# GenkiK/monodepth2

Measured on AMD Instinct MI355X. Metric: training images/sec at 640x192 mono, 1/2/4/8 GPUs; loss delta vs ref, higher is better.
Workload: dtype f32; 1 GPU; mono_640x192 ResNet-18 batch=12/GPU full train step (configs[1]); global_batch=12, height=192, width=640, parallelism=dp1, step=hipgraph replay

## Files before the change

include/md2hot.h:

```cpp
#ifndef MD2HOT_H
#define MD2HOT_H

#include <stddef.h>
#include <stdint.h>

#ifdef __cplusplus
extern "C" {
#endif

#define MD2_ABI_VERSION 24
#define MD2_MAX_SCALES 4
#define MD2_MAX_SRC 3

#define MD2_OK 0
#define MD2_ERR_ARG (-1)
#define MD2_ERR_HIP (-2)

#define MD2_NO_SSIM          (1u << 0)
#define MD2_AVG_REPROJECTION (1u << 1)
#define MD2_NO_AUTOMASK      (1u << 2)
#define MD2_V1_MULTISCALE    (1u << 3)
#define MD2_T_PER_SCALE      (1u << 4)
#define MD2_PREDICTIVE_MASK  (1u << 5)

#define MD2_DTYPE_F32  0u
#define MD2_DTYPE_BF16 1u

typedef struct md2_desc {
    int32_t batch;
    int32_t height, width;
    int32_t num_src;
    int32_t num_scales;
    uint32_t flags;
    float min_depth, max_depth;
    float disparity_smoothness;
    uint32_t disp_dtype;
    uint64_t seed;
} md2_desc;

typedef struct md2_tensors {
    const float* disp[MD2_MAX_SCALES];
    const float* color[MD2_MAX_SCALES][1 + MD2_MAX_SRC];
    const float* K[MD2_MAX_SCALES];
    const float* inv_K[MD2_MAX_SCALES];
    const float* T;
    const float* noise;
    const uint64_t* seed_ptr;
    const float* mask;
    const uint32_t* src8;
} md2_tensors;

int md2_abi_version(void);
const char* md2_last_error(void);
const char* md2_build_id(void);

size_t md2_workspace_bytes(const md2_desc* desc);

size_t md2_select_bytes(const md2_desc* desc);

int md2_photometric_fwd(const md2_desc* desc, const md2_tensors* t,
                        float* loss_out, uint8_t* select_out,
                        void* workspace, void* stream);

int md2_photometric_bwd(const md2_desc* desc, const md2_tensors* t,
                        const float* grad_loss, const uint8_t* select,
                        float* const* grad_disp, float* grad_T, float* grad_mask,
                        void* workspace, void* stream);

int md2_generate_images(const md2_desc* desc, const md2_tensors* t,
                        float* const* depth_out, float* const* sample_out,
                        float* const* color_out, void* stream);

int md2_tiebreak_noise(const md2_desc* desc, const uint64_t* seed_ptr, int scale,
                       float* out, void* stream);

int md2_timing_begin(int max_launches);
int md2_timing_end(double* fwd_ms, int* n_fwd, double* bwd_ms, int* n_bwd);
int md2_timing_calls(double* fwd_ms, int* n_fwd, double* bwd_ms, int* n_bwd);

#define MD2_PAD_ELU      (1u << 0)
#define MD2_PAD_UPSAMPLE (1u << 1)
#define MD2_PAD_NHWC     (1u << 2)
#define MD2_PAD_BF16     (1u << 3)

typedef struct md2_pad_desc {
    int32_t batch, channels, height, width;
    int32_t skip_channels;
    uint32_t flags;
} md2_pad_desc;

size_t md2_decoder_pad_workspace_bytes(const md2_pad_desc* desc);
int md2_decoder_pad_fwd(const md2_pad_desc* desc, const float* x, const float* skip, const float* bias,
                        float* out, void* stream);
int md2_decoder_pad_bwd(const md2_pad_desc* desc, const float* x, const float* bias, const float* grad_out,
                        float* grad_x, float* grad_skip, float* grad_bias, void* workspace, void* stream);
int md2_decoder_pad_bwd2(const md2_pad_desc* desc, const float* x, const float* bias, const float* grad_out,
                         const float* grad_out2, float* grad_x, float* grad_skip, float* grad_bias, void* workspace,
                         void* stream);

#define MD2_HEAD_WEIGHT_CL (1u << 0)
#define MD2_HEAD_BF16 (1u << 1)

typedef struct md2_head_desc {
    int32_t batch, channels, height, width;
    uint32_t flags;
} md2_head_desc;

size_t md2_disp_head_workspace_bytes(const md2_head_desc* desc);
int md2_disp_head_fwd(const md2_head_desc* desc, const float* padded, const float* weight, const float* bias,
                      float* disp, void* stream);
int md2_disp_head_bwd(const md2_head_desc* desc, const float* padded, const float* weight, const float* disp,
                      const float* grad_disp, float* grad_padded, float* grad_weight, float* grad_bias,
                      void* workspace, void* stream);

#define MD2_STEM_WEIGHT_CL (1u << 0)
#define MD2_STEM_BF16 (1u << 1)

typedef struct md2_stem_desc {
    int32_t batch, channels, height, width;
    uint32_t flags;
} md2_stem_desc;

size_t md2_stem_wgrad_workspace_bytes(const md2_stem_desc* desc);
int md2_stem_wgrad(const md2_stem_desc* desc, const float* x, const float* grad_y, float* grad_weight,
                   void* workspace, void* stream);

int md2_stem_fwd(const md2_stem_desc* desc, const float* x, const float* weight, float* y, void* stream);

#define MD2_BIAS_ACT_RELU (1u << 0)

typedef struct md2_bias_act_desc {
    int64_t pixels;
    int32_t channels;
    uint32_t flags;
} md2_bias_act_desc;

int md2_bias_act_fwd(const md2_bias_act_desc* desc, const float* x, const float* bias, float* y, void* stream);
size_t md2_bias_act_workspace_bytes(const md2_bias_act_desc* desc);
int md2_bias_act_bwd(const md2_bias_act_desc* desc, const float* y, const float* grad_y, float* grad_x,
                     float* grad_bias, void* workspace, void* stream);

int md2_encoder_input(int groups, int batch, int slots, int height, int width, const float* const* src, float mean,
                      float std_, float* out, void* stream);

typedef struct md2_adam_chunk {
    float* p;
    float* m;
    float* v;
    int64_t off;
    int64_t n;
    int32_t param;
    int32_t reserved;
} md2_adam_chunk;

int md2_adam_step(const md2_adam_chunk* table, const int* chunk_start, int nparams, const float* const* grads,
                  double lr, double beta1, double beta2, double eps, int step, void* stream);
int md2_adam_step_dev(const md2_adam_chunk* table, const int* chunk_start, int nparams, const float* const* grads,
                      const double* lr, double beta1, double beta2, double eps, float* step, float* hyper,
                      void* stream);
int md2_adam_hyper(const double* lr, double beta1, double beta2, float* step, float* hyper, void* stream);
int md2_adam_apply_dev(const md2_adam_chunk* table, const int* chunk_start, int k_begin, int k_end,
                       const float* const* grads, double beta1, double beta2, double eps, const float* hyper,
                       void* stream);

int md2_pose_fwd(int32_t frames, int32_t batch, uint32_t invert_mask, const float* axisangle,
                 const float* translation, float* T, void* stream);
int md2_pose_bwd(int32_t frames, int32_t batch, uint32_t invert_mask, const float* axisangle,
                 const float* translation, const float* grad_T, float* grad_axisangle,
                 float* grad_translation, void* stream);

typedef struct md2_aug_desc {
    int32_t items;
    int32_t frames;
    int32_t in_height, in_width;
    int32_t height, width;
    int32_t num_scales;
    int32_t reserved;
} md2_aug_desc;

#define MD2_AUG_BRIGHTNESS 0
#define MD2_AUG_CONTRAST   1
#define MD2_AUG_SATURATION 2
#define MD2_AUG_HUE        3

typedef struct md2_aug_item {
    uint8_t flip;
    uint8_t color_aug;
    uint8_t hue_shift;
    uint8_t reserved;
    uint8_t order[4];
    float brightness, contrast, saturation;
} md2_aug_item;

typedef struct md2_aug_plan md2_aug_plan;

md2_aug_plan* md2_aug_plan_create(const md2_aug_desc* desc);
void md2_aug_plan_destroy(md2_aug_plan* plan);

int md2_aug_run(md2_aug_plan* plan, const uint8_t* frames, const md2_aug_item* items,
                float* const* color, float* const* color_aug, void* stream);
int md2_aug_run2(md2_aug_plan* plan, const uint8_t* frames, const md2_aug_item* items,
                 float* const* color, float* const* color_aug, uint32_t* src8, void* stream);

#define MD2_BN_RELU     (1u << 0)
#define MD2_BN_RESIDUAL (1u << 1)
#define MD2_BN_BF16     (1u << 2)

typedef struct md2_bn_desc {
    int64_t pixels;
    int32_t channels;
    uint32_t flags;
    float eps, momentum;
    int32_t groups;
    int32_t reserved;
} md2_bn_desc;

size_t md2_bn_workspace_bytes(const md2_bn_desc* desc);
int md2_bn_fwd(const md2_bn_desc* desc, const void* x, const float* gamma, const float* beta,
               const void* residual, float* running_mean, float* running_var, void* y,
               float* save_mean, float* save_invstd, void* workspace, void* stream);
int md2_bn_bwd(const md2_bn_desc* desc, const void* x, const void* y, const void* grad_y,
               const float* gamma, const float* save_mean, const float* save_invstd,
               void* grad_x, void* grad_residual, float* grad_gamma, float* grad_beta,
               void* workspace, void* stream);
int md2_bn_bwd_multi(const md2_bn_desc* desc, const void* x, const void* y, const void* grad_y,
                     const void* grad_y2, const void* grad_y3, const float* gamma, const float* save_mean,
                     const float* save_invstd, void* grad_x, void* grad_residual, float* grad_gamma,
                     float* grad_beta, void* workspace, void* stream);
int md2_bn_fwd_mask(const md2_bn_desc* desc, const void* x, const float* gamma, const float* beta,
                    const void* residual, float* running_mean, float* running_var, void* y, uint8_t* relu_mask,
                    float* save_mean, float* save_invstd, void* workspace, void* stream);
int md2_bn_bwd_mask(const md2_bn_desc* desc, const void* x, const uint8_t* relu_mask, const void* grad_y,
                    const void* grad_y2, const void* grad_y3, const float* gamma, const float* save_mean,
                    const float* save_invstd, void* grad_x, void* grad_residual, float* grad_gamma,
                    float* grad_beta, void* workspace, void* stream);

#define MD2_POOL_BF16 (1u << 0)

typedef struct md2_pool_desc {
    int32_t batch, channels, height, width;
    uint32_t flags;
    int32_t reserved;
} md2_pool_desc;

int md2_maxpool3s2_fwd(const md2_pool_desc* desc, const void* x, void* y, uint32_t* idx, void* stream);
int md2_maxpool3s2_bwd(const md2_pool_desc* desc, const uint32_t* idx, const void* grad_y, void* grad_x,
                       void* stream);
int md2_maxpool3s2_bwd_add(const md2_pool_desc* desc, const uint32_t* idx, const void* grad_y, const void* grad_add,
                           void* grad_x, void* stream);
int md2_maxpool3s2_bwd_multi(const md2_pool_desc* desc, const uint32_t* idx, const void* grad_y, const void* grad_y2,
                             const void* grad_add, void* grad_x, void* stream);

#define MD2_CONV_NO_SPLIT  (1u << 1)
#define MD2_CONV_TILE_N32  (1u << 2)
#define MD2_CONV_TILE_N64  (1u << 3)
#define MD2_CONV_TILE_N128 (1u << 4)
#define MD2_CONV_X6        (1u << 5)
#define MD2_CONV_BM256     (1u << 6)
#define MD2_CONV_PRESPLIT  (1u << 7)
#define MD2_CONV_PATCH     (1u << 8)
#define MD2_CONV_S2_ONE    (1u << 9)
#define MD2_CONV_WS        (1u << 10)
#define MD2_CONV_BF16      (1u << 11)

typedef struct md2_conv_desc {
    int32_t batch, height, width, in_channels;
    int32_t out_channels, kernel_h, kernel_w, stride, pad;
    uint32_t flags;
} md2_conv_desc;

size_t md2_conv_workspace_bytes(const md2_conv_desc* desc);
int md2_conv_split_weights(const md2_conv_desc* desc, const float* weight, void* planes_fwd, void* planes_dgrad,
                           void* stream);
typedef struct md2_wsplit_entry {
    const float* weight;
    void* planes_fwd;
    void* planes_dgrad;
    int32_t co, kt, ci;
    int32_t block0;
    void* planes_col;
} md2_wsplit_entry;
int md2_conv_split_weights_multi(const md2_wsplit_entry* table, int n, int total_blocks, void* stream);
int md2_conv_bf16_weights(const md2_conv_desc* desc, const float* weight, void* w_fwd, void* w_dgrad, void* stream);
int md2_conv_bf16_weights_multi(const md2_wsplit_entry* table, int n, int total_blocks, void* stream);
int md2_conv_fwd(const md2_conv_desc* desc, const float* x, const float* weight, float* y, void* workspace,
                 void* stream);
int md2_conv_dgrad(const md2_conv_desc* desc, const float* grad_y, const float* weight, float* grad_x,
                   void* workspace, void* stream);
int md2_conv_col2im(const md2_conv_desc* desc, const float* cols, float* grad_x, void* stream);
int md2_conv_wgrad(const md2_conv_desc* desc, const float* x, const float* grad_y, float* grad_weight,
                   void* workspace, void* stream);
int md2_conv_direct(const md2_conv_desc* desc, const float* x, const float* wk, float* y, void* stream);
size_t md2_conv_wgrad_direct_workspace_bytes(const md2_conv_desc* desc);
int md2_conv_wgrad_direct(const md2_conv_desc* desc, const float* x, const float* grad_y, float* grad_weight,
                          void* workspace, void* stream);

#define MD2_EVAL_POST_PROCESS (1u << 0)
#define MD2_EVAL_RESIZE_DEPTH (1u << 1)
#define MD2_EVAL_GT_RANGE     (1u << 2)
#define MD2_EVAL_MEDIAN_SCALE (1u << 3)
#define MD2_EVAL_MEDIAN_LOWER (1u << 4)
#define MD2_EVAL_POOL_BATCH   (1u << 5)
#define MD2_EVAL_OUT 10

typedef struct md2_eval_desc {
    int32_t batch;
    int32_t height, width;
    int32_t gt_height, gt_width;
    int32_t crop_y0, crop_y1, crop_x0, crop_x1;
    uint32_t flags;
    double min_depth, max_depth;
    float eval_min, eval_max;
    double scale_factor;
} md2_eval_desc;

size_t md2_depth_eval_workspace_bytes(const md2_eval_desc* desc);
int md2_depth_eval(const md2_eval_desc* desc, const float* disp, const float* disp_flipped, const float* gt,
                   float* out, void* workspace, void* stream);

#define MD2_VELO_VEL_DEPTH (1u << 0)

typedef struct md2_velo_desc {
    int32_t batch;
    int32_t height, width;
    uint32_t flags;
    int64_t total_points;
    int32_t reserved[2];
} md2_velo_desc;

size_t md2_velo_project_workspace_bytes(const md2_velo_desc* desc);
int md2_velo_project(const md2_velo_desc* desc, const float* points, const int64_t* offsets, const double* P,
                     float* depth, void* workspace, void* stream);

typedef struct md2_pose_ate_desc {
    int32_t sequences;
    int32_t track_length;
    uint32_t flags;
    int32_t reserved0;
    int64_t total_frames;
    int64_t reserved;
} md2_pose_ate_desc;

size_t md2_pose_ate_workspace_bytes(const md2_pose_ate_desc* desc);
int md2_pose_ate(const md2_pose_ate_desc* desc, const float* pred, const double* gt, const int64_t* offsets,
                 double* ates, double* stats, void* workspace, void* stream);

typedef struct md2_viz_desc {
    int32_t batch;
    int32_t in_height, in_width;
    int32_t out_height, out_width;
    int32_t percentile;
    uint32_t flags;
    int32_t reserved;
} md2_viz_desc;

size_t md2_disp_colorize_workspace_bytes(const md2_viz_desc* desc);
int md2_disp_colorize(const md2_viz_desc* desc, const float* disp, uint8_t* rgb, float* resized, float* stats,
                      void* workspace, void* stream);

#ifdef __cplusplus
}
#endif
#endif
```

monodepth2_amd/_lib.py:

```python
from __future__ import annotations

import ctypes
import os
import threading

import torch

from .build import LIB_PATH as _BUILT_LIB
from .build import source_hash

LIB_PATH = os.environ.get("MD2_LIB", _BUILT_LIB)

MAX_SCALES = 4
MAX_SRC = 3
ABI_VERSION = 24

NO_SSIM = 1 << 0
AVG_REPROJECTION = 1 << 1
NO_AUTOMASK = 1 << 2
V1_MULTISCALE = 1 << 3
T_PER_SCALE = 1 << 4
PREDICTIVE_MASK = 1 << 5

_vp = ctypes.c_void_p


class Desc(ctypes.Structure):
    _fields_ = [("batch", ctypes.c_int32), ("height", ctypes.c_int32), ("width", ctypes.c_int32),
                ("num_src", ctypes.c_int32), ("num_scales", ctypes.c_int32), ("flags", ctypes.c_uint32),
                ("min_depth", ctypes.c_float), ("max_depth", ctypes.c_float),
                ("disparity_smoothness", ctypes.c_float), ("disp_dtype", ctypes.c_uint32),
                ("seed", ctypes.c_uint64)]


class Tensors(ctypes.Structure):
    _fields_ = [("disp", _vp * MAX_SCALES),
                ("color", (_vp * (1 + MAX_SRC)) * MAX_SCALES),
                ("K", _vp * MAX_SCALES),
                ("inv_K", _vp * MAX_SCALES),
                ("T", _vp),
                ("noise", _vp),
                ("seed_ptr", _vp),
                ("mask", _vp),
                ("src8", _vp)]


_lock = threading.Lock()
_lib = None

EXPORTS = ["md2_abi_version", "md2_last_error", "md2_workspace_bytes", "md2_select_bytes",
           "md2_photometric_fwd", "md2_photometric_bwd", "md2_generate_images", "md2_tiebreak_noise",
           "md2_timing_begin", "md2_timing_end", "md2_timing_calls", "md2_decoder_pad_fwd", "md2_decoder_pad_bwd",
           "md2_decoder_pad_workspace_bytes", "md2_adam_step", "md2_adam_step_dev", "md2_adam_hyper", "md2_adam_apply_dev", "md2_encoder_input",
           "md2_pose_fwd", "md2_pose_bwd", "md2_aug_plan_create", "md2_aug_plan_destroy", "md2_aug_run",
           "md2_bn_workspace_bytes", "md2_bn_fwd", "md2_bn_bwd", "md2_maxpool3s2_fwd", "md2_maxpool3s2_bwd",
           "md2_disp_head_workspace_bytes", "md2_disp_head_fwd", "md2_disp_head_bwd",
           "md2_stem_wgrad_workspace_bytes", "md2_stem_wgrad", "md2_stem_fwd", "md2_conv_col2im", "md2_bias_act_fwd", "md2_bias_act_bwd",
           "md2_bias_act_workspace_bytes", "md2_maxpool3s2_bwd_add", "md2_bn_bwd_multi",
           "md2_conv_fwd", "md2_conv_workspace_bytes", "md2_conv_split_weights",
           "md2_conv_dgrad", "md2_conv_wgrad", "md2_conv_direct", "md2_conv_wgrad_direct",
           "md2_conv_wgrad_direct_workspace_bytes", "md2_conv_split_weights_multi", "md2_bn_fwd_mask",
           "md2_bn_bwd_mask", "md2_build_id", "md2_maxpool3s2_bwd_multi", "md2_decoder_pad_bwd2", "md2_aug_run2",
           "md2_conv_bf16_weights", "md2_conv_bf16_weights_multi",
           "md2_depth_eval", "md2_depth_eval_workspace_bytes",
           "md2_velo_project", "md2_velo_project_workspace_bytes",
           "md2_pose_ate", "md2_pose_ate_workspace_bytes",
           "md2_disp_colorize", "md2_disp_colorize_workspace_bytes"]

DTYPE_F32 = 0
DTYPE_BF16 = 1
PAD_ELU = 1 << 0
PAD_UPSAMPLE = 1 << 1
PAD_NHWC = 1 << 2
PAD_BF16 = 1 << 3


class PadDesc(ctypes.Structure):
    _fields_ = [("batch", ctypes.c_int32), ("channels", ctypes.c_int32), ("height", ctypes.c_int32),
                ("width", ctypes.c_int32), ("skip_channels", ctypes.c_int32), ("flags", ctypes.c_uint32)]


class AugDesc(ctypes.Structure):
    _fields_ = [("items", ctypes.c_int32), ("frames", ctypes.c_int32), ("in_height", ctypes.c_int32),
                ("in_width", ctypes.c_int32), ("height", ctypes.c_int32), ("width", ctypes.c_int32),
                ("num_scales", ctypes.c_int32), ("reserved", ctypes.c_int32)]


class AugItem(ctypes.Structure):
    _fields_ = [("flip", ctypes.c_uint8), ("color_aug", ctypes.c_uint8), ("hue_shift", ctypes.c_uint8),
                ("reserved", ctypes.c_uint8), ("order", ctypes.c_uint8 * 4), ("brightness", ctypes.c_float),
                ("contrast", ctypes.c_float), ("saturation", ctypes.c_float)]


BN_RELU = 1 << 0
BN_RESIDUAL = 1 << 1
BN_BF16 = 1 << 2


class BnDesc(ctypes.Structure):
    _fields_ = [("pixels", ctypes.c_int64), ("channels", ctypes.c_int32), ("flags", ctypes.c_uint32),
                ("eps", ctypes.c_float), ("momentum", ctypes.c_float), ("groups", ctypes.c_int32),
                ("reserved", ctypes.c_int32)]


POOL_BF16 = 1 << 0


CONV_NO_SPLIT = 1 << 1
CONV_TILE_N32 = 1 << 2
CONV_TILE_N64 = 1 << 3
CONV_TILE_N128 = 1 << 4
CONV_X6 = 1 << 5
CONV_BM256 = 1 << 6
CONV_PRESPLIT = 1 << 7
CONV_PATCH = 1 << 8
CONV_S2_ONE = 1 << 9
CONV_WS = 1 << 10
CONV_BF16 = 1 << 11


class ConvDesc(ctypes.Structure):
    _fields_ = [("batch", ctypes.c_int32), ("height", ctypes.c_int32), ("width", ctypes.c_int32),
                ("in_channels", ctypes.c_int32), ("out_channels", ctypes.c_int32), ("kernel_h", ctypes.c_int32),
                ("kernel_w", ctypes.c_int32), ("stride", ctypes.c_int32), ("pad", ctypes.c_int32),
                ("flags", ctypes.c_uint32)]


class WsplitEntry(ctypes.Structure):
    _fields_ = [("weight", _vp), ("planes_fwd", _vp), ("planes_dgrad", _vp), ("co", ctypes.c_int32),
                ("kt", ctypes.c_int32), ("ci", ctypes.c_int32), ("block0", ctypes.c_int32), ("planes_col", _vp)]


class PoolDesc(ctypes.Structure):
    _fields_ = [("batch", ctypes.c_int32), ("channels", ctypes.c_int32), ("height", ctypes.c_int32),
                ("width", ctypes.c_int32), ("flags", ctypes.c_uint32), ("reserved", ctypes.c_int32)]


HEAD_WEIGHT_CL = 1 << 0
HEAD_BF16 = 1 << 1


class HeadDesc(ctypes.Structure):
    _fields_ = [("batch", ctypes.c_int32), ("channels", ctypes.c_int32), ("height", ctypes.c_int32),
                ("width", ctypes.c_int32), ("flags", ctypes.c_uint32)]


STEM_WEIGHT_CL = 1 << 0
STEM_BF16 = 1 << 1


class StemDesc(ctypes.Structure):
    _fields_ = [("batch", ctypes.c_int32), ("channels", ctypes.c_int32), ("height", ctypes.c_int32),
                ("width", ctypes.c_int32), ("flags", ctypes.c_uint32)]


BIAS_ACT_RELU = 1 << 0


class BiasActDesc(ctypes.Structure):
    _fields_ = [("pixels", ctypes.c_int64), ("channels", ctypes.c_int32), ("flags", ctypes.c_uint32)]


EVAL_POST_PROCESS = 1 << 0
EVAL_RESIZE_DEPTH = 1 << 1
EVAL_GT_RANGE = 1 << 2
EVAL_MEDIAN_SCALE = 1 << 3
EVAL_MEDIAN_LOWER = 1 << 4
EVAL_POOL_BATCH = 1 << 5
EVAL_OUT = 10


class EvalDesc(ctypes.Structure):
    _fields_ = [("batch", ctypes.c_int32), ("height", ctypes.c_int32), ("width", ctypes.c_int32),
                ("gt_height", ctypes.c_int32), ("gt_width", ctypes.c_int32),
                ("crop_y0", ctypes.c_int32), ("crop_y1", ctypes.c_int32), ("crop_x0", ctypes.c_int32),
                ("crop_x1", ctypes.c_int32), ("flags", ctypes.c_uint32),
                ("min_depth", ctypes.c_double), ("max_depth", ctypes.c_double),
                ("eval_min", ctypes.c_float), ("eval_max", ctypes.c_float),
                ("scale_factor", ctypes.c_double)]


VELO_VEL_DEPTH = 1 << 0


class VeloDesc(ctypes.Structure):
    _fields_ = [("batch", ctypes.c_int32), ("height", ctypes.c_int32), ("width", ctypes.c_int32),
                ("flags", ctypes.c_uint32), ("total_points", ctypes.c_int64), ("reserved", ctypes.c_int32 * 2)]


class PoseAteDesc(ctypes.Structure):
    _fields_ = [("sequences", ctypes.c_int32), ("track_length", ctypes.c_int32), ("flags", ctypes.c_uint32),
                ("reserved0", ctypes.c_int32), ("total_frames", ctypes.c_int64), ("reserved", ctypes.c_int64)]


class VizDesc(ctypes.Structure):
    _fields_ = [("batch", ctypes.c_int32), ("in_height", ctypes.c_int32), ("in_width", ctypes.c_int32),
                ("out_height", ctypes.c_int32), ("out_width", ctypes.c_int32), ("percentile", ctypes.c_int32),
                ("flags", ctypes.c_uint32), ("reserved", ctypes.c_int32)]


def _declare(L):
    L.md2_disp_colorize_workspace_bytes.restype = ctypes.c_size_t
    L.md2_disp_colorize_workspace_bytes.argtypes = [ctypes.POINTER(VizDesc)]
    L.md2_disp_colorize.restype = ctypes.c_int
    L.md2_disp_colorize.argtypes = [ctypes.POINTER(VizDesc)] + [_vp] * 6
    L.md2_pose_ate_workspace_bytes.restype = ctypes.c_size_t
    L.md2_pose_ate_workspace_bytes.argtypes = [ctypes.POINTER(PoseAteDesc)]
    L.md2_pose_ate.restype = ctypes.c_int
    L.md2_pose_ate.argtypes = [ctypes.POINTER(PoseAteDesc)] + [_vp] * 7
    L.md2_velo_project_workspace_bytes.restype = ctypes.c_size_t
    L.md2_velo_project_workspace_bytes.argtypes = [ctypes.POINTER(VeloDesc)]
    L.md2_velo_project.restype = ctypes.c_int
    L.md2_velo_project.argtypes = [ctypes.POINTER(VeloDesc)] + [_vp] * 6
    L.md2_depth_eval_workspace_bytes.restype = ctypes.c_size_t
    L.md2_depth_eval_workspace_bytes.argtypes = [ctypes.POINTER(EvalDesc)]
    L.md2_depth_eval.restype = ctypes.c_int
    L.md2_depth_eval.argtypes = [ctypes.POINTER(EvalDesc)] + [_vp] * 6
    L.md2_bias_act_fwd.restype = ctypes.c_int
    L.md2_bias_act_fwd.argtypes = [ctypes.POINTER(BiasActDesc)] + [_vp] * 4
    L.md2_bias_act_bwd.restype = ctypes.c_int
    L.md2_bias_act_bwd.argtypes = [ctypes.POINTER(BiasActDesc)] + [_vp] * 6
    L.md2_bias_act_workspace_bytes.restype = ctypes.c_size_t
    L.md2_bias_act_workspace_bytes.argtypes = [ctypes.POINTER(BiasActDesc)]
    L.md2_conv_fwd.restype = ctypes.c_int
    L.md2_conv_fwd.argtypes = [ctypes.POINTER(ConvDesc)] + [_vp] * 5
    L.md2_conv_dgrad.restype = ctypes.c_int
    L.md2_conv_dgrad.argtypes = [ctypes.POINTER(ConvDesc)] + [_vp] * 5
    L.md2_conv_wgrad.restype = ctypes.c_int
    L.md2_conv_wgrad.argtypes = [ctypes.POINTER(ConvDesc)] + [_vp] * 5
    L.md2_conv_split_weights.restype = ctypes.c_int
    L.md2_conv_direct.restype = ctypes.c_int
    L.md2_conv_direct.argtypes = [ctypes.POINTER(ConvDesc)] + [_vp] * 4
    L.md2_conv_wgrad_direct.restype = ctypes.c_int
    L.md2_conv_wgrad_direct.argtypes = [ctypes.POINTER(ConvDesc)] + [_vp] * 5
    L.md2_conv_wgrad_direct_workspace_bytes.restype = ctypes.c_size_t
    L.md2_conv_wgrad_direct_workspace_bytes.argtypes = [ctypes.POINTER(ConvDesc)]
    L.md2_conv_split_weights.argtypes = [ctypes.POINTER(ConvDesc)] + [_vp] * 4
    L.md2_conv_split_weights_multi.restype = ctypes.c_int
    L.md2_conv_split_weights_multi.argtypes = [_vp, ctypes.c_int, ctypes.c_int, _vp]
    L.md2_conv_bf16_weights.restype = ctypes.c_int
    L.md2_conv_bf16_weights.argtypes = [ctypes.POINTER(ConvDesc)] + [_vp] * 4
    L.md2_conv_bf16_weights_multi.restype = ctypes.c_int
    L.md2_conv_bf16_weights_multi.argtypes = [_vp, ctypes.c_int, ctypes.c_int, _vp]
    L.md2_conv_workspace_bytes.restype = ctypes.c_size_t
    L.md2_conv_workspace_bytes.argtypes = [ctypes.POINTER(ConvDesc)]
    L.md2_stem_wgrad_workspace_bytes.restype = ctypes.c_size_t
    L.md2_stem_wgrad_workspace_bytes.argtypes = [ctypes.POINTER(StemDesc)]
    L.md2_stem_wgrad.restype = ctypes.c_int
    L.md2_stem_wgrad.argtypes = [ctypes.POINTER(StemDesc)] + [_vp] * 5
    L.md2_stem_fwd.restype = ctypes.c_int
    L.md2_conv_col2im.restype = ctypes.c_int
    L.md2_conv_col2im.argtypes = [ctypes.POINTER(ConvDesc)] + [_vp] * 3
    L.md2_stem_fwd.argtypes = [ctypes.POINTER(StemDesc)] + [_vp] * 4
    L.md2_disp_head_workspace_bytes.restype = ctypes.c_size_t
    L.md2_disp_head_workspace_bytes.argtypes = [ctypes.POINTER(HeadDesc)]
    L.md2_disp_head_fwd.restype = ctypes.c_int
    L.md2_disp_head_fwd.argtypes = [ctypes.POINTER(HeadDesc)] + [_vp] * 5
    L.md2_disp_head_bwd.restype = ctypes.c_int
    L.md2_disp_head_bwd.argtypes = [ctypes.POINTER(HeadDesc)] + [_vp] * 9
    L.md2_abi_version.restype = ctypes.c_int
    L.md2_abi_version.argtypes = []
    L.md2_build_id.restype = ctypes.c_char_p
    L.md2_build_id.argtypes = []
    L.md2_last_error.restype = ctypes.c_char_p
    L.md2_last_error.argtypes = []
    L.md2_workspace_bytes.restype = ctypes.c_size_t
    L.md2_workspace_bytes.argtypes = [ctypes.POINTER(Desc)]
    L.md2_select_bytes.restype = ctypes.c_size_t
    L.md2_select_bytes.argtypes = [ctypes.POINTER(Desc)]
    L.md2_photometric_fwd.restype = ctypes.c_int
    L.md2_photometric_fwd.argtypes = [ctypes.POINTER(Desc), ctypes.POINTER(Tensors), _vp, _vp, _vp, _vp]
    L.md2_photometric_bwd.restype = ctypes.c_int
    L.md2_photometric_bwd.argtypes = [ctypes.POINTER(Desc), ctypes.POINTER(Tensors), _vp, _vp,
                                      ctypes.POINTER(_vp), _vp, _vp, _vp, _vp]
    L.md2_generate_images.restype = ctypes.c_int
    L.md2_generate_images.argtypes = [ctypes.POINTER(Desc), ctypes.POINTER(Tensors),
                                      ctypes.POINTER(_vp), ctypes.POINTER(_vp), ctypes.POINTER(_vp), _vp]
    L.md2_tiebreak_noise.restype = ctypes.c_int
    L.md2_tiebreak_noise.argtypes = [ctypes.POINTER(Desc), _vp, ctypes.c_int, _vp, _vp]
    L.md2_decoder_pad_fwd.restype = ctypes.c_int
    L.md2_decoder_pad_fwd.argtypes = [ctypes.POINTER(PadDesc), _vp, _vp, _vp, _vp, _vp]
    L.md2_decoder_pad_bwd.restype = ctypes.c_int
    L.md2_decoder_pad_bwd.argtypes = [ctypes.POINTER(PadDesc), _vp, _vp, _vp, _vp, _vp, _vp, _vp, _vp]
    L.md2_decoder_pad_bwd2.restype = ctypes.c_int
    L.md2_decoder_pad_bwd2.argtypes = [ctypes.POINTER(PadDesc)] + [_vp] * 9
    L.md2_encoder_input.restype = ctypes.c_int
    L.md2_encoder_input.argtypes = [ctypes.c_int, ctypes.c_int, ctypes.c_int, ctypes.c_int, ctypes.c_int, _vp,
                                    ctypes.c_float, ctypes.c_float, _vp, _vp]
    L.md2_adam_step.restype = ctypes.c_int
    L.md2_adam_step.argtypes = [_vp, _vp, ctypes.c_int, _vp, ctypes.c_double, ctypes.c_double, ctypes.c_double,
                                ctypes.c_double, ctypes.c_int, _vp]
    L.md2_adam_step_dev.restype = ctypes.c_int
    L.md2_adam_step_dev.argtypes = [_vp, _vp, ctypes.c_int, _vp, _vp, ctypes.c_double, ctypes.c_double,
                                    ctypes.c_double, _vp, _vp, _vp]
    L.md2_adam_hyper.restype = ctypes.c_int
    L.md2_adam_hyper.argtypes = [_vp, ctypes.c_double, ctypes.c_double, _vp, _vp, _vp]
    L.md2_adam_apply_dev.restype = ctypes.c_int
    L.md2_adam_apply_dev.argtypes = [_vp, _vp, ctypes.c_int, ctypes.c_int, _vp, ctypes.c_double, ctypes.c_double,
                                     ctypes.c_double, _vp, _vp]
    L.md2_decoder_pad_workspace_bytes.restype = ctypes.c_size_t
    L.md2_decoder_pad_workspace_bytes.argtypes = [ctypes.POINTER(PadDesc)]
    L.md2_pose_fwd.restype = ctypes.c_int
    L.md2_pose_fwd.argtypes = [ctypes.c_int32, ctypes.c_int32, ctypes.c_uint32, _vp, _vp, _vp, _vp]
    L.md2_pose_bwd.restype = ctypes.c_int
    L.md2_pose_bwd.argtypes = [ctypes.c_int32, ctypes.c_int32, ctypes.c_uint32, _vp, _vp, _vp, _vp, _vp, _vp]
    L.md2_aug_plan_create.restype = _vp
    L.md2_aug_plan_create.argtypes = [ctypes.POINTER(AugDesc)]
    L.md2_aug_plan_destroy.restype = None
    L.md2_aug_plan_destroy.argtypes = [_vp]
    L.md2_aug_run.restype = ctypes.c_int
    L.md2_aug_run.argtypes = [_vp, _vp, _vp, ctypes.POINTER(_vp), ctypes.POINTER(_vp), _vp]
    L.md2_aug_run2.restype = ctypes.c_int
    L.md2_aug_run2.argtypes = [_vp, _vp, _vp, ctypes.POINTER(_vp), ctypes.POINTER(_vp), _vp, _vp]
    L.md2_bn_workspace_bytes.restype = ctypes.c_size_t
    L.md2_bn_workspace_bytes.argtypes = [ctypes.POINTER(BnDesc)]
    L.md2_bn_fwd.restype = ctypes.c_int
    L.md2_bn_fwd.argtypes = [ctypes.POINTER(BnDesc)] + [_vp] * 11
    L.md2_bn_bwd.restype = ctypes.c_int
    L.md2_bn_bwd.argtypes = [ctypes.POINTER(BnDesc)] + [_vp] * 12
    L.md2_maxpool3s2_fwd.restype = ctypes.c_int
    L.md2_maxpool3s2_fwd.argtypes = [ctypes.POINTER(PoolDesc), _vp, _vp, _vp, _vp]
    L.md2_maxpool3s2_bwd.restype = ctypes.c_int
    L.md2_maxpool3s2_bwd.argtypes = [ctypes.POINTER(PoolDesc), _vp, _vp, _vp, _vp]
    L.md2_bn_bwd_multi.restype = ctypes.c_int
    L.md2_bn_bwd_multi.argtypes = [ctypes.POINTER(BnDesc)] + [_vp] * 14
    L.md2_bn_fwd_mask.restype = ctypes.c_int
    L.md2_bn_fwd_mask.argtypes = [ctypes.POINTER(BnDesc)] + [_vp] * 12
    L.md2_bn_bwd_mask.restype = ctypes.c_int
    L.md2_bn_bwd_mask.argtypes = [ctypes.POINTER(BnDesc)] + [_vp] * 14
    L.md2_maxpool3s2_bwd_add.restype = ctypes.c_int
    L.md2_maxpool3s2_bwd_add.argtypes = [ctypes.POINTER(PoolDesc)] + [_vp] * 5
    L.md2_maxpool3s2_bwd_multi.restype = ctypes.c_int
    L.md2_maxpool3s2_bwd_multi.argtypes = [ctypes.POINTER(PoolDesc)] + [_vp] * 6
    L.md2_timing_begin.restype = ctypes.c_int
    L.md2_timing_begin.argtypes = [ctypes.c_int]
    L.md2_timing_calls.restype = ctypes.c_int
    L.md2_timing_calls.argtypes = [ctypes.POINTER(ctypes.c_double), ctypes.POINTER(ctypes.c_int),
                                   ctypes.POINTER(ctypes.c_double), ctypes.POINTER(ctypes.c_int)]
    L.md2_timing_end.restype = ctypes.c_int
    L.md2_timing_end.argtypes = [ctypes.POINTER(ctypes.c_double), ctypes.POINTER(ctypes.c_int),
                                 ctypes.POINTER(ctypes.c_double), ctypes.POINTER(ctypes.c_int)]


def lib():
    global _lib
    if _lib is not None:
        return _lib
    with _lock:
        if _lib is None:
            if not os.path.exists(LIB_PATH):
                raise RuntimeError(
                    f"{LIB_PATH} is not built. Build it with `python -m monodepth2_amd.build` "
                    "(hipcc --offload-arch=gfx950); there is no CPU fallback.")
            L = ctypes.CDLL(LIB_PATH, mode=ctypes.RTLD_GLOBAL)
# ... 47 lines not shown
```

monodepth2_amd/bn_ops.py:

```python
from __future__ import annotations

import contextlib
import ctypes
import os
from typing import Dict, Optional

import torch
import torch.nn as nn
import torch.nn.functional as F

from . import _lib

ENABLED = True
_GROUPS = 1


@contextlib.contextmanager
def bn_groups(n: int):
    global _GROUPS
    prev, _GROUPS = _GROUPS, int(n)
    try:
        yield
    finally:
        _GROUPS = prev
# ... 18 lines not shown
_descs: Dict[tuple, tuple] = {}


def _desc(key: tuple):
    hit = _descs.get(key)
    if hit is None:
        d = _lib.BnDesc(*key, 0)
        hit = _descs[key] = (d, _lib.lib().md2_bn_workspace_bytes(ctypes.byref(d)))
    return hit


def _supported(C: int) -> bool:
    Q = C // 4
    return C % 4 == 0 and Q > 0 and (Q & (Q - 1)) == 0


class _BNAct(torch.autograd.Function):

    @staticmethod
    def forward(ctx, x, weight, bias, running_mean, running_var, residual, relu: bool, eps: float,
                momentum: float, groups: int, aliases: int = 0):
        B, C, H, W = x.shape
        flags = ((_lib.BN_RELU if relu else 0) | (_lib.BN_RESIDUAL if residual is not None else 0)
                 | (_lib.BN_BF16 if x.dtype == torch.bfloat16 else 0))
        key = (B * H * W, C, flags, eps, momentum, groups)
        d, nbytes = _desc(key)
        L = _lib.lib()
        ws = _workspace(x.device, nbytes)
        y = torch.empty_like(x, memory_format=_CL)
        stats = torch.empty(2, groups, C, device=x.device)
        mean, invstd = stats[0], stats[1]
        mask = torch.empty(x.numel() // 4, dtype=torch.uint8, device=x.device) if relu else None
        stream = _lib.stream(x.device)
        rc = L.md2_bn_fwd_mask(ctypes.byref(d), x.data_ptr(), weight.data_ptr(), bias.data_ptr(),
                               residual.data_ptr() if residual is not None else None,
                               running_mean.data_ptr() if running_mean is not None else None,
                               running_var.data_ptr() if running_var is not None else None,
                               y.data_ptr(), mask.data_ptr() if mask is not None else None,
                               mean.data_ptr(), invstd.data_ptr(), ws.data_ptr(), stream)
        _lib.check(rc, "md2_bn_fwd_mask")
        ctx.save_for_backward(x, mask, weight, mean, invstd)
        ctx.desc = key
        ctx.has_res = residual is not None
        if aliases:
            ctx.set_materialize_grads(False)
            return (y,) + tuple(y.view_as(y) for _ in range(aliases))
        return y

    @staticmethod
    def backward(ctx, *grads):
        x, mask, weight, mean, invstd = ctx.saved_tensors
        gs = [g.to(x.dtype).contiguous(memory_format=_CL) for g in grads if g is not None]
        if not gs:
            return (None,) * 11
        gy = gs[0]
        d, nbytes = _desc(ctx.desc)
        L = _lib.lib()
        ws = _workspace(x.device, nbytes)
        gx = torch.empty_like(x, memory_format=_CL)
        gr = torch.empty_like(x, memory_format=_CL) if ctx.has_res else None
        gw = torch.empty_like(weight)
        gb = torch.empty_like(weight)
        bwd, name = (L.md2_bn_bwd_mask, "md2_bn_bwd_mask") if mask is not None else \
            (L.md2_bn_bwd_multi, "md2_bn_bwd_multi")
        rc = bwd(ctypes.byref(d), x.data_ptr(), mask.data_ptr() if mask is not None else None,
                 gy.data_ptr(), gs[1].data_ptr() if len(gs) > 1 else None,
                 gs[2].data_ptr() if len(gs) > 2 else None,
                 weight.data_ptr(), mean.data_ptr(), invstd.data_ptr(), gx.data_ptr(),
                 gr.data_ptr() if gr is not None else None, gw.data_ptr(), gb.data_ptr(), ws.data_ptr(),
                 _lib.stream(x.device))
        _lib.check(rc, name)
        return gx, gw, gb, None, None, gr, None, None, None, None, None


def bn_act(bn: nn.BatchNorm2d, x: torch.Tensor, residual: Optional[torch.Tensor] = None,
           relu: bool = True, aliases: int = 0):
    if not 0 <= aliases <= 2:
        raise ValueError("bn_act: at most two aliases")
    groups = _GROUPS if bn.training else 1
    if groups > 1 and x.shape[0] % groups:
        raise ValueError(f"batch {x.shape[0]} does not split into {groups} BatchNorm groups")
    if (ENABLED and bn.training and x.is_cuda and x.dtype in (torch.float32, torch.bfloat16) and x.dim() == 4
            and bn.affine and bn.track_running_stats and bn.momentum is not None and _supported(x.shape[1])
            and x.numel() // 4 // groups < 2 ** 31
            and x.is_contiguous(memory_format=_CL) and x.shape[1] > 1
            and (residual is None or residual.is_contiguous(memory_format=_CL))):
        if residual is not None and residual.dtype != x.dtype:
            residual = residual.to(x.dtype)
        if bn.num_batches_tracked is not None:
            bn.num_batches_tracked.add_(groups)
        k = aliases if torch.is_grad_enabled() else 0
        out = _BNAct.apply(x, bn.weight, bn.bias, bn.running_mean, bn.running_var, residual, relu, bn.eps,
                           bn.momentum, groups, k)
        if aliases and not k:
            return (out,) * (aliases + 1)
        return out
    y = bn(x) if groups == 1 else torch.cat([bn(xc) for xc in x.chunk(groups)], 0)
    if residual is not None:
        y = y + residual
    y = F.relu(y) if relu else y
    return (y,) * (aliases + 1) if aliases else y


_ALIAS_SUM = os.environ.get("MD2_ALIAS_SUM", "1") != "0"


class _MaxPool(torch.autograd.Function):

    @staticmethod
    def forward(ctx, x, with_alias: bool = False, out_alias: bool = False):
        B, C, H, W = x.shape
        Ho, Wo = (H - 1) // 2 + 1, (W - 1) // 2 + 1
        d = _lib.PoolDesc(B, C, H, W, _lib.POOL_BF16 if x.dtype == torch.bfloat16 else 0, 0)
        y = torch.empty((B, C, Ho, Wo), device=x.device, dtype=x.dtype, memory_format=_CL)
        idx = torch.empty(B * Ho * Wo * C // 4, device=x.device, dtype=torch.int32)
        stream = _lib.stream(x.device)
        _lib.check(_lib.lib().md2_maxpool3s2_fwd(ctypes.byref(d), x.data_ptr(), y.data_ptr(), idx.data_ptr(), stream),
                   "md2_maxpool3s2_fwd")
        ctx.save_for_backward(idx)
        ctx.desc = (B, C, H, W, d.flags, 0)
        ctx.xshape, ctx.dtype = x.shape, x.dtype
        ctx.with_alias, ctx.out_alias = with_alias, out_alias
        if not (with_alias or out_alias):
            return y
        ctx.set_materialize_grads(False)
        outs = (y,) + ((y.view_as(y),) if out_alias else ()) + ((x.view_as(x),) if with_alias else ())
        return outs

    @staticmethod
    def backward(ctx, gy, *rest):
        (idx,) = ctx.saved_tensors
        rest = list(rest)
        gy2 = rest.pop(0) if ctx.out_alias else None
        galias = rest.pop(0) if ctx.with_alias else None
        if gy is None:
            gy, gy2 = gy2, None
        if gy is None:
            return (galias.to(ctx.dtype) if galias is not None else None), None, None
        gy = gy.to(ctx.dtype).contiguous(memory_format=_CL)
        if gy2 is not None:
            gy2 = gy2.to(ctx.dtype).contiguous(memory_format=_CL)
        if galias is not None:
            galias = galias.to(ctx.dtype).contiguous(memory_format=_CL)
        gx = torch.empty(ctx.xshape, device=gy.device, dtype=ctx.dtype, memory_format=_CL)
        d = _lib.PoolDesc(*ctx.desc)
        _lib.check(_lib.lib().md2_maxpool3s2_bwd_multi(ctypes.byref(d), idx.data_ptr(), gy.data_ptr(),
                                                       gy2.data_ptr() if gy2 is not None else None,
                                                       galias.data_ptr() if galias is not None else None,
                                                       gx.data_ptr(), _lib.stream(gy.device)),
                   "md2_maxpool3s2_bwd_multi")
        return gx, None, None


def _pool_ok(pool: nn.MaxPool2d, x: torch.Tensor) -> bool:
    return (ENABLED and x.is_cuda and x.dim() == 4 and x.dtype in (torch.float32, torch.bfloat16)
            and x.shape[1] % 4 == 0 and x.is_contiguous(memory_format=_CL)
            and pool.kernel_size in (3, (3, 3)) and pool.stride in (2, (2, 2)) and pool.padding in (1, (1, 1))
            and pool.dilation in (1, (1, 1)) and not pool.ceil_mode and not pool.return_indices)


def max_pool_3x3s2(pool: nn.MaxPool2d, x: torch.Tensor) -> torch.Tensor:
    if _pool_ok(pool, x):
        return _MaxPool.apply(x, False)
    return pool(x)


def max_pool_3x3s2_with_alias(pool: nn.MaxPool2d, x: torch.Tensor, out_alias: bool = False):
    if _pool_ok(pool, x) and torch.is_grad_enabled() and x.requires_grad:
        if out_alias and not _ALIAS_SUM:
            y, xa = _MaxPool.apply(x, True, False)
            return y, y, xa
        return _MaxPool.apply(x, True, out_alias)
    y = max_pool_3x3s2(pool, x)
    return (y, y, x) if out_alias else (y, x)
```

monodepth2_amd/build.py:

```python
from __future__ import annotations

import hashlib
import os
import shutil
import subprocess
import sys

HERE = os.path.dirname(os.path.abspath(__file__))
CSRC = os.path.join(HERE, "csrc")
INCLUDE = os.path.join(os.path.dirname(HERE), "include")
LIB_NAME = "libmd2hot.so"
LIB_PATH = os.path.join(CSRC, LIB_NAME)
SOURCES = ["md2hot.hip", "decoder.hip", "pose.hip", "augment.hip", "bnorm.hip", "pool.hip", "adam.hip", "disphead.hip", "stem.hip", "bias_act.hip", "conv.hip", "direct.hip", "glue.hip", "eval.hip", "velo.hip", "traj.hip", "viz.hip"]
ARCH = os.environ.get("MD2_OFFLOAD_ARCH", "gfx950")


def hipcc() -> str:
    for cand in (os.environ.get("HIPCC"), "/opt/rocm/bin/hipcc", shutil.which("hipcc")):
        if cand and os.path.exists(cand):
            return cand
    raise RuntimeError("hipcc not found (ROCm toolchain required to build libmd2hot.so)")


def needs_build() -> bool:
    if not os.path.exists(LIB_PATH):
        return True
    t = os.path.getmtime(LIB_PATH)
    deps = [os.path.join(CSRC, s) for s in SOURCES] + [os.path.join(INCLUDE, "md2hot.h"),
                                                       os.path.join(CSRC, "md2_bf16.h")]
    if any(os.path.getmtime(d) > t for d in deps):
        return True
    return built_id(LIB_PATH) != source_hash()


def built_id(path: str):
    try:
        with open(path, "rb") as f:
            data = f.read()
    except OSError:
        return None
    i = data.find(BUILD_ID_MARKER)
    if i < 0:
        return None
    i += len(BUILD_ID_MARKER)
    return data[i:i + 16].decode("ascii", errors="replace")


BUILD_ID_MARKER = b"md2-build-id:"


FLAGS = {"md2hot.hip": ["-fno-slp-vectorize", "-mllvm", "--amdgpu-sched-strategy=iterative-ilp"],
         "conv.hip": ["-mllvm", "--amdgpu-sched-strategy=max-ilp"],
         "bnorm.hip": ["-mllvm", "--amdgpu-sched-strategy=max-ilp"],
         "decoder.hip": ["-mllvm", "--amdgpu-sched-strategy=max-ilp"],
         "disphead.hip": ["-fno-slp-vectorize"], "glue.hip": ["-fno-slp-vectorize"]}


def source_hash() -> str:
    h = hashlib.sha256()
    for path in [os.path.join(CSRC, s) for s in SOURCES] + [os.path.join(INCLUDE, "md2hot.h"),
                                                          os.path.join(CSRC, "md2_bf16.h")]:
        h.update(os.path.basename(path).encode())
        with open(path, "rb") as f:
            h.update(f.read())
    h.update(repr(sorted(FLAGS.items())).encode())
    h.update(ARCH.encode())
    return h.hexdigest()[:16]


def build(force: bool = False, verbose: bool = False) -> str:
    if not force and not needs_build():
        return LIB_PATH
    import concurrent.futures as cf
    objdir = os.path.join(CSRC, "obj")
    os.makedirs(objdir, exist_ok=True)
    base = [hipcc(), "-O3", f"--offload-arch={ARCH}", "-std=c++17", "-fPIC", "-I" + INCLUDE]
    bid = ['-DMD2_BUILD_ID="%s"' % source_hash()]

    def compile_one(src):
        obj = os.path.join(objdir, os.path.splitext(src)[0] + ".o")
        cmd = base + FLAGS.get(src, []) + (bid if src == "glue.hip" else []) + ["-c", os.path.join(CSRC, src), "-o", obj]
        if verbose:
            print(" ".join(cmd), file=sys.stderr)
        subprocess.run(cmd, check=True)
        return obj

    with cf.ThreadPoolExecutor(max_workers=min(len(SOURCES), os.cpu_count() or 1)) as ex:
        objs = list(ex.map(compile_one, SOURCES))
    tmp = LIB_PATH + ".tmp"
    cmd = [hipcc(), f"--offload-arch={ARCH}", "-fPIC", "-shared", "-o", tmp] + objs
    if verbose:
        print(" ".join(cmd), file=sys.stderr)
    subprocess.run(cmd, check=True)
    os.replace(tmp, LIB_PATH)
    return LIB_PATH


if __name__ == "__main__":
    print(build(force="--force" in sys.argv, verbose=True))
```

monodepth2_amd/csrc/bnorm.hip:

```cpp

#include <hip/hip_runtime.h>

#include <stdint.h>
#include <stdlib.h>

#include "md2_bf16.h"
#include "md2hot.h"

int md2_report_error(int code, const char* msg);

namespace {

constexpr int kThreads = 256;
constexpr int kMaxBlocks = 1024;

struct Map {
    int Q;
    int QPT;
    int PPB;
};

__host__ __device__ inline Map make_map(int C) {
    Map m;
    m.Q = C / 4;
    m.QPT = m.Q > kThreads ? m.Q / kThreads : 1;
    m.PPB = m.Q >= kThreads ? 1 : kThreads / m.Q;
    return m;
}

struct Work {
    float* part;
    float* coef;
};

__host__ __device__ __forceinline__ Work work(void* ws, int G, int C, int NG) {
    Work w;
    w.part = (float*)ws;
    w.coef = w.part + 2 * (size_t)NG * G * C;
    return w;
}

__device__ __forceinline__ float4 ld4(const float* p) { return *(const float4*)p; }
__device__ __forceinline__ void st4(float* p, float4 v) { *(float4*)p = v; }

template <typename T>
__device__ __forceinline__ float4 ldT(const void* p, size_t off) { return md2::ld4T<T>(p, off); }
template <typename T>
__device__ __forceinline__ void stT(void* p, size_t off, float4 v) { md2::st4T<T>(p, off, v); }

__device__ void block_partials(float4 a, float4 b, int q, int pl, const Map& m, int C, int rows, int row, Work w,
                               float4 (*lds)[kThreads]) {
    lds[0][threadIdx.x] = a;
    lds[1][threadIdx.x] = b;
    __syncthreads();
    for (int half = m.PPB / 2; half > 0; half /= 2) {
        if (pl < half) {
            const int o = threadIdx.x + half * m.Q;
            const float4 u = lds[0][o], v = lds[1][o];
            a.x += u.x; a.y += u.y; a.z += u.z; a.w += u.w;
            b.x += v.x; b.y += v.y; b.z += v.z; b.w += v.w;
            lds[0][threadIdx.x] = a;
            lds[1][threadIdx.x] = b;
        }
        __syncthreads();
    }
    if (pl == 0) {
        float* pa = w.part + (size_t)(4 * q) * rows + row;
        float* pb = w.part + ((size_t)C + 4 * q) * rows + row;
        pa[0] = a.x; pa[rows] = a.y; pa[2 * (size_t)rows] = a.z; pa[3 * (size_t)rows] = a.w;
        pb[0] = b.x; pb[rows] = b.y; pb[2 * (size_t)rows] = b.z; pb[3 * (size_t)rows] = b.w;
    }
    __syncthreads();
}

template <typename T>
__global__ void __launch_bounds__(kThreads) bn_stats_kernel(const void* __restrict__ x, long long P, int C, int G,
                                                            void* ws) {
    const Map m = make_map(C);
    const int NG = gridDim.y, grp = blockIdx.y;
    const Work w = work(ws, G, C, NG);
    x = (const char*)x + (size_t)grp * P * C * sizeof(T);
    __shared__ float4 lds[2][kThreads];
    for (int qq = 0; qq < m.QPT; ++qq) {
        const int q = (threadIdx.x % m.Q) + qq * kThreads, pl = threadIdx.x / m.Q;
        float4 s = {0.f, 0.f, 0.f, 0.f}, ss = {0.f, 0.f, 0.f, 0.f};
        auto acc = [&](const float4 v) {
            s.x += v.x; s.y += v.y; s.z += v.z; s.w += v.w;
            ss.x += v.x * v.x; ss.y += v.y * v.y; ss.z += v.z * v.z; ss.w += v.w * v.w;
        };
        const long long stride = (long long)G * m.PPB;
        long long p = (long long)blockIdx.x * m.PPB + pl;
        for (; p + 3 * stride < P; p += 4 * stride) {
            const float4 v0 = ldT<T>(x, p * C + 4 * q), v1 = ldT<T>(x, (p + stride) * C + 4 * q),
                         v2 = ldT<T>(x, (p + 2 * stride) * C + 4 * q), v3 = ldT<T>(x, (p + 3 * stride) * C + 4 * q);
            acc(v0); acc(v1); acc(v2); acc(v3);
        }
        for (; p < P; p += stride) acc(ldT<T>(x, p * C + 4 * q));
        block_partials(s, ss, q, pl, m, C, NG * G, grp * G + blockIdx.x, w, lds);
    }
}

__device__ bool channel_sums(Work w, int rows, int r0, int G, int C, int c, double& a, double& b) {
    __shared__ double red[2][kThreads / 64];
    static_assert(kMaxBlocks <= 4 * kThreads, "four partial rows per thread at most");
    const float* ca = w.part + (size_t)c * rows + r0;
    const float* cb = w.part + ((size_t)C + c) * rows + r0;
    float pa[4], pb[4];
#pragma unroll
    for (int u = 0; u < 4; ++u) {
        const int g = threadIdx.x + u * kThreads;
        pa[u] = g < G ? ca[g] : 0.f;
        pb[u] = g < G ? cb[g] : 0.f;
    }
    a = 0.0;
    b = 0.0;
#pragma unroll
    for (int u = 0; u < 4; ++u) {
        a += pa[u];
        b += pb[u];
    }
#pragma unroll
    for (int o = 32; o > 0; o >>= 1) {
        a += __shfl_xor(a, o, 64);
        b += __shfl_xor(b, o, 64);
    }
    if ((threadIdx.x & 63) == 0) {
        red[0][threadIdx.x >> 6] = a;
        red[1][threadIdx.x >> 6] = b;
    }
    __syncthreads();
    a = red[0][0];
    b = red[1][0];
#pragma unroll
    for (int i = 1; i < kThreads / 64; ++i) {
        a += red[0][i];
        b += red[1][i];
    }
    __syncthreads();
    return threadIdx.x == 0;
}

__global__ void __launch_bounds__(kThreads) bn_stats_final_kernel(long long P, int C, int G, int NG, float eps,
                                                                  float momentum, float* __restrict__ rmean,
                                                                  float* __restrict__ rvar,
                                                                  float* __restrict__ smean,
                                                                  float* __restrict__ sinvstd, void* ws) {
    const int c = blockIdx.x;
    const Work w = work(ws, G, C, NG);
    for (int grp = 0; grp < NG; ++grp) {
        double a, b;
        if (!channel_sums(w, NG * G, grp * G, G, C, c, a, b)) continue;
        const double mean = a / (double)P;
        double var = b / (double)P - mean * mean;
        var = var > 0.0 ? var : 0.0;
        smean[grp * C + c] = (float)mean;
        sinvstd[grp * C + c] = (float)(1.0 / sqrt(var + (double)eps));
        if (rmean) {
            rmean[c] = (float)((1.0 - momentum) * rmean[c] + momentum * mean);
            rvar[c] = (float)((1.0 - momentum) * rvar[c] + momentum * var * (double)P / (double)(P - 1));
        }
    }
}

template <typename T>
__device__ __forceinline__ bool stored_pos(float o) {
    if constexpr (sizeof(T) == 4) return o > 0.f;
    else return md2::bf2f(md2::f2bf(o)) > 0.f;
}

template <typename T, bool RELU, bool RES, bool MOUT = false>
__global__ void __launch_bounds__(kThreads) bn_apply_kernel(const void* __restrict__ x, const void* __restrict__ r,
                                                            const float* __restrict__ gamma,
                                                            const float* __restrict__ beta,
                                                            const float* __restrict__ smean,
                                                            const float* __restrict__ sinvstd, void* __restrict__ y,
                                                            int n4g, int Q, uint8_t* __restrict__ mask = nullptr) {
    const size_t base = (size_t)blockIdx.y * n4g;
    const float* mug = smean + (size_t)blockIdx.y * 4 * Q;
    const float* isg = sinvstd + (size_t)blockIdx.y * 4 * Q;
    for (int j = blockIdx.x * kThreads + threadIdx.x; j < n4g; j += gridDim.x * kThreads) {
        const size_t i = base + j;
        const int c = 4 * (j & (Q - 1));
        const float4 v = ldT<T>(x, 4 * i), mu = ld4(mug + c), is = ld4(isg + c), ga = ld4(gamma + c),
                     be = ld4(beta + c);
        float4 o;
        o.x = (v.x - mu.x) * is.x * ga.x + be.x;
        o.y = (v.y - mu.y) * is.y * ga.y + be.y;
        o.z = (v.z - mu.z) * is.z * ga.z + be.z;
        o.w = (v.w - mu.w) * is.w * ga.w + be.w;
        if (RES) {
            const float4 rv = ldT<T>(r, 4 * i);
            o.x += rv.x; o.y += rv.y; o.z += rv.z; o.w += rv.w;
        }
        if (RELU) {
            o.x = fmaxf(o.x, 0.f); o.y = fmaxf(o.y, 0.f); o.z = fmaxf(o.z, 0.f); o.w = fmaxf(o.w, 0.f);
        }
        stT<T>(y, 4 * i, o);
        if (MOUT)
            mask[i] = (uint8_t)((stored_pos<T>(o.x) ? 1 : 0) | (stored_pos<T>(o.y) ? 2 : 0) |
                                (stored_pos<T>(o.z) ? 4 : 0) | (stored_pos<T>(o.w) ? 8 : 0));
    }
}

template <typename T, bool MIN>
__device__ __forceinline__ float4 relu_gate(const void* y, size_t off, float4 g) {
    if constexpr (MIN) {
        const uint32_t m = ((const uint8_t*)y)[off >> 2];
        g.x = (m & 1) ? g.x : 0.f; g.y = (m & 2) ? g.y : 0.f; g.z = (m & 4) ? g.z : 0.f; g.w = (m & 8) ? g.w : 0.f;
    } else {
        const float4 yv = ldT<T>(y, off);
        g.x = yv.x > 0.f ? g.x : 0.f; g.y = yv.y > 0.f ? g.y : 0.f;
        g.z = yv.z > 0.f ? g.z : 0.f; g.w = yv.w > 0.f ? g.w : 0.f;
    }
    return g;
}

template <typename T>
__device__ __forceinline__ float4 ld_grad(const void* g, const void* g2, const void* g3, size_t off) {
    float4 v = ldT<T>(g, off);
    if (g2) {
        const float4 u = ldT<T>(g2, off);
        v.x += u.x; v.y += u.y; v.z += u.z; v.w += u.w;
    }
    if (g3) {
        const float4 u = ldT<T>(g3, off);
        v.x += u.x; v.y += u.y; v.z += u.z; v.w += u.w;
    }
    return v;
}

template <typename T, bool RELU, bool MIN = false>
__global__ void __launch_bounds__(kThreads) bn_bwd_reduce_kernel(const void* __restrict__ x,
                                                                 const void* __restrict__ y,
                                                                 const void* __restrict__ g,
                                                                 const void* __restrict__ g2,
                                                                 const void* __restrict__ g3, long long P, int C,
                                                                 int G, const float* __restrict__ smean, void* ws) {
    const Map m = make_map(C);
    const int NG = gridDim.y, grp = blockIdx.y;
    const Work w = work(ws, G, C, NG);
    const size_t base = (size_t)grp * P * C;
    __shared__ float4 lds[2][kThreads];
    for (int qq = 0; qq < m.QPT; ++qq) {
        const int q = (threadIdx.x % m.Q) + qq * kThreads, pl = threadIdx.x / m.Q;
        const float4 mu = ld4(smean + grp * C + 4 * q);
        float4 s = {0.f, 0.f, 0.f, 0.f}, sx = {0.f, 0.f, 0.f, 0.f};
        auto acc = [&](float4 gv, const float4 v) {
            s.x += gv.x; s.y += gv.y; s.z += gv.z; s.w += gv.w;
            sx.x += gv.x * (v.x - mu.x); sx.y += gv.y * (v.y - mu.y);
            sx.z += gv.z * (v.z - mu.z); sx.w += gv.w * (v.w - mu.w);
        };
        const long long stride = (long long)G * m.PPB;
        long long p = (long long)blockIdx.x * m.PPB + pl;
        for (; p + stride < P; p += 2 * stride) {
            const size_t o0 = base + p * C + 4 * q, o1 = base + (p + stride) * C + 4 * q;
            float4 g0 = ld_grad<T>(g, g2, g3, o0), g1 = ld_grad<T>(g, g2, g3, o1);
            if (RELU) {
                g0 = relu_gate<T, MIN>(y, o0, g0);
                g1 = relu_gate<T, MIN>(y, o1, g1);
            }
            const float4 v0 = ldT<T>(x, o0), v1 = ldT<T>(x, o1);
            acc(g0, v0);
            acc(g1, v1);
        }
        for (; p < P; p += stride) {
            const size_t o = base + p * C + 4 * q;
            float4 gv = ld_grad<T>(g, g2, g3, o);
            if (RELU) gv = relu_gate<T, MIN>(y, o, gv);
            acc(gv, ldT<T>(x, o));
        }
        block_partials(s, sx, q, pl, m, C, NG * G, grp * G + blockIdx.x, w, lds);
    }
}

__global__ void __launch_bounds__(kThreads) bn_bwd_final_kernel(long long P, int C, int G, int NG,
                                                                const float* __restrict__ gamma,
                                                                const float* __restrict__ sinvstd,
                                                                float* __restrict__ dgamma, float* __restrict__ dbeta,
                                                                void* ws) {
    const int c = blockIdx.x;
    const Work w = work(ws, G, C, NG);
    double sdg = 0.0, sdb = 0.0;
    for (int grp = 0; grp < NG; ++grp) {
        double a, b;
        if (!channel_sums(w, NG * G, grp * G, G, C, c, a, b)) continue;
        const double is = sinvstd[grp * C + c];
        const double dg = b * is;
        sdg += dg;
        sdb += a;
        const size_t gc = (size_t)grp * C + c;
        w.coef[gc] = (float)((double)gamma[c] * is);
        w.coef[(size_t)NG * C + gc] = (float)(a / (double)P);
        w.coef[2 * (size_t)NG * C + gc] = (float)(dg * is / (double)P);
    }
    if (threadIdx.x == 0) {
        dgamma[c] = (float)sdg;
        dbeta[c] = (float)sdb;
    }
}

template <typename T, bool RELU, bool RES, bool MIN = false>
__global__ void __launch_bounds__(kThreads) bn_bwd_apply_kernel(const void* __restrict__ x,
                                                                const void* __restrict__ y,
                                                                const void* __restrict__ g,
                                                                const void* __restrict__ g2,
                                                                const void* __restrict__ g3,
                                                                const float* __restrict__ smean, const float* coef,
                                                                void* __restrict__ dx, void* __restrict__ dr,
                                                                int n4g, int Q, int C, int NG) {
    const size_t base = (size_t)blockIdx.y * n4g;
    const size_t gc = (size_t)blockIdx.y * C;
    for (int j = blockIdx.x * kThreads + threadIdx.x; j < n4g; j += gridDim.x * kThreads) {
        const size_t i = base + j;
        const size_t c = gc + 4 * (j & (Q - 1));
        float4 gv = ld_grad<T>(g, g2, g3, 4 * i);
        if (RELU) gv = relu_gate<T, MIN>(y, 4 * i, gv);
        const float4 v = ldT<T>(x, 4 * i), mu = ld4(smean + c), k1 = ld4(coef + c),
                     k2 = ld4(coef + (size_t)NG * C + c), k3 = ld4(coef + 2 * (size_t)NG * C + c);
        float4 o;
        o.x = k1.x * (gv.x - k2.x - (v.x - mu.x) * k3.x);
        o.y = k1.y * (gv.y - k2.y - (v.y - mu.y) * k3.y);
        o.z = k1.z * (gv.z - k2.z - (v.z - mu.z) * k3.z);
        o.w = k1.w * (gv.w - k2.w - (v.w - mu.w) * k3.w);
        stT<T>(dx, 4 * i, o);
        if (RES) stT<T>(dr, 4 * i, gv);
    }
}

__device__ __forceinline__ void ld8bf(const void* p, size_t off, float (&v)[8]) {
    const uint4 r = *(const uint4*)((const uint16_t*)p + off);
    const uint32_t w[4] = {r.x, r.y, r.z, r.w};
#pragma unroll
    for (int i = 0; i < 4; ++i) {
        v[2 * i] = md2::bf2f(w[i] & 0xffffu);
        v[2 * i + 1] = md2::bf2f(w[i] >> 16);
    }
}
__device__ __forceinline__ void st8bf(void* p, size_t off, const float (&v)[8]) {
    *(uint4*)((uint16_t*)p + off) =
        make_uint4(md2::f2bf(v[0]) | (md2::f2bf(v[1]) << 16), md2::f2bf(v[2]) | (md2::f2bf(v[3]) << 16),
                   md2::f2bf(v[4]) | (md2::f2bf(v[5]) << 16), md2::f2bf(v[6]) | (md2::f2bf(v[7]) << 16));
}
__device__ __forceinline__ void ld8f(const float* p, float (&v)[8]) {
    const float4 a = ld4(p), b = ld4(p + 4);
    v[0] = a.x; v[1] = a.y; v[2] = a.z; v[3] = a.w; v[4] = b.x; v[5] = b.y; v[6] = b.z; v[7] = b.w;
}

template <bool RELU, bool RES, bool MOUT = false>
__global__ void __launch_bounds__(kThreads) bn_apply8_kernel(const void* __restrict__ x, const void* __restrict__ r,
                                                             const float* __restrict__ gamma,
                                                             const float* __restrict__ beta,
                                                             const float* __restrict__ smean,
                                                             const float* __restrict__ sinvstd, void* __restrict__ y,
                                                             int n8g, int Q8, uint8_t* __restrict__ mask = nullptr) {
    const size_t base = (size_t)blockIdx.y * n8g;
    const float* mug = smean + (size_t)blockIdx.y * 8 * Q8;
    const float* isg = sinvstd + (size_t)blockIdx.y * 8 * Q8;
    for (int j = blockIdx.x * kThreads + threadIdx.x; j < n8g; j += gridDim.x * kThreads) {
        const size_t i = base + j;
        const int c = 8 * (j & (Q8 - 1));
        float v[8], mu[8], is[8], ga[8], be[8], o[8];
        ld8bf(x, 8 * i, v);
        ld8f(mug + c, mu);
        ld8f(isg + c, is);
        ld8f(gamma + c, ga);
        ld8f(beta + c, be);
#pragma unroll
        for (int e = 0; e < 8; ++e) o[e] = (v[e] - mu[e]) * is[e] * ga[e] + be[e];
        if (RES) {
            float rv[8];
            ld8bf(r, 8 * i, rv);
#pragma unroll
            for (int e = 0; e < 8; ++e) o[e] += rv[e];
        }
        if (RELU) {
#pragma unroll
            for (int e = 0; e < 8; ++e) o[e] = fmaxf(o[e], 0.f);
        }
        st8bf(y, 8 * i, o);
        if (MOUT) {
            uint32_t m = 0;
#pragma unroll
            for (int e = 0; e < 8; ++e) m |= (stored_pos<uint16_t>(o[e]) ? 1u : 0u) << ((e & 3) + 8 * (e >> 2));
            ((uint16_t*)mask)[i] = (uint16_t)m;
        }
    }
}

template <bool RELU, bool RES, bool MIN = false>
__global__ void __launch_bounds__(kThreads) bn_bwd_apply8_kernel(const void* __restrict__ x,
                                                                 const void* __restrict__ y,
                                                                 const void* __restrict__ g,
                                                                 const void* __restrict__ g2,
                                                                 const void* __restrict__ g3,
                                                                 const float* __restrict__ smean, const float* coef,
                                                                 void* __restrict__ dx, void* __restrict__ dr,
                                                                 int n8g, int Q8, int C, int NG) {
    const size_t base = (size_t)blockIdx.y * n8g;
    const size_t gc = (size_t)blockIdx.y * C;
    for (int j = blockIdx.x * kThreads + threadIdx.x; j < n8g; j += gridDim.x * kThreads) {
        const size_t i = base + j;
        const size_t c = gc + 8 * (j & (Q8 - 1));
        float gv[8];
        ld8bf(g, 8 * i, gv);
        if (g2) {
            float u[8];
            ld8bf(g2, 8 * i, u);
#pragma unroll
            for (int e = 0; e < 8; ++e) gv[e] += u[e];
        }
        if (g3) {
            float u[8];
            ld8bf(g3, 8 * i, u);
#pragma unroll
            for (int e = 0; e < 8; ++e) gv[e] += u[e];
        }
        if (RELU) {
            if constexpr (MIN) {
                const uint32_t m = ((const uint16_t*)y)[i];
#pragma unroll
                for (int e = 0; e < 8; ++e) gv[e] = ((m >> ((e & 3) + 8 * (e >> 2))) & 1u) ? gv[e] : 0.f;
            } else {
                float yv[8];
                ld8bf(y, 8 * i, yv);
#pragma unroll
                for (int e = 0; e < 8; ++e) gv[e] = yv[e] > 0.f ? gv[e] : 0.f;
            }
        }
        float v[8], mu[8], k1[8], k2[8], k3[8], o[8];
        ld8bf(x, 8 * i, v);
        ld8f(smean + c, mu);
        ld8f(coef + c, k1);
        ld8f(coef + (size_t)NG * C + c, k2);
        ld8f(coef + 2 * (size_t)NG * C + c, k3);
#pragma unroll
        for (int e = 0; e < 8; ++e) o[e] = k1[e] * (gv[e] - k2[e] - (v[e] - mu[e]) * k3[e]);
        st8bf(dx, 8 * i, o);
        if (RES) st8bf(dr, 8 * i, gv);
    }
}

template <bool UNUSED = false>
__global__ void __launch_bounds__(kThreads) bn_stats8_kernel(const void* __restrict__ x, long long P, int C, int G,
                                                             void* ws) {
    const int Q8 = C / 8;
    const Map m8 = {Q8, 1, kThreads / Q8};
    const int NG = gridDim.y, grp = blockIdx.y;
    const Work w = work(ws, G, C, NG);
    x = (const char*)x + (size_t)grp * P * C * 2;
    __shared__ float4 lds[2][kThreads];
    const int q8 = threadIdx.x % Q8, pl = threadIdx.x / Q8;
    float v[8], s[8], ss[8];
#pragma unroll
    for (int e = 0; e < 8; ++e) s[e] = ss[e] = 0.f;
    auto acc = [&]() {
#pragma unroll
        for (int e = 0; e < 8; ++e) {
            s[e] += v[e];
            ss[e] += v[e] * v[e];
        }
    };
    const long long stride = (long long)G * m8.PPB;
    for (long long p = (long long)blockIdx.x * m8.PPB + pl; p < P; p += stride) {
        ld8bf(x, p * C + 8 * q8, v);
        acc();
    }
    block_partials(make_float4(s[0], s[1], s[2], s[3]), make_float4(ss[0], ss[1], ss[2], ss[3]), 2 * q8, pl, m8, C,
                   NG * G, grp * G + blockIdx.x, w, lds);
    block_partials(make_float4(s[4], s[5], s[6], s[7]), make_float4(ss[4], ss[5], ss[6], ss[7]), 2 * q8 + 1, pl, m8,
                   C, NG * G, grp * G + blockIdx.x, w, lds);
}

template <bool RELU, bool MIN = false>
__global__ void __launch_bounds__(kThreads) bn_bwd_reduce8_kernel(const void* __restrict__ x,
                                                                  const void* __restrict__ y,
                                                                  const void* __restrict__ g,
                                                                  const void* __restrict__ g2,
                                                                  const void* __restrict__ g3, long long P, int C,
                                                                  int G, const float* __restrict__ smean, void* ws) {
    const int Q8 = C / 8;
    const Map m8 = {Q8, 1, kThreads / Q8};
    const int NG = gridDim.y, grp = blockIdx.y;
    const Work w = work(ws, G, C, NG);
    const size_t base = (size_t)grp * P * C;
    __shared__ float4 lds[2][kThreads];
    const int q8 = threadIdx.x % Q8, pl = threadIdx.x / Q8;
    float mu[8], s[8], sx[8];
    ld8f(smean + grp * C + 8 * q8, mu);
#pragma unroll
    for (int e = 0; e < 8; ++e) s[e] = sx[e] = 0.f;
    const long long stride = (long long)G * m8.PPB;
    for (long long p = (long long)blockIdx.x * m8.PPB + pl; p < P; p += stride) {
        const size_t o = base + p * C + 8 * q8;
        float gv[8], v[8];
        ld8bf(g, o, gv);
        if (g2) {
            float u[8];
            ld8bf(g2, o, u);
#pragma unroll
            for (int e = 0; e < 8; ++e) gv[e] += u[e];
        }
        if (g3) {
            float u[8];
            ld8bf(g3, o, u);
#pragma unroll
            for (int e = 0; e < 8; ++e) gv[e] += u[e];
        }
        if (RELU) {
            if constexpr (MIN) {
                const uint32_t m = ((const uint16_t*)y)[o / 8];
#pragma unroll
                for (int e = 0; e < 8; ++e) gv[e] = ((m >> ((e & 3) + 8 * (e >> 2))) & 1u) ? gv[e] : 0.f;
            } else {
                float yv[8];
                ld8bf(y, o, yv);
#pragma unroll
                for (int e = 0; e < 8; ++e) gv[e] = yv[e] > 0.f ? gv[e] : 0.f;
            }
        }
        ld8bf(x, o, v);
#pragma unroll
        for (int e = 0; e < 8; ++e) {
            s[e] += gv[e];
            sx[e] += gv[e] * (v[e] - mu[e]);
        }
    }
    block_partials(make_float4(s[0], s[1], s[2], s[3]), make_float4(sx[0], sx[1], sx[2], sx[3]), 2 * q8, pl, m8, C,
                   NG * G, grp * G + blockIdx.x, w, lds);
    block_partials(make_float4(s[4], s[5], s[6], s[7]), make_float4(sx[4], sx[5], sx[6], sx[7]), 2 * q8 + 1, pl, m8,
                   C, NG * G, grp * G + blockIdx.x, w, lds);
}

bool reduce8_on() {
    static const bool on = [] {
        const char* e = getenv("MD2_BN_RED8");
        return !(e && e[0] == '0');
    }();
    return on;
}

bool apply8_on() {
    static const bool on = [] {
        const char* e = getenv("MD2_BN_V8");
        return !(e && e[0] == '0');
    }();
    return on;
}

int blocks_for_stats(long long P, int C) {
    const Map m = make_map(C);
    const long long rows = (P + m.PPB - 1) / m.PPB;
    const long long g = (rows + 7) / 8;
    return (int)(g < 1 ? 1 : (g > kMaxBlocks ? kMaxBlocks : g));
}

int grid_elem(long long n4, int NG) {
    const long long cap = (4096 + NG - 1) / NG;
    const long long g = (n4 + kThreads - 1) / kThreads;
    return (int)(g < cap ? g : cap);
}

int groups_of(const md2_bn_desc* d) { return d->groups > 1 ? d->groups : 1; }

bool valid(const md2_bn_desc* d) {
    if (!d || d->channels < 4 || d->channels % 4) return false;
    if (d->groups < 0 || d->pixels % groups_of(d) || d->pixels / groups_of(d) < 2) return false;
    const int Q = d->channels / 4;
    if ((Q & (Q - 1)) != 0) return false;
    if ((long long)d->pixels / groups_of(d) * Q >= (1ll << 31)) return false;
    return Q >= kThreads ? (Q % kThreads == 0) : (kThreads % Q == 0);
}

template <typename T>
void launch_fwd(const md2_bn_desc* d, const void* x, const float* gamma, const float* beta, const void* residual,
                float* running_mean, float* running_var, void* y, float* save_mean, float* save_invstd,
                void* workspace, hipStream_t st, uint8_t* mask = nullptr) {
    const int NG = groups_of(d);
    const long long P = d->pixels / NG;
    const int C = d->channels, G = blocks_for_stats(P, C);
    if (sizeof(T) == 2 && C % 8 == 0 && C <= 8 * kThreads && reduce8_on())
        hipLaunchKernelGGL(bn_stats8_kernel<>, dim3(G, NG), dim3(kThreads), 0, st, x, P, C, G, workspace);
    else
        hipLaunchKernelGGL(bn_stats_kernel<T>, dim3(G, NG), dim3(kThreads), 0, st, x, P, C, G, workspace);
    hipLaunchKernelGGL(bn_stats_final_kernel, dim3(C), dim3(kThreads), 0, st, P, C, G, NG, d->eps, d->momentum,
                       running_mean, running_var, save_mean, save_invstd, workspace);
    const int n4g = (int)(P * C / 4);
    const bool relu = d->flags & MD2_BN_RELU, res = d->flags & MD2_BN_RESIDUAL;
    if (sizeof(T) == 2 && C % 8 == 0 && apply8_on()) {
        auto k8 = relu ? (mask ? (res ? bn_apply8_kernel<true, true, true> : bn_apply8_kernel<true, false, true>)
                               : (res ? bn_apply8_kernel<true, true> : bn_apply8_kernel<true, false>))
                       : (res ? bn_apply8_kernel<false, true> : bn_apply8_kernel<false, false>);
        hipLaunchKernelGGL(k8, dim3(grid_elem(n4g / 2, NG), NG), dim3(kThreads), 0, st, x, residual, gamma, beta,
                           save_mean, save_invstd, y, n4g / 2, C / 8, mask);
        return;
    }
    auto k = relu ? (mask ? (res ? bn_apply_kernel<T, true, true, true> : bn_apply_kernel<T, true, false, true>)
                          : (res ? bn_apply_kernel<T, true, true> : bn_apply_kernel<T, true, false>))
                  : (res ? bn_apply_kernel<T, false, true> : bn_apply_kernel<T, false, false>);
    hipLaunchKernelGGL(k, dim3(grid_elem(n4g, NG), NG), dim3(kThreads), 0, st, x, residual, gamma, beta, save_mean,
                       save_invstd, y, n4g, C / 4, mask);
}

template <typename T>
void launch_bwd(const md2_bn_desc* d, const void* x, const void* y, const void* grad_y, const void* grad_y2,
                const void* grad_y3, const float* gamma,
                const float* save_mean, const float* save_invstd, void* grad_x, void* grad_residual,
                float* grad_gamma, float* grad_beta, void* workspace, hipStream_t st, bool mask_in = false) {
    const int NG = groups_of(d);
    const long long P = d->pixels / NG;
    const int C = d->channels, G = blocks_for_stats(P, C);
    const bool relu = d->flags & MD2_BN_RELU, res = d->flags & MD2_BN_RESIDUAL;
    auto red = relu ? (mask_in ? bn_bwd_reduce_kernel<T, true, true> : bn_bwd_reduce_kernel<T, true>)
                    : bn_bwd_reduce_kernel<T, false>;
    if (sizeof(T) == 2 && C % 8 == 0 && C <= 8 * kThreads && reduce8_on())
        red = relu ? (mask_in ? bn_bwd_reduce8_kernel<true, true> : bn_bwd_reduce8_kernel<true>)
                   : bn_bwd_reduce8_kernel<false>;
    hipLaunchKernelGGL(red, dim3(G, NG), dim3(kThreads), 0, st, x, y, grad_y, grad_y2, grad_y3, P, C, G, save_mean,
                       workspace);
    hipLaunchKernelGGL(bn_bwd_final_kernel, dim3(C), dim3(kThreads), 0, st, P, C, G, NG, gamma, save_invstd,
                       grad_gamma, grad_beta, workspace);
    const int n4g = (int)(P * C / 4);
    const float* coef = work(workspace, G, C, NG).coef;
    if (sizeof(T) == 2 && C % 8 == 0 && apply8_on()) {
        auto k8 = relu ? (mask_in ? (res ? bn_bwd_apply8_kernel<true, true, true> : bn_bwd_apply8_kernel<true, false, true>)
                                  : (res ? bn_bwd_apply8_kernel<true, true> : bn_bwd_apply8_kernel<true, false>))
                       : (res ? bn_bwd_apply8_kernel<false, true> : bn_bwd_apply8_kernel<false, false>);
        hipLaunchKernelGGL(k8, dim3(grid_elem(n4g / 2, NG), NG), dim3(kThreads), 0, st, x, y, grad_y, grad_y2,
                           grad_y3, save_mean, coef, grad_x, grad_residual, n4g / 2, C / 8, C, NG);
        return;
    }
    auto k = relu ? (mask_in ? (res ? bn_bwd_apply_kernel<T, true, true, true> : bn_bwd_apply_kernel<T, true, false, true>)
                             : (res ? bn_bwd_apply_kernel<T, true, true> : bn_bwd_apply_kernel<T, true, false>))
                  : (res ? bn_bwd_apply_kernel<T, false, true> : bn_bwd_apply_kernel<T, false, false>);
    hipLaunchKernelGGL(k, dim3(grid_elem(n4g, NG), NG), dim3(kThreads), 0, st, x, y, grad_y, grad_y2, grad_y3,
                       save_mean, coef, grad_x, grad_residual, n4g, C / 4, C, NG);
}

}

extern "C" {

size_t md2_bn_workspace_bytes(const md2_bn_desc* d) {
    if (!valid(d)) return 0;
    const int NG = groups_of(d);
    const int G = blocks_for_stats(d->pixels / NG, d->channels);
    return (2 * (size_t)NG * G * d->channels + 3 * (size_t)NG * d->channels) * sizeof(float);
}

int md2_bn_fwd_mask(const md2_bn_desc* d, const void* x, const float* gamma, const float* beta, const void* residual,
                    float* running_mean, float* running_var, void* y, uint8_t* relu_mask, float* save_mean,
                    float* save_invstd, void* workspace, void* stream) {
    if (!valid(d)) return md2_report_error(MD2_ERR_ARG, "bn: need pixels >= 2 and channels a multiple of 4 "
                                                        "with channels/4 dividing (or a multiple of) 256");
    if (!x || !gamma || !beta || !y || !save_mean || !save_invstd || !workspace ||
        ((d->flags & MD2_BN_RESIDUAL) && !residual) || (!running_mean != !running_var))
        return md2_report_error(MD2_ERR_ARG, "bn_fwd: NULL operand");
    if (relu_mask && !(d->flags & MD2_BN_RELU)) return md2_report_error(MD2_ERR_ARG, "bn_fwd: relu_mask without MD2_BN_RELU");
    if (d->flags & MD2_BN_BF16)
        launch_fwd<uint16_t>(d, x, gamma, beta, residual, running_mean, running_var, y, save_mean, save_invstd,
                             workspace, (hipStream_t)stream, relu_mask);
    else
        launch_fwd<float>(d, x, gamma, beta, residual, running_mean, running_var, y, save_mean, save_invstd,
                          workspace, (hipStream_t)stream, relu_mask);
    const hipError_t e = hipGetLastError();
    return e == hipSuccess ? MD2_OK : md2_report_error(MD2_ERR_HIP, hipGetErrorString(e));
}

int md2_bn_fwd(const md2_bn_desc* d, const void* x, const float* gamma, const float* beta, const void* residual,
               float* running_mean, float* running_var, void* y, float* save_mean, float* save_invstd,
               void* workspace, void* stream) {
    return md2_bn_fwd_mask(d, x, gamma, beta, residual, running_mean, running_var, y, nullptr, save_mean, save_invstd,
                           workspace, stream);
}

static int bn_bwd_impl(const md2_bn_desc* d, const void* x, const void* y, bool mask_in, const void* grad_y,
                       const void* grad_y2, const void* grad_y3, const float* gamma, const float* save_mean,
                       const float* save_invstd, void* grad_x, void* grad_residual, float* grad_gamma,
                       float* grad_beta, void* workspace, void* stream) {
    if (!valid(d)) return md2_report_error(MD2_ERR_ARG, "bn: unsupported shape");
    const bool relu = d->flags & MD2_BN_RELU, res = d->flags & MD2_BN_RESIDUAL;
    if (!x || !grad_y || !gamma || !save_mean || !save_invstd || !grad_x || !grad_gamma || !grad_beta ||
        !workspace || (relu && !y) || (res && !grad_residual) || (grad_y3 && !grad_y2))
        return md2_report_error(MD2_ERR_ARG, "bn_bwd: NULL operand");
    if (d->flags & MD2_BN_BF16)
        launch_bwd<uint16_t>(d, x, y, grad_y, grad_y2, grad_y3, gamma, save_mean, save_invstd, grad_x,
                             grad_residual, grad_gamma, grad_beta, workspace, (hipStream_t)stream, mask_in);
    else
        launch_bwd<float>(d, x, y, grad_y, grad_y2, grad_y3, gamma, save_mean, save_invstd, grad_x, grad_residual,
                          grad_gamma, grad_beta, workspace, (hipStream_t)stream, mask_in);
    const hipError_t e = hipGetLastError();
    return e == hipSuccess ? MD2_OK : md2_report_error(MD2_ERR_HIP, hipGetErrorString(e));
}

int md2_bn_bwd_multi(const md2_bn_desc* d, const void* x, const void* y, const void* grad_y, const void* grad_y2,
                     const void* grad_y3, const float* gamma, const float* save_mean, const float* save_invstd,
                     void* grad_x, void* grad_residual, float* grad_gamma, float* grad_beta, void* workspace,
                     void* stream) {
    return bn_bwd_impl(d, x, y, false, grad_y, grad_y2, grad_y3, gamma, save_mean, save_invstd, grad_x, grad_residual,
                       grad_gamma, grad_beta, workspace, stream);
}

int md2_bn_bwd_mask(const md2_bn_desc* d, const void* x, const uint8_t* relu_mask, const void* grad_y,
                    const void* grad_y2, const void* grad_y3, const float* gamma, const float* save_mean,
                    const float* save_invstd, void* grad_x, void* grad_residual, float* grad_gamma, float* grad_beta,
                    void* workspace, void* stream) {
    if (!(d && (d->flags & MD2_BN_RELU))) return md2_report_error(MD2_ERR_ARG, "bn_bwd_mask: needs MD2_BN_RELU");
    return bn_bwd_impl(d, x, relu_mask, true, grad_y, grad_y2, grad_y3, gamma, save_mean, save_invstd, grad_x,
                       grad_residual, grad_gamma, grad_beta, workspace, stream);
}

int md2_bn_bwd(const md2_bn_desc* d, const void* x, const void* y, const void* grad_y, const float* gamma,
               const float* save_mean, const float* save_invstd, void* grad_x, void* grad_residual,
               float* grad_gamma, float* grad_beta, void* workspace, void* stream) {
    return md2_bn_bwd_multi(d, x, y, grad_y, nullptr, nullptr, gamma, save_mean, save_invstd, grad_x, grad_residual,
                            grad_gamma, grad_beta, workspace, stream);
}

}
```

monodepth2_amd/csrc/pool.hip:

```cpp

#include <hip/hip_runtime.h>

#include <math.h>
#include <stdint.h>
#include <stdlib.h>

#include "md2_bf16.h"
#include "md2hot.h"

int md2_report_error(int code, const char* msg);

namespace {

constexpr int kThreads = 256;

struct PoolArgs {
    int B, H, W, C, Ho, Wo;
};

__device__ __forceinline__ void take(float v, int k, float& m, int& a) {
    if (v > m || isnan(v)) {
        m = v;
        a = k;
    }
}

template <typename T>
__global__ void __launch_bounds__(kThreads) maxpool_fwd_kernel(PoolArgs p, const void* __restrict__ x,
                                                               void* __restrict__ y, uint32_t* __restrict__ idx) {
    const int C4 = p.C / 4;
    const int n = p.B * p.Ho * p.Wo * C4;
    for (int i = blockIdx.x * kThreads + threadIdx.x; i < n; i += gridDim.x * kThreads) {
        const int c = 4 * (i % C4);
        int t = i / C4;
        const int ox = t % p.Wo;
        t /= p.Wo;
        const int oy = t % p.Ho;
        const int b = t / p.Ho;
        float m[4] = {-INFINITY, -INFINITY, -INFINITY, -INFINITY};
        const int k0 = (oy == 0 ? 3 : 0) + (ox == 0 ? 1 : 0);
        int a[4] = {k0, k0, k0, k0};
        for (int ky = 0; ky < 3; ++ky) {
            const int iy = 2 * oy - 1 + ky;
            if (iy < 0 || iy >= p.H) continue;
            for (int kx = 0; kx < 3; ++kx) {
                const int ix = 2 * ox - 1 + kx;
                if (ix < 0 || ix >= p.W) continue;
                const float4 v = md2::ld4T<T>(x, (((size_t)b * p.H + iy) * p.W + ix) * p.C + c);
                const int k = ky * 3 + kx;
                take(v.x, k, m[0], a[0]);
                take(v.y, k, m[1], a[1]);
                take(v.z, k, m[2], a[2]);
                take(v.w, k, m[3], a[3]);
            }
        }
        md2::st4T<T>(y, 4 * i, make_float4(m[0], m[1], m[2], m[3]));
        idx[i] = (uint32_t)a[0] | ((uint32_t)a[1] << 8) | ((uint32_t)a[2] << 16) | ((uint32_t)a[3] << 24);
    }
}

template <typename T>
__global__ void __launch_bounds__(kThreads) maxpool_bwd_kernel(PoolArgs p, const uint32_t* __restrict__ idx,
                                                               const void* __restrict__ gy, const void* __restrict__ gy2,
                                                               const void* __restrict__ ga, void* __restrict__ gx) {
    const int C4 = p.C / 4;
    const int n = p.B * p.H * p.W * C4;
    for (int i = blockIdx.x * kThreads + threadIdx.x; i < n; i += gridDim.x * kThreads) {
        const int c4 = i % C4;
        int t = i / C4;
        const int ix = t % p.W;
        t /= p.W;
        const int iy = t % p.H;
        const int b = t / p.H;
        float s[4] = {0.f, 0.f, 0.f, 0.f};
        for (int oy = iy / 2; oy <= (iy + 1) / 2; ++oy) {
            if (oy < 0 || oy >= p.Ho || 2 * oy - 1 > iy || 2 * oy + 1 < iy) continue;
            for (int ox = ix / 2; ox <= (ix + 1) / 2; ++ox) {
                if (ox < 0 || ox >= p.Wo || 2 * ox - 1 > ix || 2 * ox + 1 < ix) continue;
                const size_t o = (((size_t)b * p.Ho + oy) * p.Wo + ox) * C4 + c4;
                const uint32_t w = idx[o];
                const int k = (iy - (2 * oy - 1)) * 3 + (ix - (2 * ox - 1));
                float4 g = md2::ld4T<T>(gy, 4 * o);
                if (gy2) {
                    const float4 h = md2::ld4T<T>(gy2, 4 * o);
                    g.x += h.x; g.y += h.y; g.z += h.z; g.w += h.w;
                }
                if ((int)(w & 255u) == k) s[0] += g.x;
                if ((int)((w >> 8) & 255u) == k) s[1] += g.y;
                if ((int)((w >> 16) & 255u) == k) s[2] += g.z;
                if ((int)(w >> 24) == k) s[3] += g.w;
            }
        }
        if (ga) {
            const float4 v = md2::ld4T<T>(ga, 4 * (size_t)i);
            s[0] += v.x; s[1] += v.y; s[2] += v.z; s[3] += v.w;
        }
        md2::st4T<T>(gx, 4 * i, make_float4(s[0], s[1], s[2], s[3]));
    }
}

template <typename T>
__global__ void __launch_bounds__(kThreads) maxpool_bwd_rows_kernel(PoolArgs p, int c4_shift,
                                                                    const uint32_t* __restrict__ idx,
                                                                    const void* __restrict__ gy,
                                                                    const void* __restrict__ gy2,
                                                                    const void* __restrict__ ga, void* __restrict__ gx) {
    const int C4 = p.C / 4;
    const int j = blockIdx.x * kThreads + threadIdx.x;
    if (j >= p.W * C4) return;
    const int row = blockIdx.y, b = row / p.H, iy = row - b * p.H;
    const int c4 = j & (C4 - 1), ix = j >> c4_shift;
    float s[4] = {0.f, 0.f, 0.f, 0.f};
    for (int oy = iy / 2; oy <= (iy + 1) / 2; ++oy) {
        if (oy >= p.Ho || 2 * oy - 1 > iy || 2 * oy + 1 < iy) continue;
        for (int ox = ix / 2; ox <= (ix + 1) / 2; ++ox) {
            if (ox >= p.Wo || 2 * ox - 1 > ix || 2 * ox + 1 < ix) continue;
            const size_t o = (((size_t)b * p.Ho + oy) * p.Wo + ox) * C4 + c4;
            const uint32_t w = idx[o];
            const int k = (iy - (2 * oy - 1)) * 3 + (ix - (2 * ox - 1));
            float4 g = md2::ld4T<T>(gy, 4 * o);
            if (gy2) {
                const float4 h = md2::ld4T<T>(gy2, 4 * o);
                g.x += h.x; g.y += h.y; g.z += h.z; g.w += h.w;
            }
            if ((int)(w & 255u) == k) s[0] += g.x;
            if ((int)((w >> 8) & 255u) == k) s[1] += g.y;
            if ((int)((w >> 16) & 255u) == k) s[2] += g.z;
            if ((int)(w >> 24) == k) s[3] += g.w;
        }
    }
    const size_t e = 4 * ((size_t)row * p.W * C4 + j);
    if (ga) {
        const float4 v = md2::ld4T<T>(ga, e);
        s[0] += v.x; s[1] += v.y; s[2] += v.z; s[3] += v.w;
    }
    md2::st4T<T>(gx, e, make_float4(s[0], s[1], s[2], s[3]));
}

template <typename T, int V>
__device__ __forceinline__ void ldV(const void* p, size_t off, float (&v)[V]) {
    if constexpr (V == 4) {
        const float4 q = md2::ld4T<T>(p, off);
        v[0] = q.x; v[1] = q.y; v[2] = q.z; v[3] = q.w;
    } else {
        static_assert(V == 8 && sizeof(T) == 2, "8 channels: bf16");
        const uint4 r = *(const uint4*)((const uint16_t*)p + off);
        const uint32_t w[4] = {r.x, r.y, r.z, r.w};
#pragma unroll
        for (int i = 0; i < 4; ++i) {
            v[2 * i] = md2::bf2f(w[i] & 0xffffu);
            v[2 * i + 1] = md2::bf2f(w[i] >> 16);
        }
    }
}
template <typename T, int V>
__device__ __forceinline__ void stV(void* p, size_t off, const float (&v)[V]) {
    if constexpr (V == 4) {
        md2::st4T<T>(p, off, make_float4(v[0], v[1], v[2], v[3]));
    } else {
        *(uint4*)((uint16_t*)p + off) =
            make_uint4(md2::f2bf(v[0]) | (md2::f2bf(v[1]) << 16), md2::f2bf(v[2]) | (md2::f2bf(v[3]) << 16),
                       md2::f2bf(v[4]) | (md2::f2bf(v[5]) << 16), md2::f2bf(v[6]) | (md2::f2bf(v[7]) << 16));
    }
}

template <typename T, int V>
__global__ void __launch_bounds__(kThreads) maxpool_fwd_rows_kernel(PoolArgs p, int cv_shift,
                                                                    const void* __restrict__ x,
                                                                    void* __restrict__ y, uint32_t* __restrict__ idx) {
    const int CV = p.C / V;
    const int j = blockIdx.x * kThreads + threadIdx.x;
    if (j >= p.Wo * CV) return;
    const int row = blockIdx.y, b = row / p.Ho, oy = row - b * p.Ho;
    const int c = V * (j & (CV - 1)), ox = j >> cv_shift;
    float m[V];
    int a[V];
    const int k0 = (oy == 0 ? 3 : 0) + (ox == 0 ? 1 : 0);
#pragma unroll
// ... 170 lines not shown
```

monodepth2_amd/csrc/stem.hip:

```cpp

#include <hip/hip_runtime.h>

#include <type_traits>

#include <stdint.h>

#include <algorithm>
#include <stdlib.h>

#include "md2hot.h"

int md2_report_error(int code, const char* msg);

namespace {

typedef float f32x16 __attribute__((ext_vector_type(16)));
typedef __bf16 bf16x8 __attribute__((ext_vector_type(8)));
typedef uint32_t u32x2 __attribute__((ext_vector_type(2)));
typedef uint32_t u32x4 __attribute__((ext_vector_type(4)));

constexpr int kCo = 64;
constexpr int kWaves = 7;
constexpr int kThreads = 64 * kWaves;
constexpr int kSeg = 32;
constexpr int kRawW = 2 * kSeg + 5;
constexpr int kCG = 3;
constexpr int kRP = 39;
constexpr int kRaw = 7 * kCG * 2 * kRP;
constexpr int kXBK = 32;
constexpr int kPA = kCo * kXBK;
constexpr int kPT = 32 * kXBK;
constexpr int kOut = 49 * kCG;
constexpr int kBlocksPerCU = 2;
constexpr int kMaxChunks = 64;

struct StemArgs {
    int B, C, H, W, Ho, Wo;
    int w_cl;
    int nseg, nchunks, splits, cps;
    const float* x;
    const float* gy;
    float* part;
    float* gw;
};

__device__ __forceinline__ float trunc16(float x) {
    return __builtin_bit_cast(float, __builtin_bit_cast(uint32_t, x) & 0xFFFF0000u);
}
__device__ __forceinline__ uint32_t hi16x2(float lo, float hi) {
    return __builtin_amdgcn_perm(__builtin_bit_cast(uint32_t, hi), __builtin_bit_cast(uint32_t, lo), 0x07060302u);
}
__device__ __forceinline__ uint16_t f2bf16(float v) {
    const uint32_t u = __builtin_bit_cast(uint32_t, v);
    if ((u & 0x7fffffffu) > 0x7f800000u) return (uint16_t)((u >> 16) | 0x40u);
    return (uint16_t)((u + 0x7fffu + ((u >> 16) & 1u)) >> 16);
}
__device__ __forceinline__ float bf16_rne(float v) { return __builtin_bit_cast(float, (uint32_t)f2bf16(v) << 16); }
__device__ __forceinline__ int xidx2(int r, int k) {
    r ^= (r >> 2) & 1;
    return r * kXBK + ((((k >> 3) ^ (r >> 2)) & 3) << 3) + (k & 7);
}
__device__ __forceinline__ int xcd_contiguous_block(int bid, int n) {
    const int q = n >> 3, r = n & 7;
    const int xcd = bid & 7, idx = bid >> 3;
    return xcd < r ? xcd * (q + 1) + idx : r * (q + 1) + (xcd - r) * q + idx;
}
__device__ __forceinline__ void lds_sync() { asm volatile("s_waitcnt lgkmcnt(0)\n\ts_barrier" ::: "memory"); }

template <int C>
__global__ __launch_bounds__(kThreads) __attribute__((amdgpu_waves_per_eu(4))) void stem_x6_wgrad_kernel(StemArgs a) {
    __shared__ float raw[2][kRaw];
    __shared__ __bf16 At[3 * kPA];
    __shared__ __bf16 Bt[7 * 3 * kPT];
    const int tid = threadIdx.x, lane = tid & 63, wid = tid >> 6;
    const int NG = a.C / kCG;
    const int j8 = blockIdx.x >> 3;
    const int cg = j8 % NG, ks = (j8 / NG) * 8 + (blockIdx.x & 7);
    if (ks >= a.splits) return;
    const int t0 = ks * a.cps;
    const int n = min(a.cps, a.nchunks - t0);
    const int H = a.H, W = a.W;
    constexpr int runq = (kRawW * C + 3) / 4;
    constexpr int nq = 7 * runq;
    constexpr int QPT = (nq + kThreads - 1) / kThreads;
    constexpr uint32_t cinv = (65536u + C - 1) / C;
    const long long total = (long long)a.B * H * W * C;

    struct Pos {
        int seg, oh, b;
    };
    auto pos_of = [&](int t) {
        Pos p;
        const int rr = t / a.nseg;
        p.seg = t - rr * a.nseg;
        p.b = rr / a.Ho;
        p.oh = rr - p.b * a.Ho;
        return p;
    };
    auto advance = [&](Pos& p) {
        if (++p.seg == a.nseg) {
            p.seg = 0;
            if (++p.oh == a.Ho) {
                p.oh = 0;
                ++p.b;
            }
        }
    };
    Pos praw = pos_of(t0), pgy = pos_of(t0);
    float4 RV[QPT];
    auto load_raw = [&]() {
        const int ih0 = 2 * praw.oh - 3, iw0 = 2 * praw.seg * kSeg - 3;
#pragma unroll
        for (int j = 0; j < QPT; ++j) {
            const int q = tid + kThreads * j;
            const int r = q / runq, k = 4 * (q - r * runq);
            const int ih = ih0 + r;
            RV[j] = make_float4(0.f, 0.f, 0.f, 0.f);
            if (q < nq && (unsigned)ih < (unsigned)H) {
                const long long e0 = ((long long)(praw.b * H + ih) * W + iw0) * C + k;
                const float* p = a.x + e0;
                if (e0 >= 0 && e0 + 4 <= total) {
                    RV[j] = *(const float4*)p;
                } else {
                    float v[4];
#pragma unroll
                    for (int i = 0; i < 4; ++i) v[i] = (e0 + i >= 0 && e0 + i < total) ? p[i] : 0.f;
                    RV[j] = make_float4(v[0], v[1], v[2], v[3]);
                }
            }
        }
    };
    auto store_raw = [&](float* dst) {
        const int iw0 = 2 * praw.seg * kSeg - 3;
#pragma unroll
        for (int j = 0; j < QPT; ++j) {
            const int q = tid + kThreads * j;
            if (q >= nq) break;
            const int r = q / runq, k0 = 4 * (q - r * runq);
            const float v[4] = {RV[j].x, RV[j].y, RV[j].z, RV[j].w};
#pragma unroll
            for (int i = 0; i < 4; ++i) {
                const int k = k0 + i, col = (int)(((uint32_t)k * cinv) >> 16), c = k - col * C - kCG * cg;
                const int iw = iw0 + col;
                if (col < kRawW && (unsigned)c < (unsigned)kCG)
                    dst[((r * kCG + c) * 2 + (col & 1)) * kRP + (col >> 1)] = (unsigned)iw < (unsigned)W ? v[i] : 0.f;
            }
        }
    };
    const int u = tid - 192, kq = u & 7, mq = u >> 3;
    const bool gyrole = u >= 0 && u < 128;
    float4 GV[4];
    auto load_gy = [&]() {
        if (!gyrole) return;
        const int ow0 = pgy.seg * kSeg + 4 * kq;
        const float* row = a.gy + (size_t)(pgy.b * a.Ho + pgy.oh) * a.Wo * kCo + 4 * mq;
#pragma unroll
        for (int i = 0; i < 4; ++i)
            GV[i] = ow0 + i < a.Wo ? *(const float4*)(row + (size_t)(ow0 + i) * kCo) : make_float4(0.f, 0.f, 0.f, 0.f);
    };
    auto store_gy = [&]() {
        if (!gyrole) return;
#pragma unroll
        for (int j = 0; j < 4; ++j) {
            float c[3][4];
#pragma unroll
            for (int i = 0; i < 4; ++i) {
                const float x = j == 0 ? GV[i].x : (j == 1 ? GV[i].y : (j == 2 ? GV[i].z : GV[i].w));
                const float a0 = trunc16(x), r1 = x - a0, a1 = trunc16(r1);
                c[0][i] = a0;
                c[1][i] = a1;
                c[2][i] = r1 - a1;
            }
#pragma unroll
            for (int pl = 0; pl < 3; ++pl) {
                u32x2 v;
                v.x = hi16x2(c[pl][0], c[pl][1]);
                v.y = hi16x2(c[pl][2], c[pl][3]);
                *(u32x2*)(At + pl * kPA + xidx2(4 * mq + j, 4 * kq)) = v;
            }
        }
    };
    constexpr int kLive = 7 * kCG;
    auto build = [&](const float* src) {
#pragma unroll 2
        for (int j = 0; j < (7 * kLive * 8 + kThreads - 1) / kThreads; ++j) {
            const int id = tid + kThreads * j;
            if (id >= 7 * kLive * 8) break;
            const int g = id & 7, rl = (id >> 3) % kLive, kh = (id >> 3) / kLive;
            const int kx = rl / kCG, ci = rl - kx * kCG, r = 4 * kx + ci;
            float v[4];
#pragma unroll
            for (int i = 0; i < 4; ++i) v[i] = src[((kh * kCG + ci) * 2 + (kx & 1)) * kRP + 4 * g + i + (kx >> 1)];
            float c[3][4];
#pragma unroll
            for (int i = 0; i < 4; ++i) {
                const float a0 = trunc16(v[i]), r1 = v[i] - a0, a1 = trunc16(r1);
                c[0][i] = a0;
                c[1][i] = a1;
                c[2][i] = r1 - a1;
            }
#pragma unroll
            for (int pl = 0; pl < 3; ++pl) {
                u32x2 q;
                q.x = hi16x2(c[pl][0], c[pl][1]);
                q.y = hi16x2(c[pl][2], c[pl][3]);
                *(u32x2*)(Bt + (kh * 3 + pl) * kPT + xidx2(r, 4 * g)) = q;
            }
        }
    };

    const int lr = lane & 31, h = lane >> 5;
    f32x16 acc[2];
#pragma unroll
    for (int i = 0; i < 2; ++i)
#pragma unroll
        for (int e = 0; e < 16; ++e) acc[i][e] = 0.f;
    auto mma = [&]() {
        const __bf16* LB = Bt + wid * 3 * kPT;
#pragma unroll
        for (int s = 0; s < kXBK / 16; ++s) {
            bf16x8 fb[3];
            const int eb = xidx2(lr, 16 * s + 8 * h);
#pragma unroll
            for (int pl = 0; pl < 3; ++pl) fb[pl] = *(const bf16x8*)(LB + pl * kPT + eb);
#pragma unroll
            for (int i = 0; i < 2; ++i) {
                bf16x8 fa[3];
                const int e = xidx2(32 * i + lr, 16 * s + 8 * h);
#pragma unroll
                for (int pl = 0; pl < 3; ++pl) fa[pl] = *(const bf16x8*)(At + pl * kPA + e);
                acc[i] = __builtin_amdgcn_mfma_f32_32x32x16_bf16(fa[2], fb[0], acc[i], 0, 0, 0);
                acc[i] = __builtin_amdgcn_mfma_f32_32x32x16_bf16(fa[1], fb[1], acc[i], 0, 0, 0);
                acc[i] = __builtin_amdgcn_mfma_f32_32x32x16_bf16(fa[0], fb[2], acc[i], 0, 0, 0);
                acc[i] = __builtin_amdgcn_mfma_f32_32x32x16_bf16(fa[1], fb[0], acc[i], 0, 0, 0);
                acc[i] = __builtin_amdgcn_mfma_f32_32x32x16_bf16(fa[0], fb[1], acc[i], 0, 0, 0);
                acc[i] = __builtin_amdgcn_mfma_f32_32x32x16_bf16(fa[0], fb[0], acc[i], 0, 0, 0);
            }
        }
    };

    for (int e = tid; e < 7 * 3 * 32 * 8; e += kThreads) {
        const int g = e & 7, r = (e >> 3) & 31, khp = e >> 8;
        if ((r >> 2) == 7 || (r & 3) == kCG) *(u32x2*)(Bt + khp * kPT + xidx2(r, 4 * g)) = u32x2{0u, 0u};
    }
    if (n > 0) {
        load_raw();
        load_gy();
        store_raw(raw[0]);
        advance(praw);
        if (n > 1) load_raw();
    }
    lds_sync();
    for (int t = 0; t < n; ++t) {
        build(raw[t & 1]);
        store_gy();
        if (t + 1 < n) {
            advance(pgy);
            load_gy();
        }
        lds_sync();
        mma();
        if (t + 1 < n) {
            store_raw(raw[(t + 1) & 1]);
            advance(praw);
            if (t + 2 < n) load_raw();
        }
        lds_sync();
    }

    const int kx = lr >> 2, ci = lr & 3;
    if (kx < 7 && ci < kCG) {
        float* out = a.part + (((size_t)cg * a.splits + ks) * kCo) * kOut + (wid * 7 + kx) * kCG + ci;
#pragma unroll
        for (int i = 0; i < 2; ++i)
#pragma unroll
            for (int e = 0; e < 16; ++e) {
                const int co = 32 * i + (e & 3) + 8 * (e >> 2) + 4 * h;
                out[(size_t)co * kOut] = acc[i][e];
            }
    }
}

constexpr int kTSeg = 64, kTWaves = 7, kTThreads = 64 * kTWaves;
constexpr int kTCols = 136;
__device__ __forceinline__ int tr_goff(int px, int co4) {
    const int sw = ((px >> 1) & 1) | (((px >> 3) & 1) << 1);
    return px * kCo + 4 * (co4 ^ (sw << 2));
}
typedef short s16x4 __attribute__((ext_vector_type(4)));
__device__ __forceinline__ bf16x8 tr_pair(const __bf16* lo, const __bf16* hi) {
    const s16x4 a = __builtin_amdgcn_ds_read_tr16_b64_v4i16((__attribute__((address_space(3))) s16x4*)lo);
    const s16x4 b = __builtin_amdgcn_ds_read_tr16_b64_v4i16((__attribute__((address_space(3))) s16x4*)hi);
    return __builtin_bit_cast(bf16x8, __builtin_shufflevector(a, b, 0, 1, 2, 3, 4, 5, 6, 7));
}
typedef float f32x4 __attribute__((ext_vector_type(4)));

template <int C, bool BF = false, bool PF = BF>
__global__ __launch_bounds__(kTThreads, 2) void stem_x6_wgrad_tr_kernel(StemArgs a) {
    constexpr int CP = C == 3 ? 4 : 6, NB = (7 * CP + 15) / 16;
    constexpr int XE = 7 * kTCols * CP, GE = kTSeg * kCo;
    constexpr int NPL = BF ? 1 : 3;
    __shared__ __attribute__((aligned(16))) __bf16 xs[NPL][XE];
    __shared__ __attribute__((aligned(16))) __bf16 gs[NPL][GE];
    const uint16_t* xh = (const uint16_t*)a.x;
    const uint16_t* gh = (const uint16_t*)a.gy;
    const int tid = threadIdx.x, lane = tid & 63, kh = tid >> 6;
    const int ks = blockIdx.x;
    const int t0 = ks * a.cps, n = min(a.cps, a.nchunks - t0);
    const int g16 = lane >> 4, q = (lane >> 2) & 3, p4 = lane & 3;
    f32x4 acc[4][NB];
#pragma unroll
    for (int mi = 0; mi < 4; ++mi)
#pragma unroll
        for (int ni = 0; ni < NB; ++ni) acc[mi][ni] = f32x4{0.f, 0.f, 0.f, 0.f};
    const int H = a.H, W = a.W;
    auto compute = [&]() {
#pragma unroll
        for (int kk = 0; kk < kTSeg / 32; ++kk) {
            const int px = 32 * kk + 8 * g16 + q;
            bf16x8 fb[NB][NPL];
#pragma unroll
            for (int ni = 0; ni < NB; ++ni) {
                const int n0 = 16 * ni + 4 * p4;
                const int olo = (kh * kTCols + 2 * px) * CP + n0;
                const int ohi = (kh * kTCols + 2 * (px + 4)) * CP + n0;
#pragma unroll
                for (int pl = 0; pl < NPL; ++pl) fb[ni][pl] = tr_pair(&xs[pl][olo], &xs[pl][ohi]);
            }
#pragma unroll
            for (int mi = 0; mi < 4; ++mi) {
                bf16x8 fa[NPL];
                const int glo = tr_goff(px, 4 * mi + p4), ghi = tr_goff(px + 4, 4 * mi + p4);
#pragma unroll
                for (int pl = 0; pl < NPL; ++pl) fa[pl] = tr_pair(&gs[pl][glo], &gs[pl][ghi]);
#pragma unroll
                for (int ni = 0; ni < NB; ++ni) {
                    if constexpr (BF) {
                        acc[mi][ni] = __builtin_amdgcn_mfma_f32_16x16x32_bf16(fa[0], fb[ni][0], acc[mi][ni], 0, 0, 0);
                        continue;
                    }
                    f32x4 c = acc[mi][ni];
                    c = __builtin_amdgcn_mfma_f32_16x16x32_bf16(fa[2], fb[ni][0], c, 0, 0, 0);
                    c = __builtin_amdgcn_mfma_f32_16x16x32_bf16(fa[1], fb[ni][1], c, 0, 0, 0);
                    c = __builtin_amdgcn_mfma_f32_16x16x32_bf16(fa[0], fb[ni][2], c, 0, 0, 0);
                    c = __builtin_amdgcn_mfma_f32_16x16x32_bf16(fa[1], fb[ni][0], c, 0, 0, 0);
                    c = __builtin_amdgcn_mfma_f32_16x16x32_bf16(fa[0], fb[ni][1], c, 0, 0, 0);
                    acc[mi][ni] = __builtin_amdgcn_mfma_f32_16x16x32_bf16(fa[0], fb[ni][0], c, 0, 0, 0);
                }
            }
        }
    };
    if constexpr (PF) {
        constexpr int NGT = kTSeg * 16, LG = (NGT + kTThreads - 1) / kTThreads;
        constexpr int NXT = CP == 4 ? 7 * (2 * kTSeg + 6) : 7 * ((2 * kTSeg + 6) * CP / 4);
        constexpr int LX = (NXT + kTThreads - 1) / kTThreads;
        using RT = typename std::conditional<BF, uint2, float4>::type;
        RT rg[LG], rx[LX];
        auto put3 = [&](__bf16* base, int stride, int o, float4 v) {
            const float e[4] = {v.x, v.y, v.z, v.w};
            float c[3][4];
#pragma unroll
            for (int j = 0; j < 4; ++j) {
                const float a0 = trunc16(e[j]), r1 = e[j] - a0, a1 = trunc16(r1);
                c[0][j] = a0;
                c[1][j] = a1;
                c[2][j] = r1 - a1;
            }
#pragma unroll
            for (int pl = 0; pl < 3; ++pl)
                *(u32x2*)(base + pl * stride + o) = u32x2{hi16x2(c[pl][0], c[pl][1]), hi16x2(c[pl][2], c[pl][3])};
        };
        auto fetch = [&](int tt) {
            const int per_img = a.nseg * a.Ho, b = tt / per_img, rem = tt - b * per_img;
            const int seg = rem / a.Ho, oh = rem - seg * a.Ho;
            const int ow0 = seg * kTSeg, iw0 = 2 * ow0 - 3;
#pragma unroll
            for (int k = 0; k < LG; ++k) {
                const int i = tid + k * kTThreads;
                const int px = i >> 4, co4 = i & 15, ow = ow0 + px;
                const size_t go = ((size_t)(b * a.Ho + oh) * a.Wo + ow) * kCo + 4 * co4;
                if constexpr (BF) rg[k] = (i < NGT && ow < a.Wo) ? *(const uint2*)(gh + go) : uint2{0u, 0u};
                else rg[k] = (i < NGT && ow < a.Wo) ? *(const float4*)(a.gy + go) : float4{0.f, 0.f, 0.f, 0.f};
            }
            if constexpr (BF) {
#pragma unroll
            for (int k = 0; k < LX; ++k) {
                const int e = tid + k * kTThreads;
                uint32_t h0 = 0u, h1 = 0u;
                if (e < NXT) {
                    if constexpr (CP == 4) {
                        const int r = e / (2 * kTSeg + 6), col = e - r * (2 * kTSeg + 6);
                        const int ih = 2 * oh - 3 + r, iw = iw0 + col;
                        if ((unsigned)ih < (unsigned)H && (unsigned)iw < (unsigned)W) {
                            const uint16_t* px = xh + ((size_t)(b * H + ih) * W + iw) * C;
                            uint32_t hh[4] = {0u, 0u, 0u, 0u};
#pragma unroll
                            for (int ci = 0; ci < C; ++ci) hh[ci] = px[ci];
                            h0 = hh[0] | (hh[1] << 16);
                            h1 = hh[2] | (hh[3] << 16);
                        }
                    } else {
                        constexpr int RQ = (2 * kTSeg + 6) * CP / 4;
                        const int r = e / RQ, kq = 4 * (e - r * RQ);
                        const int ih = 2 * oh - 3 + r;
                        if ((unsigned)ih < (unsigned)H) {
                            const long long f0 = (long long)iw0 * C + kq;
                            const uint16_t* row = xh + (size_t)(b * H + ih) * W * C;
                            if (f0 >= 0 && f0 + 4 <= (long long)W * C) {
                                h0 = *(const uint32_t*)(row + f0);
                                h1 = *(const uint32_t*)(row + f0 + 2);
                            } else {
                                uint32_t hh[2] = {0u, 0u};
#pragma unroll
                                for (int q2 = 0; q2 < 4; ++q2)
                                    if (f0 + q2 >= 0 && f0 + q2 < (long long)W * C)
                                        hh[q2 / 2] |= (uint32_t)row[f0 + q2] << (16 * (q2 & 1));
                                h0 = hh[0];
                                h1 = hh[1];
                            }
                        }
                    }
                }
                rx[k] = uint2{h0, h1};
            }
            } else {
#pragma unroll
            for (int k = 0; k < LX; ++k) {
                const int e = tid + k * kTThreads;
                float v[4] = {0.f, 0.f, 0.f, 0.f};
                if (e < NXT) {
                    if constexpr (CP == 4) {
                        const int r = e / (2 * kTSeg + 6), col = e - r * (2 * kTSeg + 6);
                        const int ih = 2 * oh - 3 + r, iw = iw0 + col;
                        if ((unsigned)ih < (unsigned)H && (unsigned)iw < (unsigned)W) {
                            const float* px = a.x + ((size_t)(b * H + ih) * W + iw) * C;
#pragma unroll
                            for (int ci = 0; ci < C; ++ci) v[ci] = px[ci];
                        }
                    } else {
                        constexpr int RQ = (2 * kTSeg + 6) * CP / 4;
                        const int r = e / RQ, kq = 4 * (e - r * RQ);
                        const int ih = 2 * oh - 3 + r;
                        if ((unsigned)ih < (unsigned)H) {
                            const long long f0 = (long long)iw0 * C + kq;
                            const float* row = a.x + (size_t)(b * H + ih) * W * C;
                            if (f0 >= 0 && f0 + 4 <= (long long)W * C) {
                                const float4 q4 = *(const float4*)(row + f0);
                                v[0] = q4.x; v[1] = q4.y; v[2] = q4.z; v[3] = q4.w;
                            } else {
#pragma unroll
                                for (int q2 = 0; q2 < 4; ++q2)
                                    if (f0 + q2 >= 0 && f0 + q2 < (long long)W * C) v[q2] = row[f0 + q2];
                            }
                        }
                    }
                }
                rx[k] = float4{v[0], v[1], v[2], v[3]};
            }
            }
        };
        if (n > 0) fetch(t0);
        for (int t = 0; t < n; ++t) {
#pragma unroll
            for (int k = 0; k < LG; ++k) {
                const int i = tid + k * kTThreads;
                if (NGT % kTThreads && i >= NGT) break;
                if constexpr (BF) *(u32x2*)&gs[0][tr_goff(i >> 4, i & 15)] = u32x2{rg[k].x, rg[k].y};
                else put3(&gs[0][0], GE, tr_goff(i >> 4, i & 15), rg[k]);
            }
#pragma unroll
            for (int k = 0; k < LX; ++k) {
                const int e = tid + k * kTThreads;
                if (NXT % kTThreads && e >= NXT) break;
                int o;
                if constexpr (CP == 4) {
                    const int r = e / (2 * kTSeg + 6), col = e - r * (2 * kTSeg + 6);
                    o = (r * kTCols + col) * CP;
                } else {
                    constexpr int RQ = (2 * kTSeg + 6) * CP / 4;
                    const int r = e / RQ;
                    o = r * kTCols * CP + 4 * (e - r * RQ);
                }
                if constexpr (BF) *(u32x2*)&xs[0][o] = u32x2{rx[k].x, rx[k].y};
                else put3(&xs[0][0], XE, o, rx[k]);
            }
            __syncthreads();
            if (t + 1 < n) fetch(t0 + t + 1);
            compute();
            __syncthreads();
        }
    } else {
    for (int t = 0; t < n; ++t) {
        const int tt = t0 + t, per_img = a.nseg * a.Ho, b = tt / per_img, rem = tt - b * per_img;
        const int seg = rem / a.Ho, oh = rem - seg * a.Ho;
        const int ow0 = seg * kTSeg, iw0 = 2 * ow0 - 3;
        for (int i = tid; i < kTSeg * 16; i += kTThreads) {
            const int px = i >> 4, co4 = i & 15, ow = ow0 + px;
            if constexpr (BF) {
                uint2 v = {0u, 0u};
                if (ow < a.Wo) v = *(const uint2*)(gh + ((size_t)(b * a.Ho + oh) * a.Wo + ow) * kCo + 4 * co4);
                *(u32x2*)&gs[0][tr_goff(px, co4)] = u32x2{v.x, v.y};
                continue;
            }
            float4 v = {0.f, 0.f, 0.f, 0.f};
            if (ow < a.Wo) v = *(const float4*)(a.gy + ((size_t)(b * a.Ho + oh) * a.Wo + ow) * kCo + 4 * co4);
            const float e[4] = {v.x, v.y, v.z, v.w};
            float c[3][4];
#pragma unroll
            for (int j = 0; j < 4; ++j) {
                const float a0 = trunc16(e[j]), r1 = e[j] - a0, a1 = trunc16(r1);
                c[0][j] = a0;
                c[1][j] = a1;
                c[2][j] = r1 - a1;
            }
            const int o = tr_goff(px, co4);
#pragma unroll
            for (int pl = 0; pl < NPL; ++pl) *(u32x2*)&gs[pl][o] = u32x2{hi16x2(c[pl][0], c[pl][1]), hi16x2(c[pl][2], c[pl][3])};
        }
        if constexpr (CP == 4) {
            for (int e = tid; e < 7 * (2 * kTSeg + 6); e += kTThreads) {
                const int r = e / (2 * kTSeg + 6), col = e - r * (2 * kTSeg + 6);
                const int ih = 2 * oh - 3 + r, iw = iw0 + col;
                if constexpr (BF) {
                    uint32_t h[4] = {0u, 0u, 0u, 0u};
                    if ((unsigned)ih < (unsigned)H && (unsigned)iw < (unsigned)W) {
                        const uint16_t* px = xh + ((size_t)(b * H + ih) * W + iw) * C;
#pragma unroll
                        for (int ci = 0; ci < C; ++ci) h[ci] = px[ci];
                    }
                    *(u32x2*)&xs[0][(r * kTCols + col) * CP] = u32x2{h[0] | (h[1] << 16), h[2] | (h[3] << 16)};
                    continue;
                }
                float v[4] = {0.f, 0.f, 0.f, 0.f};
                if ((unsigned)ih < (unsigned)H && (unsigned)iw < (unsigned)W) {
                    const float* px = a.x + ((size_t)(b * H + ih) * W + iw) * C;
#pragma unroll
                    for (int ci = 0; ci < C; ++ci) v[ci] = px[ci];
                }
                const int o = (r * kTCols + col) * CP;
                u32x2 pk[3];
#pragma unroll
                for (int j = 0; j < 4; j += 2) {
                    const float a0 = trunc16(v[j]), r0 = v[j] - a0, m0 = trunc16(r0);
                    const float a1 = trunc16(v[j + 1]), r1 = v[j + 1] - a1, m1 = trunc16(r1);
                    pk[0][j / 2] = hi16x2(a0, a1);
                    pk[1][j / 2] = hi16x2(m0, m1);
                    pk[2][j / 2] = hi16x2(r0 - m0, r1 - m1);
                }
#pragma unroll
                for (int pl = 0; pl < NPL; ++pl) *(u32x2*)&xs[pl][o] = pk[pl];
            }
        } else {
            constexpr int RQ = (2 * kTSeg + 6) * CP / 4;
            for (int e = tid; e < 7 * RQ; e += kTThreads) {
                const int r = e / RQ, k = 4 * (e - r * RQ);
                const int ih = 2 * oh - 3 + r;
                if constexpr (BF) {
                    uint32_t h[2] = {0u, 0u};
                    if ((unsigned)ih < (unsigned)H) {
                        const long long f0 = (long long)iw0 * C + k;
                        const uint16_t* row = xh + (size_t)(b * H + ih) * W * C;
                        if (f0 >= 0 && f0 + 4 <= (long long)W * C) {
                            h[0] = *(const uint32_t*)(row + f0);
                            h[1] = *(const uint32_t*)(row + f0 + 2);
                        } else {
#pragma unroll
                            for (int i = 0; i < 4; ++i)
                                if (f0 + i >= 0 && f0 + i < (long long)W * C) h[i / 2] |= (uint32_t)row[f0 + i] << (16 * (i & 1));
                        }
                    }
                    *(u32x2*)&xs[0][r * kTCols * CP + k] = u32x2{h[0], h[1]};
                    continue;
                }
                float v[4] = {0.f, 0.f, 0.f, 0.f};
                if ((unsigned)ih < (unsigned)H) {
                    const long long f0 = (long long)iw0 * C + k;
                    const float* row = a.x + (size_t)(b * H + ih) * W * C;
                    if (f0 >= 0 && f0 + 4 <= (long long)W * C) {
                        const float4 q4 = *(const float4*)(row + f0);
                        v[0] = q4.x; v[1] = q4.y; v[2] = q4.z; v[3] = q4.w;
                    } else {
#pragma unroll
                        for (int i = 0; i < 4; ++i)
                            if (f0 + i >= 0 && f0 + i < (long long)W * C) v[i] = row[f0 + i];
                    }
                }
                const int o = r * kTCols * CP + k;
                u32x2 pk[3];
#pragma unroll
                for (int j = 0; j < 4; j += 2) {
                    const float a0 = trunc16(v[j]), r0 = v[j] - a0, m0 = trunc16(r0);
                    const float a1 = trunc16(v[j + 1]), r1 = v[j + 1] - a1, m1 = trunc16(r1);
                    pk[0][j / 2] = hi16x2(a0, a1);
                    pk[1][j / 2] = hi16x2(m0, m1);
                    pk[2][j / 2] = hi16x2(r0 - m0, r1 - m1);
                }
#pragma unroll
                for (int pl = 0; pl < NPL; ++pl) *(u32x2*)&xs[pl][o] = pk[pl];
            }
        }
        __syncthreads();
#pragma unroll
        for (int kk = 0; kk < kTSeg / 32; ++kk) {
            const int px = 32 * kk + 8 * g16 + q;
            bf16x8 fb[NB][NPL];
#pragma unroll
            for (int ni = 0; ni < NB; ++ni) {
                const int n0 = 16 * ni + 4 * p4;
                const int olo = (kh * kTCols + 2 * px) * CP + n0;
                const int ohi = (kh * kTCols + 2 * (px + 4)) * CP + n0;
#pragma unroll
                for (int pl = 0; pl < NPL; ++pl) fb[ni][pl] = tr_pair(&xs[pl][olo], &xs[pl][ohi]);
            }
#pragma unroll
            for (int mi = 0; mi < 4; ++mi) {
                bf16x8 fa[NPL];
                const int glo = tr_goff(px, 4 * mi + p4), ghi = tr_goff(px + 4, 4 * mi + p4);
#pragma unroll
                for (int pl = 0; pl < NPL; ++pl) fa[pl] = tr_pair(&gs[pl][glo], &gs[pl][ghi]);
#pragma unroll
                for (int ni = 0; ni < NB; ++ni) {
                    if constexpr (BF) {
                        acc[mi][ni] = __builtin_amdgcn_mfma_f32_16x16x32_bf16(fa[0], fb[ni][0], acc[mi][ni], 0, 0, 0);
                        continue;
                    }
                    f32x4 c = acc[mi][ni];
                    c = __builtin_amdgcn_mfma_f32_16x16x32_bf16(fa[2], fb[ni][0], c, 0, 0, 0);
                    c = __builtin_amdgcn_mfma_f32_16x16x32_bf16(fa[1], fb[ni][1], c, 0, 0, 0);
                    c = __builtin_amdgcn_mfma_f32_16x16x32_bf16(fa[0], fb[ni][2], c, 0, 0, 0);
                    c = __builtin_amdgcn_mfma_f32_16x16x32_bf16(fa[1], fb[ni][0], c, 0, 0, 0);
                    c = __builtin_amdgcn_mfma_f32_16x16x32_bf16(fa[0], fb[ni][1], c, 0, 0, 0);
                    acc[mi][ni] = __builtin_amdgcn_mfma_f32_16x16x32_bf16(fa[0], fb[ni][0], c, 0, 0, 0);
                }
            }
        }
        __syncthreads();
    }
    }
#pragma unroll
    for (int ni = 0; ni < NB; ++ni) {
        const int nn = 16 * ni + (lane & 15), kw = nn / CP, ci = nn - kw * CP;
        if (kw >= 7 || ci >= C) continue;
        const int cg = ci / kCG, cl = ci - cg * kCG;
        float* out = a.part + ((size_t)cg * a.splits + ks) * kCo * kOut + (kh * 7 + kw) * kCG + cl;
#pragma unroll
        for (int mi = 0; mi < 4; ++mi)
#pragma unroll
            for (int e = 0; e < 4; ++e) out[(size_t)(16 * mi + 4 * g16 + e) * kOut] = acc[mi][ni][e];
    }
}

constexpr int kFinOut = 16, kFinLanes = 256 / kFinOut;
__global__ __launch_bounds__(256) void stem_wgrad_final_kernel(StemArgs a) {
    const int NG = a.C / kCG, outs = NG * kCo * kOut;
    const int el = threadIdx.x % kFinOut, sl = threadIdx.x / kFinOut;
    const int e = blockIdx.x * kFinOut + el;
    float s = 0.f;
    if (e < outs) {
// ... 131 lines not shown
#pragma unroll
    for (int q = 0; q < kPD && q < NQ; ++q) load(q, raw[q]);
#pragma unroll
    for (int q = 0; q < NQ; ++q) {
        if (q + kPD < NQ) load(q + kPD, raw[(q + kPD) % (kPD + 1)]);
        const float (&cur)[2][8] = raw[q % (kPD + 1)];
        bf16x8 fa[2][3];
#pragma unroll
        for (int p = 0; p < 2; ++p) {
            uint32_t pk[3][4];
#pragma unroll
            for (int i = 0; i < 8; i += 2) {
                const float x0 = cur[p][i], x1 = cur[p][i + 1];
                const float a0 = trunc16(x0), r0 = x0 - a0, m0 = trunc16(r0);
                const float a1 = trunc16(x1), r1 = x1 - a1, m1 = trunc16(r1);
                pk[0][i / 2] = hi16x2(a0, a1);
                pk[1][i / 2] = hi16x2(m0, m1);
                pk[2][i / 2] = hi16x2(r0 - m0, r1 - m1);
            }
#pragma unroll
            for (int pl = 0; pl < 3; ++pl)
                fa[p][pl] = __builtin_bit_cast(bf16x8, u32x4{pk[pl][0], pk[pl][1], pk[pl][2], pk[pl][3]});
        }
#pragma unroll
        for (int j = 0; j < 2; ++j) {
            bf16x8 fb[3];
#pragma unroll
            for (int pl = 0; pl < 3; ++pl) fb[pl] = __builtin_bit_cast(bf16x8, wf[((q * 2 + j) * 3 + pl) * 64 + lane]);
#pragma unroll
            for (int p = 0; p < 2; ++p) {
                acc[p][j] = __builtin_amdgcn_mfma_f32_32x32x16_bf16(fa[p][2], fb[0], acc[p][j], 0, 0, 0);
                acc[p][j] = __builtin_amdgcn_mfma_f32_32x32x16_bf16(fa[p][1], fb[1], acc[p][j], 0, 0, 0);
                acc[p][j] = __builtin_amdgcn_mfma_f32_32x32x16_bf16(fa[p][0], fb[2], acc[p][j], 0, 0, 0);
                acc[p][j] = __builtin_amdgcn_mfma_f32_32x32x16_bf16(fa[p][1], fb[0], acc[p][j], 0, 0, 0);
                acc[p][j] = __builtin_amdgcn_mfma_f32_32x32x16_bf16(fa[p][0], fb[1], acc[p][j], 0, 0, 0);
                acc[p][j] = __builtin_amdgcn_mfma_f32_32x32x16_bf16(fa[p][0], fb[0], acc[p][j], 0, 0, 0);
            }
        }
    }
    float* yrow = a.y + (size_t)(b * a.Ho + oh) * a.Wo * kCo;
#pragma unroll
    for (int p = 0; p < 2; ++p)
#pragma unroll
        for (int e = 0; e < 16; ++e) {
            const int ow = ow0 + 32 * p + (e & 3) + 8 * (e >> 2) + 4 * h;
            if (!EDGE || ow < a.Wo) {
#pragma unroll
                for (int j = 0; j < 2; ++j) yrow[(size_t)ow * kCo + 32 * j + lr] = acc[p][j][e];
            }
        }
}

template <int C, bool BF = false>
__global__ __launch_bounds__(64 * kFwdWaves, 1) void stem_x6_fwd_kernel(StemFwdArgs a) {
    constexpr int KP = (7 * C + 15) / 16 * 16, S = KP / 16;
    constexpr int NQ = 7 * S;
    constexpr int NPL = BF ? 1 : 3;
    __shared__ u32x4 wf[NQ * 2 * NPL * 64];
    const int tid = threadIdx.x, lane = tid & 63, wid = tid >> 6;
#pragma unroll
    for (int id = tid; id < NQ * 2 * 64; id += 64 * kFwdWaves) {
        const int l = id & 63, j = (id >> 6) & 1, q = id >> 7;
        const int kh = q / S, s = q - kh * S;
        const int co = 32 * j + (l & 31), k0 = 16 * s + 8 * (l >> 5);
        float c[3][8];
#pragma unroll
        for (int i = 0; i < 8; ++i) {
            const int k = k0 + i, kw = k / C, ci = k - kw * C;
            float v = 0.f;
            if (k < 7 * C)
                v = a.w_cl ? a.w[((co * 7 + kh) * 7 + kw) * C + ci] : a.w[((co * C + ci) * 7 + kh) * 7 + kw];
            if constexpr (BF) v = bf16_rne(v);
            const float a0 = trunc16(v), r1 = v - a0, a1 = trunc16(r1);
            c[0][i] = a0;
            c[1][i] = a1;
            c[2][i] = r1 - a1;
        }
#pragma unroll
        for (int pl = 0; pl < NPL; ++pl)
            wf[((q * 2 + j) * NPL + pl) * 64 + l] = u32x4{hi16x2(c[pl][0], c[pl][1]), hi16x2(c[pl][2], c[pl][3]),
                                                          hi16x2(c[pl][4], c[pl][5]), hi16x2(c[pl][6], c[pl][7])};
    }
    __syncthreads();

    const int bid = xcd_contiguous_block(blockIdx.x, gridDim.x);
    for (int t = bid * kFwdWaves + wid; t < a.tiles; t += gridDim.x * kFwdWaves) {
        const int rr = t / a.nseg, seg = t - rr * a.nseg, b = rr / a.Ho, oh = rr - b * a.Ho;
        const int ow0 = seg * kFwdSeg;
        constexpr int XTRA = (BF && (C & 1)) ? 1 : 0;
        const bool inner = 2 * oh - 3 >= 0 && 2 * oh + 3 < a.H && ow0 >= 2 &&
                           (2 * (ow0 + kFwdSeg - 1) - 3) * C + KP + XTRA <= a.W * C && ow0 + kFwdSeg <= a.Wo;
        if (inner) stem_fwd_tile<C, false, BF>(a, wf, b, oh, ow0, lane);
        else stem_fwd_tile<C, true, BF>(a, wf, b, oh, ow0, lane);
    }
}

bool valid(const md2_stem_desc* d) {
    return d && d->batch >= 1 && d->height >= 1 && d->width >= 1 &&
           (d->channels == 3 || d->channels == 6 || d->channels == 9) &&
           (long long)d->batch * d->height * d->width * d->channels < (1ll << 31);
}

StemArgs plan(const md2_stem_desc* d) {
    StemArgs a = {};
    a.B = d->batch;
    a.C = d->channels;
    a.H = d->height;
    a.W = d->width;
    a.Ho = (d->height - 1) / 2 + 1;
    a.Wo = (d->width - 1) / 2 + 1;
    a.w_cl = (d->flags & MD2_STEM_WEIGHT_CL) ? 1 : 0;
    a.nseg = (a.Wo + kSeg - 1) / kSeg;
    a.nchunks = a.B * a.Ho * a.nseg;
    const int NG = a.C / kCG;
    int want = 256 * kBlocksPerCU / NG;
    want = want < 1 ? 1 : want;
    const int need = (a.nchunks + kMaxChunks - 1) / kMaxChunks;
    want = want > need ? want : need;
    a.cps = (a.nchunks + want - 1) / want;
    a.splits = (a.nchunks + a.cps - 1) / a.cps;
    return a;
}

bool use_tr(const md2_stem_desc* d) {
    static const bool build = [] {
        const char* e = getenv("MD2_STEM_WGRAD_BUILD");
        return e && e[0] == '1';
    }();
    return !build && (d->channels == 3 || d->channels == 6);
}

StemArgs plan_tr(const md2_stem_desc* d) {
    StemArgs a = plan(d);
    a.nseg = (a.Wo + kTSeg - 1) / kTSeg;
    a.nchunks = a.B * a.Ho * a.nseg;
    int want = 256 * 2;
    const int need = (a.nchunks + 31) / 32;
    want = want > need ? want : need;
    a.cps = (a.nchunks + want - 1) / want;
    a.splits = (a.nchunks + a.cps - 1) / a.cps;
    return a;
}

}

extern "C" {

size_t md2_stem_wgrad_workspace_bytes(const md2_stem_desc* d) {
    if (!valid(d)) return 0;
    const StemArgs a = use_tr(d) ? plan_tr(d) : plan(d);
    return sizeof(float) * (size_t)(a.C / kCG) * a.splits * kCo * kOut;
}

int md2_stem_wgrad(const md2_stem_desc* d, const float* x, const float* grad_y, float* grad_weight, void* workspace,
                   void* stream) {
    if (!valid(d)) return md2_report_error(MD2_ERR_ARG, "stem_wgrad: channels 3/6/9, 32-bit element count");
    if (!x || !grad_y || !grad_weight || !workspace) return md2_report_error(MD2_ERR_ARG, "stem_wgrad: NULL operand");
    const bool tr = use_tr(d);
    if ((d->flags & MD2_STEM_BF16) && !tr)
        return md2_report_error(MD2_ERR_ARG, "stem_wgrad: bf16 operands (MD2_STEM_BF16) need channels 3 / 6");
    StemArgs a = tr ? plan_tr(d) : plan(d);
    a.x = x;
    a.gy = grad_y;
    a.part = (float*)workspace;
    a.gw = grad_weight;
    const int NG = a.C / kCG;
    const hipStream_t st = (hipStream_t)stream;
    if (tr) {
        const bool bf = (d->flags & MD2_STEM_BF16) != 0;
        static const bool pf32 = [] {
            const char* e = getenv("MD2_STEM_PF32");
            return e && e[0] == '1';
        }();
        void (*k)(StemArgs) =
            a.C == 3 ? (bf ? stem_x6_wgrad_tr_kernel<3, true>
                           : (pf32 ? stem_x6_wgrad_tr_kernel<3, false, true> : stem_x6_wgrad_tr_kernel<3>))
                     : (bf ? stem_x6_wgrad_tr_kernel<6, true>
                           : (pf32 ? stem_x6_wgrad_tr_kernel<6, false, true> : stem_x6_wgrad_tr_kernel<6>));
        hipLaunchKernelGGL(k, dim3(a.splits), dim3(kTThreads), 0, st, a);
    } else {
        void (*k)(StemArgs) =
            a.C == 3 ? stem_x6_wgrad_kernel<3> : a.C == 6 ? stem_x6_wgrad_kernel<6> : stem_x6_wgrad_kernel<9>;
        hipLaunchKernelGGL(k, dim3(NG * ((a.splits + 7) / 8) * 8), dim3(kThreads), 0, st, a);
    }
    const int outs = NG * kCo * kOut;
    hipLaunchKernelGGL(stem_wgrad_final_kernel, dim3((outs + kFinOut - 1) / kFinOut), dim3(256), 0, st, a);
    const hipError_t e = hipGetLastError();
    return e == hipSuccess ? MD2_OK : md2_report_error(MD2_ERR_HIP, hipGetErrorString(e));
}

int md2_stem_fwd(const md2_stem_desc* d, const float* x, const float* weight, float* y, void* stream) {
    if (!valid(d) || (d->channels != 3 && d->channels != 6))
        return md2_report_error(MD2_ERR_ARG, "stem_fwd: channels 3/6, 32-bit element count");
    if (!x || !weight || !y) return md2_report_error(MD2_ERR_ARG, "stem_fwd: NULL operand");
    StemFwdArgs a = {};
    a.B = d->batch;
    a.C = d->channels;
    a.H = d->height;
    a.W = d->width;
    a.Ho = (d->height - 1) / 2 + 1;
    a.Wo = (d->width - 1) / 2 + 1;
    a.w_cl = (d->flags & MD2_STEM_WEIGHT_CL) ? 1 : 0;
    a.nseg = (a.Wo + kFwdSeg - 1) / kFwdSeg;
    a.tiles = a.B * a.Ho * a.nseg;
    a.x = x;
    a.w = weight;
    a.y = y;
    const int blocks = std::min(256, (a.tiles + kFwdWaves - 1) / kFwdWaves);
    const bool bf = (d->flags & MD2_STEM_BF16) != 0;
    void (*k)(StemFwdArgs) = a.C == 3 ? (bf ? stem_x6_fwd_kernel<3, true> : stem_x6_fwd_kernel<3>)
                                      : (bf ? stem_x6_fwd_kernel<6, true> : stem_x6_fwd_kernel<6>);
    hipLaunchKernelGGL(k, dim3(blocks), dim3(64 * kFwdWaves), 0, (hipStream_t)stream, a);
    const hipError_t e = hipGetLastError();
    return e == hipSuccess ? MD2_OK : md2_report_error(MD2_ERR_HIP, hipGetErrorString(e));
}

}
```

monodepth2_amd/networks/resnet_encoder.py:

```python
from __future__ import annotations

import warnings

import numpy as np
import torch
import torch.nn as nn

from ..bn_ops import bn_act, max_pool_3x3s2, max_pool_3x3s2_with_alias
from ..conv_ops import conv2d
from ..stem_ops import stem_conv


def _conv3x3(cin, cout, stride=1):
    return nn.Conv2d(cin, cout, 3, stride=stride, padding=1, bias=False)


def _conv1x1(cin, cout, stride=1):
    return nn.Conv2d(cin, cout, 1, stride=stride, bias=False)


class BasicBlock(nn.Module):
    expansion = 1

    def __init__(self, inplanes, planes, stride=1, downsample=None):
        super().__init__()
        self.conv1 = _conv3x3(inplanes, planes, stride)
        self.bn1 = nn.BatchNorm2d(planes)
        self.relu = nn.ReLU(inplace=True)
        self.conv2 = _conv3x3(planes, planes)
        self.bn2 = nn.BatchNorm2d(planes)
        self.downsample = downsample
        self.stride = stride

    def forward(self, x):
        identity = x if self.downsample is None else _downsample(self.downsample, x)
        out = bn_act(self.bn1, self.conv1(x))
        return bn_act(self.bn2, self.conv2(out), residual=identity)


def _downsample(down: nn.Sequential, x):
    return bn_act(down[1], conv2d(down[0], x), relu=False)


class Bottleneck(nn.Module):
    expansion = 4

    def __init__(self, inplanes, planes, stride=1, downsample=None):
        super().__init__()
        self.conv1 = _conv1x1(inplanes, planes)
        self.bn1 = nn.BatchNorm2d(planes)
        self.conv2 = _conv3x3(planes, planes, stride)
        self.bn2 = nn.BatchNorm2d(planes)
        self.conv3 = _conv1x1(planes, planes * 4)
        self.bn3 = nn.BatchNorm2d(planes * 4)
        self.relu = nn.ReLU(inplace=True)
        self.downsample = downsample
        self.stride = stride

    def forward(self, x):
        identity = x if self.downsample is None else _downsample(self.downsample, x)
        out = bn_act(self.bn1, self.conv1(x))
        out = bn_act(self.bn2, self.conv2(out))
        return bn_act(self.bn3, self.conv3(out), residual=identity)


def _run_layer(layer: nn.Sequential, x, xs, skip_alias: bool):
    n = len(layer)
    skip = None
    for bi, blk in enumerate(layer):
        shortcut = xs if blk.downsample is None else _downsample(blk.downsample, xs)
        out = bn_act(blk.bn1, conv2d(blk.conv1, x))
        if isinstance(blk, Bottleneck):
            out = bn_act(blk.bn2, conv2d(blk.conv2, out))
            bn, conv = blk.bn3, blk.conv3
        else:
            bn, conv = blk.bn2, blk.conv2
        last = bi == n - 1
        k = (2 if skip_alias else 1) if last else 1
        res = bn_act(bn, conv2d(conv, out), residual=shortcut, aliases=k)
        x, xs = res[0], res[1]
        skip = res[2] if (last and skip_alias) else x
    return x, xs, skip


_SPECS = {18: (BasicBlock, [2, 2, 2, 2]), 34: (BasicBlock, [3, 4, 6, 3]), 50: (Bottleneck, [3, 4, 6, 3]),
          101: (Bottleneck, [3, 4, 23, 3]), 152: (Bottleneck, [3, 8, 36, 3])}


class ResNet(nn.Module):

    def __init__(self, num_layers=18, in_channels=3, num_classes=1000):
        super().__init__()
        block, counts = _SPECS[num_layers]
        self.inplanes = 64
        self.conv1 = nn.Conv2d(in_channels, 64, kernel_size=7, stride=2, padding=3, bias=False)
        self.bn1 = nn.BatchNorm2d(64)
        self.relu = nn.ReLU(inplace=True)
        self.maxpool = nn.MaxPool2d(kernel_size=3, stride=2, padding=1)
        self.layer1 = self._stage(block, 64, counts[0])
        self.layer2 = self._stage(block, 128, counts[1], stride=2)
        self.layer3 = self._stage(block, 256, counts[2], stride=2)
        self.layer4 = self._stage(block, 512, counts[3], stride=2)
        self.avgpool = nn.AdaptiveAvgPool2d((1, 1))
        self.fc = nn.Linear(512 * block.expansion, num_classes)
        for m in self.modules():
            if isinstance(m, nn.Conv2d):
                nn.init.kaiming_normal_(m.weight, mode="fan_out", nonlinearity="relu")
            elif isinstance(m, nn.BatchNorm2d):
                nn.init.constant_(m.weight, 1)
                nn.init.constant_(m.bias, 0)

    def _stage(self, block, planes, n, stride=1):
        down = None
        if stride != 1 or self.inplanes != planes * block.expansion:
            down = nn.Sequential(_conv1x1(self.inplanes, planes * block.expansion, stride),
                                 nn.BatchNorm2d(planes * block.expansion))
        blocks = [block(self.inplanes, planes, stride, down)]
        self.inplanes = planes * block.expansion
        blocks += [block(self.inplanes, planes) for _ in range(1, n)]
        return nn.Sequential(*blocks)


class ResnetEncoder(nn.Module):

    def __init__(self, num_layers, pretrained, num_input_images=1):
        super().__init__()
        if num_layers not in _SPECS:
            raise ValueError("{} is not a valid number of resnet layers".format(num_layers))
        if num_input_images > 1 and num_layers not in (18, 50):
            raise AssertionError("Can only run with 18 or 50 layer resnet")
        if pretrained:
            warnings.warn("ImageNet weights need network access and are unavailable offline; "
                          "using the random (scratch) initialisation instead")
        self.num_ch_enc = np.array([64, 64, 128, 256, 512])
        self.encoder = ResNet(num_layers, in_channels=3 * num_input_images)
        if num_layers > 34:
            self.num_ch_enc[1:] *= 4

    MEAN, STD = 0.45, 0.225

    def prepare(self, frames):
        groups = [[frames]] if torch.is_tensor(frames) else [list(p) for p in frames]
        f0 = groups[0][0]
        if (f0.is_cuda and f0.dtype == torch.float32 and f0.dim() == 4 and f0.shape[1] == 3
                and self.encoder.conv1.weight.is_contiguous(memory_format=torch.channels_last)
                and len(groups) * len(groups[0]) <= 8
                and all(t.shape == f0.shape and t.dtype == f0.dtype and t.is_contiguous() for g in groups for t in g)):
            import ctypes
            from .. import _lib
            B, _, H, W = f0.shape
            S = len(groups[0])
            out = torch.empty(len(groups) * B, 3 * S, H, W, device=f0.device, memory_format=torch.channels_last)
            src = (ctypes.c_void_p * (len(groups) * S))(*[t.data_ptr() for g in groups for t in g])
            rc = _lib.lib().md2_encoder_input(len(groups), B, S, H, W, src, self.MEAN, self.STD, out.data_ptr(),
                                              torch.cuda.current_stream(f0.device).cuda_stream)
            _lib.check(rc, "md2_encoder_input")
            return out
        x = torch.cat([torch.cat(g, 1) for g in groups], 0) if len(groups) * len(groups[0]) > 1 else f0
        x = (x - self.MEAN) / self.STD
        if self.encoder.conv1.weight.is_contiguous(memory_format=torch.channels_last):
            x = x.contiguous(memory_format=torch.channels_last)
        return x

    def forward(self, input_image):
        return self.forward_prepared(self.prepare(input_image))

    def forward_prepared(self, x):
        e = self.encoder
        f0 = bn_act(e.bn1, stem_conv(e.conv1, x))
        x, xs, f0 = max_pool_3x3s2_with_alias(e.maxpool, f0, out_alias=True)
        feats = [f0]
        layers = [e.layer1, e.layer2, e.layer3, e.layer4]
        for li, layer in enumerate(layers):
            x, xs, skip = _run_layer(layer, x, xs, skip_alias=li < len(layers) - 1)
            feats.append(skip)
        self.features = feats
        return self.features
```

monodepth2_amd/stem_ops.py:

```python
from __future__ import annotations

import ctypes
import os

import torch
import torch.nn as nn
import torch.nn.functional as F

from . import _lib

_CL = torch.channels_last
ENABLED = True
FWD_ENABLED = os.environ.get("MD2_STEM_FWD", "1") != "0"
BF16_ENABLED = os.environ.get("MD2_CONV_BF16", "1") != "0"


def _fwd(x: torch.Tensor, weight: torch.Tensor) -> torch.Tensor:
    B, C, H, W = x.shape
    if not (FWD_ENABLED and C in (3, 6)):
        return F.conv2d(x, weight, None, 2, 3)
    w_cl = weight.is_contiguous(memory_format=_CL)
    if not (w_cl or weight.is_contiguous()):
        weight = weight.contiguous()
    d = _lib.StemDesc(B, C, H, W, _lib.STEM_WEIGHT_CL if w_cl else 0)
    y = torch.empty((B, 64, (H - 1) // 2 + 1, (W - 1) // 2 + 1), device=x.device, dtype=torch.float32,
                    memory_format=_CL)
    rc = _lib.lib().md2_stem_fwd(ctypes.byref(d), x.data_ptr(), weight.data_ptr(), y.data_ptr(), _lib.stream(x.device))
    _lib.check(rc, "md2_stem_fwd")
    return y


def _fwd_bf16(xb: torch.Tensor, weight: torch.Tensor) -> torch.Tensor:
    B, C, H, W = xb.shape
    w_cl = weight.is_contiguous(memory_format=_CL)
    if not (w_cl or weight.is_contiguous()):
        weight = weight.contiguous()
    d = _lib.StemDesc(B, C, H, W, (_lib.STEM_WEIGHT_CL if w_cl else 0) | _lib.STEM_BF16)
    y = torch.empty((B, 64, (H - 1) // 2 + 1, (W - 1) // 2 + 1), device=xb.device, dtype=torch.bfloat16,
                    memory_format=_CL)
    _lib.check(_lib.lib().md2_stem_fwd(ctypes.byref(d), xb.data_ptr(), weight.data_ptr(), y.data_ptr(),
                                       _lib.stream(xb.device)), "md2_stem_fwd")
    return y


_FWD_BF16 = os.environ.get("MD2_STEM_FWD_BF16", "1") != "0"


class _StemConv(torch.autograd.Function):

    @staticmethod
    def forward(ctx, x, weight):
        ctx.save_for_backward(x)
        ctx.w_cl = weight.is_contiguous(memory_format=_CL)
        ctx.w_shape = weight.shape
        return _fwd(x, weight)

    @staticmethod
    def backward(ctx, gy):
        x, = ctx.saved_tensors
        gy = gy.contiguous(memory_format=_CL)
        B, C, H, W = x.shape
        d = _lib.StemDesc(B, C, H, W, _lib.STEM_WEIGHT_CL if ctx.w_cl else 0)
        gw = torch.empty(ctx.w_shape, device=x.device, dtype=torch.float32,
                         memory_format=_CL if ctx.w_cl else torch.contiguous_format)
        L = _lib.lib()
        ws = torch.empty(L.md2_stem_wgrad_workspace_bytes(ctypes.byref(d)), dtype=torch.uint8, device=x.device)
        rc = L.md2_stem_wgrad(ctypes.byref(d), x.data_ptr(), gy.data_ptr(), gw.data_ptr(), ws.data_ptr(),
                              _lib.stream(x.device))
        _lib.check(rc, "md2_stem_wgrad")
        return None, gw


_WGRAD_BF16 = os.environ.get("MD2_STEM_WGRAD_BF16", "1") != "0"


class _StemConvBF16(torch.autograd.Function):

    @staticmethod
    def forward(ctx, x, weight):
        xb = x.to(torch.bfloat16)
        ctx.save_for_backward(xb)
        ctx.w_cl = weight.is_contiguous(memory_format=_CL)
        ctx.w_shape = weight.shape
        if _FWD_BF16 and FWD_ENABLED and xb.shape[1] in (3, 6) and xb.is_contiguous(memory_format=_CL):
            return _fwd_bf16(xb, weight)
        with torch.autocast("cuda", enabled=False):
            return F.conv2d(xb, weight.to(torch.bfloat16), None, 2, 3)

    @staticmethod
    def backward(ctx, gy):
        xb, = ctx.saved_tensors
        B, C, H, W = xb.shape
        flags = _lib.STEM_WEIGHT_CL if ctx.w_cl else 0
        if C in (3, 6) and gy.dtype == torch.bfloat16 and _WGRAD_BF16:
            x = xb.contiguous(memory_format=_CL)
            gy = gy.contiguous(memory_format=_CL)
            flags |= _lib.STEM_BF16
        else:
            x = xb.float().contiguous(memory_format=_CL)
            gy = gy.float().contiguous(memory_format=_CL)
        d = _lib.StemDesc(B, C, H, W, flags)
        gw = torch.empty(ctx.w_shape, device=x.device, dtype=torch.float32,
                         memory_format=_CL if ctx.w_cl else torch.contiguous_format)
        L = _lib.lib()
        ws = torch.empty(L.md2_stem_wgrad_workspace_bytes(ctypes.byref(d)), dtype=torch.uint8, device=x.device)
        _lib.check(L.md2_stem_wgrad(ctypes.byref(d), x.data_ptr(), gy.data_ptr(), gw.data_ptr(), ws.data_ptr(),
                                    _lib.stream(x.device)), "md2_stem_wgrad")
        return None, gw.to(torch.bfloat16).to(torch.float32)


def supports_stem_bf16(conv: nn.Conv2d, x: torch.Tensor) -> bool:
    from .conv_ops import _bf16_autocast
    return (BF16_ENABLED and x.is_cuda and x.dtype == torch.float32 and conv.weight.dtype == torch.float32
            and not x.requires_grad and x.dim() == 4 and x.shape[1] in (3, 6, 9)
            and x.is_contiguous(memory_format=_CL) and conv.out_channels == 64
            and tuple(conv.kernel_size) == (7, 7) and tuple(conv.stride) == (2, 2) and tuple(conv.padding) == (3, 3)
            and tuple(conv.dilation) == (1, 1) and conv.groups == 1 and conv.bias is None
            and conv.padding_mode == "zeros" and _bf16_autocast() and x.numel() < 2 ** 31)


def supports_stem(conv: nn.Conv2d, x: torch.Tensor) -> bool:
    return (x.is_cuda and x.dtype == torch.float32 and conv.weight.dtype == torch.float32 and not x.requires_grad
            and x.dim() == 4 and x.shape[1] in (3, 6, 9) and x.is_contiguous(memory_format=_CL)
            and conv.out_channels == 64 and tuple(conv.kernel_size) == (7, 7) and tuple(conv.stride) == (2, 2)
            and tuple(conv.padding) == (3, 3) and tuple(conv.dilation) == (1, 1) and conv.groups == 1
            and conv.bias is None and conv.padding_mode == "zeros" and not torch.is_autocast_enabled()
            and x.numel() < 2 ** 31)


def stem_conv(conv: nn.Conv2d, x: torch.Tensor) -> torch.Tensor:
    if ENABLED and supports_stem(conv, x):
        if torch.is_grad_enabled() and conv.weight.requires_grad:
            return _StemConv.apply(x, conv.weight)
        return _fwd(x, conv.weight.detach())
    if ENABLED and torch.is_grad_enabled() and conv.weight.requires_grad and supports_stem_bf16(conv, x):
        return _StemConvBF16.apply(x, conv.weight)
    return conv(x)
```

monodepth2_amd/trainer.py:

```python
from __future__ import annotations

import json
import os
import time
from typing import Dict, Iterable, Optional

import numpy as np
import torch
import torch.distributed as dist
import torch.nn as nn
import torch.nn.functional as F
import torch.optim as optim

from . import conv_ops, networks
from .distributed import FlatGradSync, wrap_ddp
from .eval_ops import depth_metrics
from .hotpath import HotPathConfig, generate_images, photometric_loss, predictive_mask_inputs, selection_maps
from .bn_ops import bn_groups
from .layers import compute_depth_errors, disp_to_depth
from .optim import FusedAdam
from .pose_ops import packed_poses_to_transforms, poses_to_transforms


def _sec_to_hm_str(t):
# ... 99 lines not shown
                                                           num_input_features=1, num_frames_to_predict_for=2)
            elif self.opt.pose_model_type == "shared":
                self.models["pose"] = networks.PoseDecoder(self.models["encoder"].num_ch_enc, self.num_pose_frames)
            elif self.opt.pose_model_type == "posecnn":
                self.models["pose"] = networks.PoseCNN(
                    self.num_input_frames if self.opt.pose_model_input == "all" else 2)
        if self.opt.predictive_mask:
            self.models["predictive_mask"] = networks.DepthDecoder(
                self.models["encoder"].num_ch_enc, self.opt.scales,
                num_output_channels=(len(self.opt.frame_ids) - 1))
        for m in self.models.values():
            m.to(self.device)
            if getattr(self.opt, "channels_last", False):
                m.to(memory_format=torch.channels_last)
        self.nets = _Networks(self.models)
        self.parameters_to_train = [p for m in self.models.values() for p in m.parameters()]
        self._bn_layers, self._bn_mult = [], []
        pairs = sum(1 for f in self.opt.frame_ids[1:] if f != "s")
        for name, m in self.nets.named_modules():
            if isinstance(m, nn.modules.batchnorm._BatchNorm) and m.momentum is not None \
                    and m.num_batches_tracked is not None:
                self._bn_layers.append(m)
                self._bn_mult.append(pairs if (name.startswith("models.pose_encoder.")
                                               and self.num_pose_frames == 2) else 1)
                m.num_batches_tracked = None
        self._bn_steps = 0
        self.batch_pose_pairs = True
        self._pose_stream = (torch.cuda.Stream(self.device)
                             if self.device.type == "cuda" and getattr(self.opt, "pose_streams", 1) else None)
        self._in_step = False

        self.use_graph = bool(getattr(self.opt, "hip_graph", False))
        if (self.use_graph and self.device.type == "cuda" and self._pose_stream is None
                and os.environ.get("MD2_ALLOW_ONESTREAM_GRAPH", "0") != "1"):
            raise ValueError("--hip_graph needs the pose network on its own stream (--pose_streams 1)")
        sync = getattr(self.opt, "grad_sync", "auto")
        if sync == "auto":
            sync = "flat" if self.use_graph else "ddp"
        if self.use_graph and sync == "ddp" and world_size > 1:
            raise ValueError("--hip_graph needs --grad_sync flat (DDP hooks are not graph-capturable)")
        streams = ([torch.cuda.current_stream(self.device), self._pose_stream]
                   if self._pose_stream is not None else None)
        self.ddp = wrap_ddp(self.nets, self.device, streams) if (world_size > 1 and sync == "ddp") else None
        explicit_flat = getattr(self.opt, "grad_sync", "auto") == "flat"
        self.flat_sync = FlatGradSync(self.nets.named_parameters(), world_size) \
            if ((world_size > 1 and (sync == "flat" or self.use_graph)) or explicit_flat) else None
        self.graph = None
        self.seed_tensor = None
        self._choices_agreed = False

        if self.device.type == "cuda":
            self.model_optimizer = FusedAdam(self.parameters_to_train, self.opt.learning_rate,
                                             capturable=self.use_graph)
            if (self.use_graph and world_size == 1 and self.flat_sync is None and self._pose_stream is not None
                    and self.use_pose_net and self.opt.pose_model_type == "separate_resnet"
                    and os.environ.get("MD2_ADAM_SPLIT", "1") != "0"):
                pose_params = [p for n in ("pose_encoder", "pose") if n in self.models
                               for p in self.models[n].parameters()]
                self.model_optimizer.split = (self._pose_stream, pose_params)
        else:
            self.model_optimizer = optim.Adam(self.parameters_to_train, self.opt.learning_rate)
        self._adam_split = getattr(self.model_optimizer, "split", None) is not None
        self.model_lr_scheduler = optim.lr_scheduler.StepLR(self.model_optimizer, self.opt.scheduler_step_size, 0.1)
        if self.opt.load_weights_folder is not None:
            self.load_model()

        self.src_frames = list(self.opt.frame_ids[1:])
        self.hot = HotPathConfig(
            batch=self.opt.batch_size, height=self.opt.height, width=self.opt.width,
            num_src=len(self.src_frames), num_scales=self.num_scales, min_depth=self.opt.min_depth,
            max_depth=self.opt.max_depth, disparity_smoothness=self.opt.disparity_smoothness,
            no_ssim=self.opt.no_ssim, avg_reprojection=self.opt.avg_reprojection,
            disable_automasking=self.opt.disable_automasking, v1_multiscale=self.opt.v1_multiscale,
            t_per_scale=self.opt.pose_model_type == "posecnn", predictive_mask=bool(self.opt.predictive_mask))
        self.noise_override = None
        self.depth_metric_names = ["de/abs_rel", "de/sq_rel", "de/rms", "de/log_rms", "da/a1", "da/a2", "da/a3"]
        self.epoch = 0
        self.step = 0

    def set_train(self):
        for m in self.models.values():
            m.train()

    def set_eval(self):
        for m in self.models.values():
            m.eval()

    def _run_networks(self, models, inputs):
        amp = getattr(self.opt, "amp", "none") == "bf16"
        with torch.autocast("cuda", dtype=torch.bfloat16, enabled=amp and self.device.type == "cuda"):
            outputs = self._networks_body(models, inputs)
        if amp:
            outputs = _to_fp32(outputs)
        return outputs

    def _networks_body(self, models, inputs):
        side = self._pose_stream if (self.use_pose_net and self.opt.pose_model_type != "shared") else None
        main = torch.cuda.current_stream(self.device) if side is not None else None
        pose_out = None
        pose_last = side is not None and (getattr(self, "pose_last", False) or _POSE_LAST)
        inputs_ready = None
        if pose_last:
            inputs_ready = torch.cuda.Event()
            inputs_ready.record(main)
        if side is not None and not pose_last:
            side.wait_stream(main)
            with torch.cuda.stream(side):
                pose_out = self.predict_poses(inputs, None, models)
        if self.opt.pose_model_type == "shared":
            all_color_aug = torch.cat([inputs[("color_aug", i, 0)] for i in self.opt.frame_ids])
            all_features = models["encoder"](all_color_aug)
            all_features = [torch.split(f, self.opt.batch_size) for f in all_features]
            features = {k: [f[i] for f in all_features] for i, k in enumerate(self.opt.frame_ids)}
            outputs = models["depth"](features[0])
        else:
            features = models["encoder"](inputs["color_aug", 0, 0])
            outputs = models["depth"](features)
        if self.opt.predictive_mask:
            outputs["predictive_mask"] = models["predictive_mask"](
                features[0] if isinstance(features, dict) else features)
        if pose_last:
            side.wait_event(inputs_ready)
            with torch.cuda.stream(side):
                pose_out = self.predict_poses(inputs, None, models)
        if self.use_pose_net:
            if side is not None:
                main.wait_stream(side)
                for v in pose_out.values():
                    v.record_stream(main)
            else:
                pose_out = self.predict_poses(inputs, features, models)
            outputs.update(pose_out)
        return outputs

    def predict_poses(self, inputs, features, models=None):
        models = models if models is not None else self.models
        outputs = {}
        aas, trs, invs, fids = [], [], [], []
        packed = None
        if self.num_pose_frames == 2:
            if self.opt.pose_model_type == "shared":
                pose_feats = {f_i: features[f_i] for f_i in self.opt.frame_ids}
            else:
                pose_feats = {f_i: inputs["color_aug", f_i, 0] for f_i in self.opt.frame_ids}
            temporal = [f_i for f_i in self.opt.frame_ids[1:] if f_i != "s"]
            pairs = [[pose_feats[f_i], pose_feats[0]] if f_i < 0 else [pose_feats[0], pose_feats[f_i]]
                     for f_i in temporal]
            if (self.opt.pose_model_type == "separate_resnet" and len(temporal) > 1 and self.device.type == "cuda"
                    and self.batch_pose_pairs):
                B = self.opt.batch_size
                enc = models["pose_encoder"]
                x = enc.prepare(pairs)
                with bn_groups(len(temporal)):
                    feats = enc.forward_prepared(x)
                dec = getattr(models["pose"], "module", models["pose"])
                dec.packed_output = True
                try:
                    x6 = models["pose"]([feats])
                finally:
                    dec.packed_output = False
                axisangle_all, translation_all = x6[..., :3], x6[..., 3:]
                per_pair = [(axisangle_all[i * B:(i + 1) * B], translation_all[i * B:(i + 1) * B])
                            for i in range(len(temporal))]
                if x6.dtype == torch.float32:
                    packed = x6[:, 0, 0].view(len(temporal), B, 6)
            else:
                per_pair = []
                for pair in pairs:
                    if self.opt.pose_model_type == "separate_resnet":
                        pair = [models["pose_encoder"](torch.cat(pair, 1))]
                    elif self.opt.pose_model_type == "posecnn":
                        pair = torch.cat(pair, 1)
                    per_pair.append(models["pose"](pair))
            for f_i, (axisangle, translation) in zip(temporal, per_pair):
                outputs[("axisangle", 0, f_i)] = axisangle
                outputs[("translation", 0, f_i)] = translation
                aas.append(axisangle[:, 0, 0])
                trs.append(translation[:, 0, 0])
                invs.append(f_i < 0)
                fids.append(f_i)
        else:
            if self.opt.pose_model_type in ["separate_resnet", "posecnn"]:
                pose_inputs = torch.cat([inputs[("color_aug", i, 0)] for i in self.opt.frame_ids if i != "s"], 1)
                if self.opt.pose_model_type == "separate_resnet":
                    pose_inputs = [models["pose_encoder"](pose_inputs)]
            else:
                pose_inputs = [features[i] for i in self.opt.frame_ids if i != "s"]
            axisangle, translation = models["pose"](pose_inputs)
            for i, f_i in enumerate(self.opt.frame_ids[1:]):
                if f_i != "s":
                    outputs[("axisangle", 0, f_i)] = axisangle
                    outputs[("translation", 0, f_i)] = translation
                    aas.append(axisangle[:, i, 0])
                    trs.append(translation[:, i, 0])
                    invs.append(False)
                    fids.append(f_i)
        self._T_all = None
        if fids:
            if packed is not None:
                T = packed_poses_to_transforms(packed, invs)
            else:
                T = poses_to_transforms(torch.stack(aas).float(), torch.stack(trs).float(), invs)
            for i, f_i in enumerate(fids):
                outputs[("cam_T_cam", 0, f_i)] = T[i]
            self._T_all = (T, tuple(fids))
        return outputs

    def _colors(self, inputs):
        cols = []
        for s in range(self.num_scales):
            row = [inputs[("color", 0, s)]]
            for f in self.src_frames:
                row.append(inputs.get(("color", f, s)) if (self.opt.v1_multiscale or s == 0) else None)
            cols.append(row)
        return cols

    def _intrinsics(self, inputs):
        K = [inputs[("K", s)] for s in range(self.num_scales)]
        inv_K = [inputs[("inv_K", s)] for s in range(self.num_scales)]
        return K, inv_K

    def _stacked_T(self, inputs, outputs):
        if self.opt.pose_model_type != "posecnn":
            Ts = [inputs["stereo_T"] if f == "s" else outputs[("cam_T_cam", 0, f)] for f in self.src_frames]
            T_all = getattr(self, "_T_all", None)
            if (T_all is not None and T_all[1] == tuple(self.src_frames)
                    and all(t._base is T_all[0] and t.storage_offset() == i * T_all[0].stride(0)
                            for i, t in enumerate(Ts))):
                return T_all[0]
            return torch.stack(Ts, 0)
        temporal = [f for f in self.src_frames if f != "s"]
        return posecnn_transforms([outputs[("disp", s)] for s in range(self.num_scales)],
                                  torch.stack([outputs[("axisangle", 0, f)][:, 0, 0] for f in temporal]),
                                  torch.stack([outputs[("translation", 0, f)][:, 0, 0] for f in temporal]),
                                  self.src_frames, inputs.get("stereo_T"), self.opt.height, self.opt.width,
                                  self.opt.min_depth, self.opt.max_depth, self.opt.v1_multiscale)

    def generate_images_pred(self, inputs, outputs):
        K, inv_K = self._intrinsics(inputs)
        with torch.no_grad():
            T = self._stacked_T(inputs, outputs)
            if self.hot.t_per_scale:
                T = T[0]
                cfg = HotPathConfig(**{**self.hot.__dict__, "t_per_scale": False})
            else:
                cfg = self.hot
            res = generate_images(cfg, [outputs[("disp", s)].detach() for s in range(self.num_scales)],
                                  self._colors(inputs), K, inv_K, T.detach())
        for s in range(self.num_scales):
            outputs[("depth", 0, s)] = res["depth"][s]
            src_s = s if self.opt.v1_multiscale else 0
            for fi, f in enumerate(self.src_frames):
                outputs[("sample", f, s)] = res["sample"][(fi, s)]
                outputs[("color", f, s)] = res["color"][(fi, s)]
                if not self.opt.disable_automasking:
                    outputs[("color_identity", f, s)] = inputs[("color", f, src_s)]

    def compute_losses(self, inputs, outputs):
        K, inv_K = self._intrinsics(inputs)
        T = self._stacked_T(inputs, outputs)
        if self.seed_tensor is not None:
            seed = int(self.opt.noise_seed) * 1000003 * 131 + self.rank
        else:
            seed = (int(self.opt.noise_seed) * 1000003 + self.step) * 131 + self.rank
        mask, bce = None, None
        if self.hot.predictive_mask:
            mask, bce = predictive_mask_inputs(self.hot, {s: outputs["predictive_mask"][("disp", s)]
                                                          for s in range(self.num_scales)})
        loss_vec, sel = photometric_loss(self.hot, [outputs[("disp", s)] for s in range(self.num_scales)],
                                         self._colors(inputs), K, inv_K, T, noise=self.noise_override,
                                         seed=seed, seed_tensor=self.seed_tensor, mask=mask,
                                         src8=inputs.get("color_src8"))
        if bce is not None:
            loss_vec = loss_vec + torch.cat([bce, bce.mean().view(1)])
        losses = {"loss/{}".format(s): loss_vec[s] for s in range(self.num_scales)}
        losses["loss"] = loss_vec[self.num_scales]
        if not self.opt.disable_automasking:
            C = self.hot.noise_channels()
            side = (self._pose_stream if (self._in_step and self.use_pose_net and _LOGMAPS_SIDE) else None)
            if side is not None:
                main = torch.cuda.current_stream(self.device)
                side.wait_stream(main)
                with torch.cuda.stream(side):
                    maps = selection_maps(self.hot, sel.gt(C - 1).float())
                sel.record_stream(side)
                for m in maps.values():
                    m.record_stream(main)
            else:
                maps = selection_maps(self.hot, sel.gt(C - 1).float())
            for s, m in maps.items():
                outputs["identity_selection/{}".format(s)] = m
        return losses

    def process_batch(self, inputs):
        for key, ipt in inputs.items():
            if ipt.device != self.device:
                inputs[key] = ipt.to(self.device, non_blocking=True)
        nets = self.ddp if self.ddp is not None else self.nets
        outputs = nets(self, inputs)
        if self.opt.materialize_images:
            self.generate_images_pred(inputs, outputs)
        losses = self.compute_losses(inputs, outputs)
        return outputs, losses

    def _step_body(self, inputs):
        bank = self.device.type == "cuda" and conv_ops.PLANE_BANK
        if bank:
# ... 205 lines not shown
```

Baseline: 1076 images/s.

## Fuse stem BN+ReLU+maxpool forward and BN backward into stem weight-gradient

Adds a fused kernel that applies batch-norm, ReLU and 3x3/2 max-pool in one pass over the stem conv output. It can skip writing the full-resolution activation when it is not needed, as in the pose encoder. In backward, it computes only the BN reduction and folds the BN input-gradient into the stem weight-gradient kernel, so the full-resolution grad_z tensor is never materialised. Together these cut several full-resolution memory passes and kernel launches. The cost is more complex custom kernels and a fallback path, which bring a risk of numerical or tie-break differences.

```diff
diff --git a/include/md2hot.h b/include/md2hot.h
--- a/include/md2hot.h
+++ b/include/md2hot.h
@@ -115,6 +115,7 @@
 
 #define MD2_STEM_WEIGHT_CL (1u << 0)
 #define MD2_STEM_BF16 (1u << 1)
+#define MD2_STEM_PREFETCH (1u << 2)
 
 typedef struct md2_stem_desc {
     int32_t batch, channels, height, width;
@@ -358,6 +359,20 @@
 int md2_disp_colorize(const md2_viz_desc* desc, const float* disp, uint8_t* rgb, float* resized, float* stats,
                       void* workspace, void* stream);
 
+int md2_bn_pool_fwd_supported(const md2_bn_desc* desc, int height, int width);
+int md2_bn_pool_fwd(const md2_bn_desc* desc, int height, int width, const float* x, const float* gamma,
+                    const float* beta, float* running_mean, float* running_var, float* y, uint8_t* relu_mask,
+                    float* pooled, uint32_t* idx, float* save_mean, float* save_invstd, void* workspace,
+                    void* stream);
+int md2_bn_bwd_reduce_mask(const md2_bn_desc* desc, const void* x, const uint8_t* relu_mask, const void* grad_y,
+                           const float* gamma, const float* save_mean, const float* save_invstd, float* grad_gamma,
+                           float* grad_beta, void* workspace, void* stream);
+size_t md2_bn_coef_offset(const md2_bn_desc* desc);
+int md2_stem_wgrad_bn_supported(const md2_stem_desc* desc);
+int md2_stem_wgrad_bn(const md2_stem_desc* desc, const float* x, const float* grad, const float* z,
+                      const uint8_t* relu_mask, const float* save_mean, const float* coef, int bn_groups,
+                      float* grad_weight, void* workspace, void* stream);
+
 #ifdef __cplusplus
 }
 #endif
diff --git a/monodepth2_amd/_lib.py b/monodepth2_amd/_lib.py
--- a/monodepth2_amd/_lib.py
+++ b/monodepth2_amd/_lib.py
@@ -65,7 +65,9 @@
            "md2_depth_eval", "md2_depth_eval_workspace_bytes",
            "md2_velo_project", "md2_velo_project_workspace_bytes",
            "md2_pose_ate", "md2_pose_ate_workspace_bytes",
-           "md2_disp_colorize", "md2_disp_colorize_workspace_bytes"]
+           "md2_disp_colorize", "md2_disp_colorize_workspace_bytes",
+           "md2_bn_pool_fwd_supported", "md2_bn_pool_fwd", "md2_bn_bwd_reduce_mask", "md2_bn_coef_offset",
+           "md2_stem_wgrad_bn_supported", "md2_stem_wgrad_bn"]
 
 DTYPE_F32 = 0
 DTYPE_BF16 = 1
@@ -147,6 +149,7 @@
 
 STEM_WEIGHT_CL = 1 << 0
 STEM_BF16 = 1 << 1
+STEM_PREFETCH = 1 << 2
 
 
 class StemDesc(ctypes.Structure):
@@ -200,6 +203,18 @@
 
 
 def _declare(L):
+    L.md2_bn_pool_fwd_supported.restype = ctypes.c_int
+    L.md2_bn_pool_fwd_supported.argtypes = [ctypes.POINTER(BnDesc), ctypes.c_int, ctypes.c_int]
+    L.md2_bn_pool_fwd.restype = ctypes.c_int
+    L.md2_bn_pool_fwd.argtypes = [ctypes.POINTER(BnDesc), ctypes.c_int, ctypes.c_int] + [_vp] * 13
+    L.md2_bn_bwd_reduce_mask.restype = ctypes.c_int
+    L.md2_bn_bwd_reduce_mask.argtypes = [ctypes.POINTER(BnDesc)] + [_vp] * 10
+    L.md2_bn_coef_offset.restype = ctypes.c_size_t
+    L.md2_bn_coef_offset.argtypes = [ctypes.POINTER(BnDesc)]
+    L.md2_stem_wgrad_bn_supported.restype = ctypes.c_int
+    L.md2_stem_wgrad_bn_supported.argtypes = [ctypes.POINTER(StemDesc)]
+    L.md2_stem_wgrad_bn.restype = ctypes.c_int
+    L.md2_stem_wgrad_bn.argtypes = [ctypes.POINTER(StemDesc)] + [_vp] * 6 + [ctypes.c_int] + [_vp] * 3
     L.md2_disp_colorize_workspace_bytes.restype = ctypes.c_size_t
     L.md2_disp_colorize_workspace_bytes.argtypes = [ctypes.POINTER(VizDesc)]
     L.md2_disp_colorize.restype = ctypes.c_int
diff --git a/monodepth2_amd/bn_ops.py b/monodepth2_amd/bn_ops.py
--- a/monodepth2_amd/bn_ops.py
+++ b/monodepth2_amd/bn_ops.py
@@ -194,11 +194,14 @@
         return gx, None, None
 
 
+def _pool_geometry_ok(pool: nn.MaxPool2d) -> bool:
+    return (pool.kernel_size in (3, (3, 3)) and pool.stride in (2, (2, 2)) and pool.padding in (1, (1, 1))
+            and pool.dilation in (1, (1, 1)) and not pool.ceil_mode and not pool.return_indices)
+
+
 def _pool_ok(pool: nn.MaxPool2d, x: torch.Tensor) -> bool:
     return (ENABLED and x.is_cuda and x.dim() == 4 and x.dtype in (torch.float32, torch.bfloat16)
-            and x.shape[1] % 4 == 0 and x.is_contiguous(memory_format=_CL)
-            and pool.kernel_size in (3, (3, 3)) and pool.stride in (2, (2, 2)) and pool.padding in (1, (1, 1))
-            and pool.dilation in (1, (1, 1)) and not pool.ceil_mode and not pool.return_indices)
+            and x.shape[1] % 4 == 0 and x.is_contiguous(memory_format=_CL) and _pool_geometry_ok(pool))
 
 
 def max_pool_3x3s2(pool: nn.MaxPool2d, x: torch.Tensor) -> torch.Tensor:
diff --git a/monodepth2_amd/build.py b/monodepth2_amd/build.py
--- a/monodepth2_amd/build.py
+++ b/monodepth2_amd/build.py
@@ -12,6 +12,7 @@
 LIB_NAME = "libmd2hot.so"
 LIB_PATH = os.path.join(CSRC, LIB_NAME)
 SOURCES = ["md2hot.hip", "decoder.hip", "pose.hip", "augment.hip", "bnorm.hip", "pool.hip", "adam.hip", "disphead.hip", "stem.hip", "bias_act.hip", "conv.hip", "direct.hip", "glue.hip", "eval.hip", "velo.hip", "traj.hip", "viz.hip"]
+HEADERS = [os.path.join(INCLUDE, "md2hot.h"), os.path.join(CSRC, "md2_bf16.h"), os.path.join(CSRC, "md2_bn_expr.h")]
 ARCH = os.environ.get("MD2_OFFLOAD_ARCH", "gfx950")
 
 
@@ -26,8 +27,7 @@
     if not os.path.exists(LIB_PATH):
         return True
     t = os.path.getmtime(LIB_PATH)
-    deps = [os.path.join(CSRC, s) for s in SOURCES] + [os.path.join(INCLUDE, "md2hot.h"),
-                                                       os.path.join(CSRC, "md2_bf16.h")]
+    deps = [os.path.join(CSRC, s) for s in SOURCES] + HEADERS
     if any(os.path.getmtime(d) > t for d in deps):
         return True
     return built_id(LIB_PATH) != source_hash()
@@ -58,8 +58,7 @@
 
 def source_hash() -> str:
     h = hashlib.sha256()
-    for path in [os.path.join(CSRC, s) for s in SOURCES] + [os.path.join(INCLUDE, "md2hot.h"),
-                                                          os.path.join(CSRC, "md2_bf16.h")]:
+    for path in [os.path.join(CSRC, s) for s in SOURCES] + HEADERS:
         h.update(os.path.basename(path).encode())
         with open(path, "rb") as f:
             h.update(f.read())
diff --git a/monodepth2_amd/csrc/bnorm.hip b/monodepth2_amd/csrc/bnorm.hip
--- a/monodepth2_amd/csrc/bnorm.hip
+++ b/monodepth2_amd/csrc/bnorm.hip
@@ -5,6 +5,7 @@
 #include <stdlib.h>
 
 #include "md2_bf16.h"
+#include "md2_bn_expr.h"
 #include "md2hot.h"
 
 int md2_report_error(int code, const char* msg);
@@ -183,18 +184,12 @@
         const int c = 4 * (j & (Q - 1));
         const float4 v = ldT<T>(x, 4 * i), mu = ld4(mug + c), is = ld4(isg + c), ga = ld4(gamma + c),
                      be = ld4(beta + c);
-        float4 o;
-        o.x = (v.x - mu.x) * is.x * ga.x + be.x;
-        o.y = (v.y - mu.y) * is.y * ga.y + be.y;
-        o.z = (v.z - mu.z) * is.z * ga.z + be.z;
-        o.w = (v.w - mu.w) * is.w * ga.w + be.w;
+        float4 o = md2::bn_affine4(v, mu, is, ga, be);
         if (RES) {
             const float4 rv = ldT<T>(r, 4 * i);
             o.x += rv.x; o.y += rv.y; o.z += rv.z; o.w += rv.w;
         }
-        if (RELU) {
-            o.x = fmaxf(o.x, 0.f); o.y = fmaxf(o.y, 0.f); o.z = fmaxf(o.z, 0.f); o.w = fmaxf(o.w, 0.f);
-        }
+        if (RELU) o = md2::relu4(o);
         stT<T>(y, 4 * i, o);
         if (MOUT)
             mask[i] = (uint8_t)((stored_pos<T>(o.x) ? 1 : 0) | (stored_pos<T>(o.y) ? 2 : 0) |
@@ -205,8 +200,7 @@
 template <typename T, bool MIN>
 __device__ __forceinline__ float4 relu_gate(const void* y, size_t off, float4 g) {
     if constexpr (MIN) {
-        const uint32_t m = ((const uint8_t*)y)[off >> 2];
-        g.x = (m & 1) ? g.x : 0.f; g.y = (m & 2) ? g.y : 0.f; g.z = (m & 4) ? g.z : 0.f; g.w = (m & 8) ? g.w : 0.f;
+        g = md2::relu_gate_mask4(y, off, g);
     } else {
         const float4 yv = ldT<T>(y, off);
         g.x = yv.x > 0.f ? g.x : 0.f; g.y = yv.y > 0.f ? g.y : 0.f;
@@ -317,11 +311,7 @@
         if (RELU) gv = relu_gate<T, MIN>(y, 4 * i, gv);
         const float4 v = ldT<T>(x, 4 * i), mu = ld4(smean + c), k1 = ld4(coef + c),
                      k2 = ld4(coef + (size_t)NG * C + c), k3 = ld4(coef + 2 * (size_t)NG * C + c);
-        float4 o;
-        o.x = k1.x * (gv.x - k2.x - (v.x - mu.x) * k3.x);
-        o.y = k1.y * (gv.y - k2.y - (v.y - mu.y) * k3.y);
-        o.z = k1.z * (gv.z - k2.z - (v.z - mu.z) * k3.z);
-        o.w = k1.w * (gv.w - k2.w - (v.w - mu.w) * k3.w);
+        const float4 o = md2::bn_bwd_dx4(gv, v, mu, k1, k2, k3);
         stT<T>(dx, 4 * i, o);
         if (RES) stT<T>(dr, 4 * i, gv);
     }
@@ -571,10 +561,61 @@
     return Q >= kThreads ? (Q % kThreads == 0) : (kThreads % Q == 0);
 }
 
+struct StemPoolGeom {
+    int B, H, W, Ho, Wo;
+    int ipg;
+};
+
+template <bool YOUT>
+__global__ void __launch_bounds__(kThreads) bn_relu_pool_kernel(StemPoolGeom p, int q_shift,
+                                                                const float* __restrict__ z,
+                                                                const float* __restrict__ gamma,
+                                                                const float* __restrict__ beta,
+                                                                const float* __restrict__ smean,
+                                                                const float* __restrict__ sinvstd,
+                                                                float* __restrict__ y, uint8_t* __restrict__ mask,
+                                                                float* __restrict__ pooled,
+                                                                uint32_t* __restrict__ idx) {
+    const int Q = 1 << q_shift, C = 4 * Q;
+    const int j = blockIdx.x * kThreads + threadIdx.x;
+    if (j >= p.Wo * Q) return;
+    const int row = blockIdx.y, b = row / p.Ho, oy = row - b * p.Ho;
+    const int c = 4 * (j & (Q - 1)), ox = j >> q_shift;
+    const int gc = (b / p.ipg) * C + c;
+    const float4 mu = ld4(smean + gc), is = ld4(sinvstd + gc), ga = ld4(gamma + c), be = ld4(beta + c);
+    float m[4] = {-INFINITY, -INFINITY, -INFINITY, -INFINITY};
+    const int k0 = (oy == 0 ? 3 : 0) + (ox == 0 ? 1 : 0);
+    int a[4] = {k0, k0, k0, k0};
+#pragma unroll
+    for (int ky = 0; ky < 3; ++ky) {
+        const int iy = 2 * oy - 1 + ky;
+        if (iy < 0 || iy >= p.H) continue;
+#pragma unroll
+        for (int kx = 0; kx < 3; ++kx) {
+            const int ix = 2 * ox - 1 + kx;
+            if (ix < 0 || ix >= p.W) continue;
+            const size_t e = (((size_t)b * p.H + iy) * p.W + ix) * C + c;
+            const float4 o = md2::relu4(md2::bn_affine4(ld4(z + e), mu, is, ga, be));
+            const int k = ky * 3 + kx;
+            md2::pool_take(o.x, k, m[0], a[0]);
+            md2::pool_take(o.y, k, m[1], a[1]);
+            md2::pool_take(o.z, k, m[2], a[2]);
+            md2::pool_take(o.w, k, m[3], a[3]);
+            if (ky >= 1 && kx >= 1) {
+                if (YOUT) st4(y + e, o);
+                mask[e >> 2] = (uint8_t)((stored_pos<float>(o.x) ? 1 : 0) | (stored_pos<float>(o.y) ? 2 : 0) |
+                                         (stored_pos<float>(o.z) ? 4 : 0) | (stored_pos<float>(o.w) ? 8 : 0));
+            }
+        }
+    }
+    const size_t o = (((size_t)b * p.Ho + oy) * p.Wo + ox) * C + c;
+    st4(pooled + o, make_float4(m[0], m[1], m[2], m[3]));
+    idx[o >> 2] = (uint32_t)a[0] | ((uint32_t)a[1] << 8) | ((uint32_t)a[2] << 16) | ((uint32_t)a[3] << 24);
+}
+
 template <typename T>
-void launch_fwd(const md2_bn_desc* d, const void* x, const float* gamma, const float* beta, const void* residual,
-                float* running_mean, float* running_var, void* y, float* save_mean, float* save_invstd,
-                void* workspace, hipStream_t st, uint8_t* mask = nullptr) {
+void launch_stats(const md2_bn_desc* d, const void* x, float* running_mean, float* running_var, float* save_mean,
+                  float* save_invstd, void* workspace, hipStream_t st) {
     const int NG = groups_of(d);
     const long long P = d->pixels / NG;
     const int C = d->channels, G = blocks_for_stats(P, C);
@@ -584,6 +625,16 @@
         hipLaunchKernelGGL(bn_stats_kernel<T>, dim3(G, NG), dim3(kThreads), 0, st, x, P, C, G, workspace);
     hipLaunchKernelGGL(bn_stats_final_kernel, dim3(C), dim3(kThreads), 0, st, P, C, G, NG, d->eps, d->momentum,
                        running_mean, running_var, save_mean, save_invstd, workspace);
+}
+
+template <typename T>
+void launch_fwd(const md2_bn_desc* d, const void* x, const float* gamma, const float* beta, const void* residual,
+                float* running_mean, float* running_var, void* y, float* save_mean, float* save_invstd,
+                void* workspace, hipStream_t st, uint8_t* mask = nullptr) {
+    const int NG = groups_of(d);
+    const long long P = d->pixels / NG;
+    const int C = d->channels;
+    launch_stats<T>(d, x, running_mean, running_var, save_mean, save_invstd, workspace, st);
     const int n4g = (int)(P * C / 4);
     const bool relu = d->flags & MD2_BN_RELU, res = d->flags & MD2_BN_RESIDUAL;
     if (sizeof(T) == 2 && C % 8 == 0 && apply8_on()) {
@@ -602,14 +653,13 @@
 }
 
 template <typename T>
-void launch_bwd(const md2_bn_desc* d, const void* x, const void* y, const void* grad_y, const void* grad_y2,
-                const void* grad_y3, const float* gamma,
-                const float* save_mean, const float* save_invstd, void* grad_x, void* grad_residual,
-                float* grad_gamma, float* grad_beta, void* workspace, hipStream_t st, bool mask_in = false) {
+void launch_bwd_reduce(const md2_bn_desc* d, const void* x, const void* y, const void* grad_y, const void* grad_y2,
+                       const void* grad_y3, const float* gamma, const float* save_mean, const float* save_invstd,
+                       float* grad_gamma, float* grad_beta, void* workspace, hipStream_t st, bool mask_in) {
     const int NG = groups_of(d);
     const long long P = d->pixels / NG;
     const int C = d->channels, G = blocks_for_stats(P, C);
-    const bool relu = d->flags & MD2_BN_RELU, res = d->flags & MD2_BN_RESIDUAL;
+    const bool relu = d->flags & MD2_BN_RELU;
     auto red = relu ? (mask_in ? bn_bwd_reduce_kernel<T, true, true> : bn_bwd_reduce_kernel<T, true>)
                     : bn_bwd_reduce_kernel<T, false>;
     if (sizeof(T) == 2 && C % 8 == 0 && C <= 8 * kThreads && reduce8_on())
@@ -619,6 +669,19 @@
                        workspace);
     hipLaunchKernelGGL(bn_bwd_final_kernel, dim3(C), dim3(kThreads), 0, st, P, C, G, NG, gamma, save_invstd,
                        grad_gamma, grad_beta, workspace);
+}
+
+template <typename T>
+void launch_bwd(const md2_bn_desc* d, const void* x, const void* y, const void* grad_y, const void* grad_y2,
+                const void* grad_y3, const float* gamma,
+                const float* save_mean, const float* save_invstd, void* grad_x, void* grad_residual,
+                float* grad_gamma, float* grad_beta, void* workspace, hipStream_t st, bool mask_in = false) {
+    const int NG = groups_of(d);
+    const long long P = d->pixels / NG;
+    const int C = d->channels, G = blocks_for_stats(P, C);
+    const bool relu = d->flags & MD2_BN_RELU, res = d->flags & MD2_BN_RESIDUAL;
+    launch_bwd_reduce<T>(d, x, y, grad_y, grad_y2, grad_y3, gamma, save_mean, save_invstd, grad_gamma, grad_beta,
+                         workspace, st, mask_in);
     const int n4g = (int)(P * C / 4);
     const float* coef = work(workspace, G, C, NG).coef;
     if (sizeof(T) == 2 && C % 8 == 0 && apply8_on()) {
@@ -709,6 +772,76 @@
                        grad_residual, grad_gamma, grad_beta, workspace, stream);
 }
 
+static bool stem_pool_geom(const md2_bn_desc* d, int height, int width, StemPoolGeom& p) {
+    if (!valid(d) || (d->flags & (MD2_BN_RELU | MD2_BN_RESIDUAL | MD2_BN_BF16)) != MD2_BN_RELU) return false;
+    if (height < 2 || width < 2 || (height & 1) || (width & 1)) return false;
+    const long long hw = (long long)height * width;
+    if (d->pixels % hw) return false;
+    const long long B = d->pixels / hw;
+    const int NG = groups_of(d);
+    if (B % NG || B * (height / 2) > 65535) return false;
+    p.B = (int)B;
+    p.H = height;
+    p.W = width;
+    p.Ho = height / 2;
+    p.Wo = width / 2;
+    p.ipg = (int)(B / NG);
+    return true;
+}
+
+int md2_bn_pool_fwd_supported(const md2_bn_desc* d, int height, int width) {
+    StemPoolGeom p;
+    return stem_pool_geom(d, height, width, p) ? 1 : 0;
+}
+
+int md2_bn_pool_fwd(const md2_bn_desc* d, int height, int width, const float* x, const float* gamma,
+                    const float* beta, float* running_mean, float* running_var, float* y, uint8_t* relu_mask,
+                    float* pooled, uint32_t* idx, float* save_mean, float* save_invstd, void* workspace,
+                    void* stream) {
+    StemPoolGeom p;
+    if (!stem_pool_geom(d, height, width, p))
+        return md2_report_error(MD2_ERR_ARG, "bn_pool_fwd: fp32, MD2_BN_RELU alone, even height and width, "
+                                             "batch * height / 2 <= 65535");
+    if (!x || !gamma || !beta || !relu_mask || !pooled || !idx || !save_mean || !save_invstd || !workspace ||
+        (!running_mean != !running_var))
+        return md2_report_error(MD2_ERR_ARG, "bn_pool_fwd: NULL operand");
+    const hipStream_t st = (hipStream_t)stream;
+    launch_stats<float>(d, x, running_mean, running_var, save_mean, save_invstd, workspace, st);
+    const int Q = d->channels / 4;
+    int sh = 0;
+    while ((1 << sh) < Q) ++sh;
+    auto k = y ? bn_relu_pool_kernel<true> : bn_relu_pool_kernel<false>;
+    hipLaunchKernelGGL(k, dim3((p.Wo * Q + kThreads - 1) / kThreads, p.B * p.Ho), dim3(kThreads), 0, st, p, sh, x,
+                       gamma, beta, save_mean, save_invstd, y, relu_mask, pooled, idx);
+    const hipError_t e = hipGetLastError();
+    return e == hipSuccess ? MD2_OK : md2_report_error(MD2_ERR_HIP, hipGetErrorString(e));
+}
+
+int md2_bn_bwd_reduce_mask(const md2_bn_desc* d, const void* x, const uint8_t* relu_mask, const void* grad_y,
+                           const float* gamma, const float* save_mean, const float* save_invstd, float* grad_gamma,
+                           float* grad_beta, void* workspace, void* stream) {
+    if (!valid(d)) return md2_report_error(MD2_ERR_ARG, "bn: unsupported shape");
+    if (!(d->flags & MD2_BN_RELU)) return md2_report_error(MD2_ERR_ARG, "bn_bwd_reduce_mask: needs MD2_BN_RELU");
+    if (!x || !relu_mask || !grad_y || !gamma || !save_mean || !save_invstd || !grad_gamma || !grad_beta ||
+        !workspace)
+        return md2_report_error(MD2_ERR_ARG, "bn_bwd_reduce_mask: NULL operand");
+    if (d->flags & MD2_BN_BF16)
+        launch_bwd_reduce<uint16_t>(d, x, relu_mask, grad_y, nullptr, nullptr, gamma, save_mean, save_invstd,
+                                    grad_gamma, grad_beta, workspace, (hipStream_t)stream, true);
+    else
+        launch_bwd_reduce<float>(d, x, relu_mask, grad_y, nullptr, nullptr, gamma, save_mean, save_invstd,
+                                 grad_gamma, grad_beta, workspace, (hipStream_t)stream, true);
+    const hipError_t e = hipGetLastError();
+    return e == hipSuccess ? MD2_OK : md2_report_error(MD2_ERR_HIP, hipGetErrorString(e));
+}
+
+size_t md2_bn_coef_offset(const md2_bn_desc* d) {
+    if (!valid(d)) return 0;
+    const int NG = groups_of(d);
+    const int G = blocks_for_stats(d->pixels / NG, d->channels);
+    return 2 * (size_t)NG * G * d->channels * sizeof(float);
+}
+
 int md2_bn_bwd(const md2_bn_desc* d, const void* x, const void* y, const void* grad_y, const float* gamma,
                const float* save_mean, const float* save_invstd, void* grad_x, void* grad_residual,
                float* grad_gamma, float* grad_beta, void* workspace, void* stream) {
diff --git a/monodepth2_amd/csrc/md2_bn_expr.h b/monodepth2_amd/csrc/md2_bn_expr.h
--- /dev/null
+++ b/monodepth2_amd/csrc/md2_bn_expr.h
@@ -0,0 +1,49 @@
+#pragma once
+
+#include <hip/hip_runtime.h>
+
+#include <stdint.h>
+
+namespace md2 {
+
+__device__ __forceinline__ float4 bn_affine4(const float4 v, const float4 mu, const float4 is, const float4 ga,
+                                             const float4 be) {
+    float4 o;
+    o.x = (v.x - mu.x) * is.x * ga.x + be.x;
+    o.y = (v.y - mu.y) * is.y * ga.y + be.y;
+    o.z = (v.z - mu.z) * is.z * ga.z + be.z;
+    o.w = (v.w - mu.w) * is.w * ga.w + be.w;
+    return o;
+}
+
+__device__ __forceinline__ float4 relu4(float4 o) {
+    o.x = fmaxf(o.x, 0.f); o.y = fmaxf(o.y, 0.f); o.z = fmaxf(o.z, 0.f); o.w = fmaxf(o.w, 0.f);
+    return o;
+}
+
+__device__ __forceinline__ float4 relu_gate_bits4(const uint32_t m, float4 g) {
+    g.x = (m & 1) ? g.x : 0.f; g.y = (m & 2) ? g.y : 0.f; g.z = (m & 4) ? g.z : 0.f; g.w = (m & 8) ? g.w : 0.f;
+    return g;
+}
+__device__ __forceinline__ float4 relu_gate_mask4(const void* mask, size_t off, float4 g) {
+    return relu_gate_bits4(((const uint8_t*)mask)[off >> 2], g);
+}
+
+__device__ __forceinline__ float4 bn_bwd_dx4(const float4 gv, const float4 v, const float4 mu, const float4 k1,
+                                             const float4 k2, const float4 k3) {
+    float4 o;
+    o.x = k1.x * (gv.x - k2.x - (v.x - mu.x) * k3.x);
+    o.y = k1.y * (gv.y - k2.y - (v.y - mu.y) * k3.y);
+    o.z = k1.z * (gv.z - k2.z - (v.z - mu.z) * k3.z);
+    o.w = k1.w * (gv.w - k2.w - (v.w - mu.w) * k3.w);
+    return o;
+}
+
+__device__ __forceinline__ void pool_take(float v, int k, float& m, int& a) {
+    if (v > m || isnan(v)) {
+        m = v;
+        a = k;
+    }
+}
+
+}
diff --git a/monodepth2_amd/csrc/pool.hip b/monodepth2_amd/csrc/pool.hip
--- a/monodepth2_amd/csrc/pool.hip
+++ b/monodepth2_amd/csrc/pool.hip
@@ -6,6 +6,7 @@
 #include <stdlib.h>
 
 #include "md2_bf16.h"
+#include "md2_bn_expr.h"
 #include "md2hot.h"
 
 int md2_report_error(int code, const char* msg);
@@ -18,12 +19,7 @@
     int B, H, W, C, Ho, Wo;
 };
 
-__device__ __forceinline__ void take(float v, int k, float& m, int& a) {
-    if (v > m || isnan(v)) {
-        m = v;
-        a = k;
-    }
-}
+__device__ __forceinline__ void take(float v, int k, float& m, int& a) { md2::pool_take(v, k, m, a); }
 
 template <typename T>
 __global__ void __launch_bounds__(kThreads) maxpool_fwd_kernel(PoolArgs p, const void* __restrict__ x,
diff --git a/monodepth2_amd/csrc/stem.hip b/monodepth2_amd/csrc/stem.hip
--- a/monodepth2_amd/csrc/stem.hip
+++ b/monodepth2_amd/csrc/stem.hip
@@ -8,6 +8,7 @@
 #include <algorithm>
 #include <stdlib.h>
 
+#include "md2_bn_expr.h"
 #include "md2hot.h"
 
 int md2_report_error(int code, const char* msg);
@@ -42,6 +43,11 @@
     const float* gy;
     float* part;
     float* gw;
+    const float* z;
+    const uint8_t* mask;
+    const float* mean;
+    const float* coef;
+    int bn_groups, bn_ipg;
 };
 
 __device__ __forceinline__ float trunc16(float x) {
@@ -295,8 +301,26 @@
 }
 typedef float f32x4 __attribute__((ext_vector_type(4)));
 
-template <int C, bool BF = false, bool PF = BF>
+struct BnCoef {
+    float4 mu, k1, k2, k3;
+};
+__device__ __forceinline__ BnCoef bn_coef(const StemArgs& a, int b, int co4) {
+    const int gc = (b / a.bn_ipg) * kCo + 4 * co4, s = a.bn_groups * kCo;
+    BnCoef c;
+    c.mu = *(const float4*)(a.mean + gc);
+    c.k1 = *(const float4*)(a.coef + gc);
+    c.k2 = *(const float4*)(a.coef + s + gc);
+    c.k3 = *(const float4*)(a.coef + 2 * s + gc);
+    return c;
+}
+__device__ __forceinline__ float4 bn_dy(const BnCoef& c, uint32_t m, const float4 g, const float4 z) {
+    return md2::bn_bwd_dx4(md2::relu_gate_bits4(m, g), z, c.mu, c.k1, c.k2, c.k3);
+}
+
+template <int C, bool BF = false, bool PF = BF, bool FUSE = false>
 __global__ __launch_bounds__(kTThreads, 2) void stem_x6_wgrad_tr_kernel(StemArgs a) {
+    static_assert(!(BF && FUSE), "the fused BatchNorm backward is fp32");
+    static_assert(kTThreads % 16 == 0, "one channel quad per thread");
     constexpr int CP = C == 3 ? 4 : 6, NB = (7 * CP + 15) / 16;
     constexpr int XE = 7 * kTCols * CP, GE = kTSeg * kCo;
     constexpr int NPL = BF ? 1 : 3;
@@ -356,6 +380,8 @@
         constexpr int LX = (NXT + kTThreads - 1) / kTThreads;
         using RT = typename std::conditional<BF, uint2, float4>::type;
         RT rg[LG], rx[LX];
+        float4 rz[FUSE ? LG : 1];
+        uint32_t rm[FUSE ? LG : 1];
         auto put3 = [&](__bf16* base, int stride, int o, float4 v) {
             const float e[4] = {v.x, v.y, v.z, v.w};
             float c[3][4];
@@ -381,6 +407,11 @@
                 const size_t go = ((size_t)(b * a.Ho + oh) * a.Wo + ow) * kCo + 4 * co4;
                 if constexpr (BF) rg[k] = (i < NGT && ow < a.Wo) ? *(const uint2*)(gh + go) : uint2{0u, 0u};
                 else rg[k] = (i < NGT && ow < a.Wo) ? *(const float4*)(a.gy + go) : float4{0.f, 0.f, 0.f, 0.f};
+                if constexpr (FUSE) {
+                    const bool in = i < NGT && ow < a.Wo;
+                    rz[k] = in ? *(const float4*)(a.z + go) : float4{0.f, 0.f, 0.f, 0.f};
+                    rm[k] = in ? (uint32_t)a.mask[go >> 2] : 0x100u;
+                }
             }
             if constexpr (BF) {
 #pragma unroll
@@ -461,11 +492,16 @@
         };
         if (n > 0) fetch(t0);
         for (int t = 0; t < n; ++t) {
+            BnCoef bc;
+            if constexpr (FUSE) bc = bn_coef(a, (t0 + t) / (a.nseg * a.Ho), tid & 15);
 #pragma unroll
             for (int k = 0; k < LG; ++k) {
                 const int i = tid + k * kTThreads;
                 if (NGT % kTThreads && i >= NGT) break;
                 if constexpr (BF) *(u32x2*)&gs[0][tr_goff(i >> 4, i & 15)] = u32x2{rg[k].x, rg[k].y};
+                else if constexpr (FUSE)
+                    put3(&gs[0][0], GE, tr_goff(i >> 4, i & 15),
+                         (rm[k] & 0x100u) ? rg[k] : bn_dy(bc, rm[k], rg[k], rz[k]));
                 else put3(&gs[0][0], GE, tr_goff(i >> 4, i & 15), rg[k]);
             }
 #pragma unroll
@@ -494,6 +530,8 @@
         const int tt = t0 + t, per_img = a.nseg * a.Ho, b = tt / per_img, rem = tt - b * per_img;
         const int seg = rem / a.Ho, oh = rem - seg * a.Ho;
         const int ow0 = seg * kTSeg, iw0 = 2 * ow0 - 3;
+        BnCoef bc;
+        if constexpr (FUSE) bc = bn_coef(a, b, tid & 15);
         for (int i = tid; i < kTSeg * 16; i += kTThreads) {
             const int px = i >> 4, co4 = i & 15, ow = ow0 + px;
             if constexpr (BF) {
@@ -503,7 +541,11 @@
                 continue;
             }
             float4 v = {0.f, 0.f, 0.f, 0.f};
-            if (ow < a.Wo) v = *(const float4*)(a.gy + ((size_t)(b * a.Ho + oh) * a.Wo + ow) * kCo + 4 * co4);
+            if (ow < a.Wo) {
+                const size_t go = ((size_t)(b * a.Ho + oh) * a.Wo + ow) * kCo + 4 * co4;
+                v = *(const float4*)(a.gy + go);
+                if constexpr (FUSE) v = bn_dy(bc, a.mask[go >> 2], v, *(const float4*)(a.z + go));
+            }
             const float e[4] = {v.x, v.y, v.z, v.w};
             float c[3][4];
 #pragma unroll
@@ -941,8 +983,8 @@
     return sizeof(float) * (size_t)(a.C / kCG) * a.splits * kCo * kOut;
 }
 
-int md2_stem_wgrad(const md2_stem_desc* d, const float* x, const float* grad_y, float* grad_weight, void* workspace,
-                   void* stream) {
+static int stem_wgrad_impl(const md2_stem_desc* d, const float* x, const float* grad_y, const StemArgs* fuse,
+                           float* grad_weight, void* workspace, void* stream) {
     if (!valid(d)) return md2_report_error(MD2_ERR_ARG, "stem_wgrad: channels 3/6/9, 32-bit element count");
     if (!x || !grad_y || !grad_weight || !workspace) return md2_report_error(MD2_ERR_ARG, "stem_wgrad: NULL operand");
     const bool tr = use_tr(d);
@@ -953,19 +995,37 @@
     a.gy = grad_y;
     a.part = (float*)workspace;
     a.gw = grad_weight;
+    if (fuse) {
+        if (!tr || (d->flags & MD2_STEM_BF16))
+            return md2_report_error(MD2_ERR_ARG, "stem_wgrad_bn: fp32, channels 3 / 6, the transposed-read kernel");
+        if (!fuse->z || !fuse->mask || !fuse->mean || !fuse->coef || fuse->bn_groups < 1 || a.B % fuse->bn_groups)
+            return md2_report_error(MD2_ERR_ARG, "stem_wgrad_bn: NULL operand or batch not a multiple of groups");
+        a.z = fuse->z;
+        a.mask = fuse->mask;
+        a.mean = fuse->mean;
+        a.coef = fuse->coef;
+        a.bn_groups = fuse->bn_groups;
+        a.bn_ipg = a.B / fuse->bn_groups;
+    }
     const int NG = a.C / kCG;
     const hipStream_t st = (hipStream_t)stream;
     if (tr) {
         const bool bf = (d->flags & MD2_STEM_BF16) != 0;
-        static const bool pf32 = [] {
+        static const bool pf32_env = [] {
             const char* e = getenv("MD2_STEM_PF32");
             return e && e[0] == '1';
         }();
+        const bool pf32 = pf32_env || (d->flags & MD2_STEM_PREFETCH);
         void (*k)(StemArgs) =
             a.C == 3 ? (bf ? stem_x6_wgrad_tr_kernel<3, true>
                            : (pf32 ? stem_x6_wgrad_tr_kernel<3, false, true> : stem_x6_wgrad_tr_kernel<3>))
                      : (bf ? stem_x6_wgrad_tr_kernel<6, true>
                            : (pf32 ? stem_x6_wgrad_tr_kernel<6, false, true> : stem_x6_wgrad_tr_kernel<6>));
+        if (fuse)
+            k = a.C == 3 ? (pf32 ? stem_x6_wgrad_tr_kernel<3, false, true, true>
+                                 : stem_x6_wgrad_tr_kernel<3, false, false, true>)
+                         : (pf32 ? stem_x6_wgrad_tr_kernel<6, false, true, true>
+                                 : stem_x6_wgrad_tr_kernel<6, false, false, true>);
         hipLaunchKernelGGL(k, dim3(a.splits), dim3(kTThreads), 0, st, a);
     } else {
         void (*k)(StemArgs) =
@@ -976,6 +1036,27 @@
     hipLaunchKernelGGL(stem_wgrad_final_kernel, dim3((outs + kFinOut - 1) / kFinOut), dim3(256), 0, st, a);
     const hipError_t e = hipGetLastError();
     return e == hipSuccess ? MD2_OK : md2_report_error(MD2_ERR_HIP, hipGetErrorString(e));
+}
+
+int md2_stem_wgrad(const md2_stem_desc* d, const float* x, const float* grad_y, float* grad_weight, void* workspace,
+                   void* stream) {
+    return stem_wgrad_impl(d, x, grad_y, nullptr, grad_weight, workspace, stream);
+}
+
+int md2_stem_wgrad_bn_supported(const md2_stem_desc* d) {
+    return valid(d) && use_tr(d) && !(d->flags & MD2_STEM_BF16);
+}
+
+int md2_stem_wgrad_bn(const md2_stem_desc* d, const float* x, const float* grad, const float* z,
+                      const uint8_t* relu_mask, const float* save_mean, const float* coef, int bn_groups,
+                      float* grad_weight, void* workspace, void* stream) {
+    StemArgs f = {};
+    f.z = z;
+    f.mask = relu_mask;
+    f.mean = save_mean;
+    f.coef = coef;
+    f.bn_groups = bn_groups;
+    return stem_wgrad_impl(d, x, grad, &f, grad_weight, workspace, stream);
 }
 
 int md2_stem_fwd(const md2_stem_desc* d, const float* x, const float* weight, float* y, void* stream) {
diff --git a/monodepth2_amd/networks/resnet_encoder.py b/monodepth2_amd/networks/resnet_encoder.py
--- a/monodepth2_amd/networks/resnet_encoder.py
+++ b/monodepth2_amd/networks/resnet_encoder.py
@@ -6,9 +6,9 @@
 import torch
 import torch.nn as nn
 
-from ..bn_ops import bn_act, max_pool_3x3s2, max_pool_3x3s2_with_alias
+from ..bn_ops import bn_act
 from ..conv_ops import conv2d
-from ..stem_ops import stem_conv
+from ..stem_ops import stem_bn_pool
 
 
 def _conv3x3(cin, cout, stride=1):
@@ -165,10 +165,9 @@
     def forward(self, input_image):
         return self.forward_prepared(self.prepare(input_image))
 
-    def forward_prepared(self, x):
+    def forward_prepared(self, x, need_f0: bool = True):
         e = self.encoder
-        f0 = bn_act(e.bn1, stem_conv(e.conv1, x))
-        x, xs, f0 = max_pool_3x3s2_with_alias(e.maxpool, f0, out_alias=True)
+        x, xs, f0 = stem_bn_pool(e.conv1, e.bn1, e.maxpool, x, need_f0=need_f0)
         feats = [f0]
         layers = [e.layer1, e.layer2, e.layer3, e.layer4]
         for li, layer in enumerate(layers):
diff --git a/monodepth2_amd/stem_ops.py b/monodepth2_amd/stem_ops.py
--- a/monodepth2_amd/stem_ops.py
+++ b/monodepth2_amd/stem_ops.py
@@ -109,6 +109,133 @@
         return None, gw.to(torch.bfloat16).to(torch.float32)
 
 
+FUSE = os.environ.get("MD2_STEM_FUSE", "1") != "0"
+FUSE_FWD = os.environ.get("MD2_STEM_FUSE_FWD", "1") != "0"
+FUSE_WGRAD = os.environ.get("MD2_STEM_FUSE_WGRAD", "1") != "0"
+
+
+def bn_relu_pool_fwd(z, gamma, beta, running_mean, running_var, eps: float, momentum: float, groups: int,
+                     need_y: bool):
+    from . import bn_ops
+    B, C, H, W = z.shape
+    Ho, Wo = (H - 1) // 2 + 1, (W - 1) // 2 + 1
+    key = (B * H * W, C, _lib.BN_RELU, eps, momentum, groups)
+    d, nbytes = bn_ops._desc(key)
+    L = _lib.lib()
+    ws = bn_ops._workspace(z.device, nbytes)
+    stats = torch.empty(2, groups, C, device=z.device)
+    mean, invstd = stats[0], stats[1]
+    mask = torch.empty(z.numel() // 4, dtype=torch.uint8, device=z.device)
+    p = torch.empty((B, C, Ho, Wo), device=z.device, dtype=z.dtype, memory_format=_CL)
+    idx = torch.empty(B * Ho * Wo * C // 4, device=z.device, dtype=torch.int32)
+    stream = _lib.stream(z.device)
+    rm = running_mean.data_ptr() if running_mean is not None else None
+    rv = running_var.data_ptr() if running_var is not None else None
+    if FUSE_FWD and L.md2_bn_pool_fwd_supported(ctypes.byref(d), H, W):
+        y = torch.empty_like(z, memory_format=_CL) if need_y else None
+        _lib.check(L.md2_bn_pool_fwd(ctypes.byref(d), H, W, z.data_ptr(), gamma.data_ptr(), beta.data_ptr(), rm, rv,
+                                     y.data_ptr() if y is not None else None, mask.data_ptr(), p.data_ptr(),
+                                     idx.data_ptr(), mean.data_ptr(), invstd.data_ptr(), ws.data_ptr(), stream),
+                   "md2_bn_pool_fwd")
+    else:
+        y = torch.empty_like(z, memory_format=_CL)
+        _lib.check(L.md2_bn_fwd_mask(ctypes.byref(d), z.data_ptr(), gamma.data_ptr(), beta.data_ptr(), None, rm, rv,
+                                     y.data_ptr(), mask.data_ptr(), mean.data_ptr(), invstd.data_ptr(),
+                                     ws.data_ptr(), stream), "md2_bn_fwd_mask")
+        pd = _lib.PoolDesc(B, C, H, W, 0, 0)
+        _lib.check(L.md2_maxpool3s2_fwd(ctypes.byref(pd), y.data_ptr(), p.data_ptr(), idx.data_ptr(), stream),
+                   "md2_maxpool3s2_fwd")
+    return p, idx, mask, y, mean, invstd, key
+
+
+class _StemBNPool(torch.autograd.Function):
+
+    @staticmethod
+    def forward(ctx, x, weight, gamma, beta, running_mean, running_var, eps: float, momentum: float, groups: int,
+                need_f0: bool):
+        z = _fwd(x, weight)
+        p, idx, mask, y, mean, invstd, key = bn_relu_pool_fwd(z, gamma, beta, running_mean, running_var, eps,
+                                                              momentum, groups, need_f0)
+        ctx.save_for_backward(x, z, mask, idx, gamma, mean, invstd)
+        ctx.bn_key = key
+        ctx.w_cl = weight.is_contiguous(memory_format=_CL)
+        ctx.w_shape = weight.shape
+        ctx.set_materialize_grads(False)
+        return (p, p.view_as(p)) + ((y,) if need_f0 else ())
+
+    @staticmethod
+    def backward(ctx, gp, gp2, gf0=None):
+        from . import bn_ops
+        x, z, mask, idx, gamma, mean, invstd = ctx.saved_tensors
+        if gp is None:
+            gp, gp2 = gp2, None
+        if gp is None and gf0 is None:
+            return (None,) * 10
+        L = _lib.lib()
+        B, C, H, W = z.shape
+        stream = _lib.stream(z.device)
+        if gf0 is not None:
+            gf0 = gf0.to(z.dtype).contiguous(memory_format=_CL)
+        if gp is None:
+            g = gf0
+        else:
+            gp = gp.to(z.dtype).contiguous(memory_format=_CL)
+            if gp2 is not None:
+                gp2 = gp2.to(z.dtype).contiguous(memory_format=_CL)
+            g = torch.empty_like(z, memory_format=_CL)
+            pd = _lib.PoolDesc(B, C, H, W, 0, 0)
+            _lib.check(L.md2_maxpool3s2_bwd_multi(ctypes.byref(pd), idx.data_ptr(), gp.data_ptr(),
+                                                  gp2.data_ptr() if gp2 is not None else None,
+                                                  gf0.data_ptr() if gf0 is not None else None, g.data_ptr(), stream),
+                       "md2_maxpool3s2_bwd_multi")
+        d, nbytes = bn_ops._desc(ctx.bn_key)
+        ws = bn_ops._workspace(z.device, nbytes)
+        ggamma = torch.empty_like(gamma)
+        gbeta = torch.empty_like(gamma)
+        xb, xc, xh, xw = x.shape
+        sd = _lib.StemDesc(xb, xc, xh, xw, _lib.STEM_WEIGHT_CL if ctx.w_cl else 0)
+        gw = torch.empty(ctx.w_shape, device=x.device, dtype=torch.float32,
+                         memory_format=_CL if ctx.w_cl else torch.contiguous_format)
+        sws = torch.empty(L.md2_stem_wgrad_workspace_bytes(ctypes.byref(sd)), dtype=torch.uint8, device=x.device)
+        if FUSE_WGRAD and L.md2_stem_wgrad_bn_supported(ctypes.byref(sd)):
+            _lib.check(L.md2_bn_bwd_reduce_mask(ctypes.byref(d), z.data_ptr(), mask.data_ptr(), g.data_ptr(),
+                                                gamma.data_ptr(), mean.data_ptr(), invstd.data_ptr(),
+                                                ggamma.data_ptr(), gbeta.data_ptr(), ws.data_ptr(), stream),
+                       "md2_bn_bwd_reduce_mask")
+            coef = ws.data_ptr() + L.md2_bn_coef_offset(ctypes.byref(d))
+            _lib.check(L.md2_stem_wgrad_bn(ctypes.byref(sd), x.data_ptr(), g.data_ptr(), z.data_ptr(), mask.data_ptr(),
+                                           mean.data_ptr(), coef, ctx.bn_key[5], gw.data_ptr(), sws.data_ptr(),
+                                           stream), "md2_stem_wgrad_bn")
+        else:
+            gz = torch.empty_like(z, memory_format=_CL)
+            _lib.check(L.md2_bn_bwd_mask(ctypes.byref(d), z.data_ptr(), mask.data_ptr(), g.data_ptr(), None, None,
+                                         gamma.data_ptr(), mean.data_ptr(), invstd.data_ptr(), gz.data_ptr(), None,
+                                         ggamma.data_ptr(), gbeta.data_ptr(), ws.data_ptr(), stream),
+                       "md2_bn_bwd_mask")
+            _lib.check(L.md2_stem_wgrad(ctypes.byref(sd), x.data_ptr(), gz.data_ptr(), gw.data_ptr(), sws.data_ptr(),
+                                        stream), "md2_stem_wgrad")
+        return None, gw, ggamma, gbeta, None, None, None, None, None, None
+
+
+def stem_bn_pool(conv: nn.Conv2d, bn: nn.BatchNorm2d, pool: nn.MaxPool2d, x: torch.Tensor, need_f0: bool = True):
+    from . import bn_ops
+    groups = bn_ops._GROUPS if bn.training else 1
+    if (FUSE and ENABLED and FWD_ENABLED and bn_ops.ENABLED and supports_stem(conv, x) and x.shape[1] in (3, 6)
+            and torch.is_grad_enabled() and conv.weight.requires_grad
+            and bn.training and bn.affine and bn.track_running_stats and bn.momentum is not None
+            and bn.weight.dtype == torch.float32 and x.shape[0] % groups == 0
+            and x.shape[0] * ((x.shape[2] - 1) // 2 + 1) * ((x.shape[3] - 1) // 2 + 1) * 16 // groups < 2 ** 31
+            and bn_ops._pool_geometry_ok(pool) and bn_ops._ALIAS_SUM):
+        if bn.num_batches_tracked is not None:
+            bn.num_batches_tracked.add_(groups)
+        out = _StemBNPool.apply(x, conv.weight, bn.weight, bn.bias, bn.running_mean, bn.running_var, bn.eps,
+                                bn.momentum, groups, need_f0)
+        return (out[0], out[1], out[2] if need_f0 else None)
+    f0 = bn_ops.bn_act(bn, stem_conv(conv, x))
+    p, ps, f0 = bn_ops.max_pool_3x3s2_with_alias(pool, f0, out_alias=True)
+    return p, ps, (f0 if need_f0 else None)
+
+
 def supports_stem_bf16(conv: nn.Conv2d, x: torch.Tensor) -> bool:
     from .conv_ops import _bf16_autocast
     return (BF16_ENABLED and x.is_cuda and x.dtype == torch.float32 and conv.weight.dtype == torch.float32
diff --git a/monodepth2_amd/trainer.py b/monodepth2_amd/trainer.py
--- a/monodepth2_amd/trainer.py
+++ b/monodepth2_amd/trainer.py
@@ -275,7 +275,7 @@
                 enc = models["pose_encoder"]
                 x = enc.prepare(pairs)
                 with bn_groups(len(temporal)):
-                    feats = enc.forward_prepared(x)
+                    feats = enc.forward_prepared(x, need_f0=False)
                 dec = getattr(models["pose"], "module", models["pose"])
                 dec.packed_output = True
                 try:
```

Result: faster. 1096 images/s, median of 6 (+1.8%).
